# SMART-TTS/SMART-NAR_Fast_TTS

Hardware: AMD Instinct MI355X
Metric: mel_frames_per_sec (higher is better)
Workload: dtype f32

## Files before the change

### include/nar_fs2.h

```cpp
#ifndef NAR_FS2_H
#define NAR_FS2_H

#include <stddef.h>
#include <stdint.h>

#ifdef __cplusplus
extern "C" {
#endif

#define NS_ABI_VERSION 6

typedef struct ns_model ns_model;

typedef struct ns_config {
  int32_t n_vocab;
  int32_t max_seq_len;
  int32_t d_enc, n_enc_layer, n_enc_head;
  int32_t d_dec, n_dec_layer, n_dec_head;
  int32_t d_inner;
  int32_t ffn_k1, ffn_k2;
  int32_t vp_filter, vp_kernel;
  int32_t n_bins;
  int32_t n_mel;
  int32_t postnet_dim, postnet_k, postnet_n;
// ... 73 lines not shown
int ns_op_mel_decoder(ns_model* m, const float* x, const int64_t* lens, int B, int T, float* out, void* ws, size_t ws_bytes, void* stream);
int ns_op_mel_linear(ns_model* m, const float* x, int B, int T, float* out, void* stream);
int ns_op_postnet(ns_model* m, const float* mel, int B, int T, float* out, void* ws, size_t ws_bytes, void* stream);

int ns_op_ffn_conv1(ns_model* m, const char* prefix, const float* x, int B, int S, float* hidden, void* stream);
int ns_op_attention_core(const float* qkv, const int64_t* lens, int B, int S, int H, int dk, float* out, void* scratch,
                         size_t scratch_bytes, void* stream);
int ns_op_attention_core_mode(const float* qkv, const int64_t* lens, int B, int S, int H, int dk, float* out, void* scratch,
                              size_t scratch_bytes, void* stream, int flags);
int ns_op_attention_carve(int B, int S, int H, size_t scratch_bytes, int flags, size_t* partial_floats, int32_t* has_tickets);
int ns_plan_attention_dense(int B, int S, int H, int dk, size_t scratch_floats, int has_tickets, int32_t out[4]);
int ns_op_gemm(ns_model* m, const char* name, const float* x, int B, int S, float* out, void* stream);

int ns_plan_gemm(int M, int N, int Cin, int KW, int32_t out[8]);
int ns_plan_gemm_launches(int M, int N, int Cin, int KW, int epi, int32_t out[2][8]);
int ns_plan_row_tile(int M, int N);
int ns_plan_row_tile_k(int M, int N, int K);
int ns_acc_chunk(void);
int ns_abi_version(void);
int ns_plan_attention_split(int B, int S, int H, int dk);
int ns_plan_gemm_bf16(int M, int N, int32_t* bm, int32_t* bn);
int ns_plan_gemm_bf16_ln(int M, int N, int Cin, int KW);
int ns_plan_gemm_b3(int M, int N, int Cin, int KW, int epi, int32_t out[4]);
size_t ns_op_attention_scratch_bytes(int B, int S, int H, int dk);

int ns_op_pack_plan(const int64_t* lens_dev, const int64_t* lens_host, int B, int S, int H, int guard, int32_t* plan_dev, size_t plan_ints,
                    int32_t* Mp, int32_t* att_wgs, void* stream);
int ns_op_gemm_packed(ns_model* m, const char* name, const float* x_p, const int32_t* plan_dev, int B, int S, int Mp, int att_wgs, float* out_p,
                      void* stream);
int ns_op_attention_core_packed(const float* qkv_p, const int64_t* lens, const int32_t* plan_dev, int B, int S, int Mp, int att_wgs, int H, int dk,
                                float* out_p, void* scratch , size_t scratch_bytes, void* stream, int flags);
int ns_op_attention_packed_carve(int B, int S, int H, size_t scratch_bytes, int flags, size_t* partial_floats, int32_t* has_tickets);
int ns_plan_attention_packed(int B, int S, int H, int dk, int att_wgs, int Mp, size_t scratch_floats, int has_tickets, int32_t out[4]);
int ns_plan_attention_split_packed(int att_wgs, int S, int H, int dk, int Mp);
int ns_op_block_packed(ns_model* m, int which, const char* prefix, const float* x_p, const int64_t* lens ,
                       const int32_t* plan_dev, int B, int S, int Mp, int att_wgs, int mask_rows, float* out_p, void* ws, size_t ws_bytes,
                       void* stream);
int ns_op_length_regulate_packed(const float* x, const int32_t* cum, const int64_t* mel_lens, int B, int L, int D, int T, int Mp, int H,
                                 float* out_p, int32_t* status, int32_t* plan_dev, size_t plan_ints, void* stream);
int ns_op_gaussian_regulate(const float* x, const float* durations, const int64_t* own_len, int B, int L, int D, int T, float* out, float* s,
                            float* w, int32_t* status, int32_t* zero, int nzero, const int32_t* plan_dev, int Mp, int att_wgs, void* stream);
int ns_op_embed_pos_packed(const int64_t* texts, const float* emb, const float* pos, const int32_t* plan_dev, int B, int L, int Mp, int att_wgs, int D,
                           int n_vocab, float* out_p, void* stream);
int ns_op_add_pos_packed(const float* x_p, const float* pos, const int32_t* plan_dev, int B, int S, int Mp, int att_wgs, int D, float* out_p,
                         void* stream);
int ns_op_pack_vector(const float* src, const int32_t* plan_dev, int B, int S, int Mp, int att_wgs, float* dst_p, void* stream);
int ns_op_unpack_rows(const float* src_p, const int64_t* lens , const int32_t* plan_dev, int B, int S, int Mp, int att_wgs, int D,
                      float* dst, void* stream);
int ns_op_unpack_phase1(const float* rows_p, const float* vec_p, const int64_t* lens, const int32_t* plan_dev, int B, int S, int Mp, int att_wgs,
                        int D, float* rows, float* vec, void* stream);
int ns_op_unpack_outputs(const int32_t* plan_dev, int B, int T, int Mp, int att_wgs, int n_mel, const int64_t* mel_lens, const float* mel_p,
                         const float* post_p, const float* p_p, const float* e_p, const float* mel_bias, const float* post_const, float* mel,
                         float* post, float* p_pred, float* e_pred, uint8_t* mel_mask, void* stream);

#define NS_PROFILE_SLOTS 3
#define NS_PROFILE_OFF 0
#define NS_PROFILE_ALL 1
#define NS_PROFILE_SLOT(i) (2 << (i))
#define NS_PROFILE_KEEP 0x10000
int ns_profile_enable(ns_model* m, int on);
int ns_profile_read(ns_model* m, double* total_ms, double* total_flops, int64_t* launches);
int ns_profile_read_slot(ns_model* m, int slot, double* total_ms, double* total_flops, int64_t* launches);

#define NS_VOC_ABI_VERSION 1
typedef struct ns_vocoder ns_vocoder;
typedef struct ns_voc_config {
  int32_t n_mel;
  int32_t initial_channel;
  int32_t n_up;
  int32_t up_rates[4];
  int32_t up_kernels[4];
  int32_t n_rb;
  int32_t rb_kernels[4];
  int32_t rb_dilations[4][4];
  int32_t resblock;
} ns_voc_config;
int ns_voc_abi_version(void);
int ns_voc_create(const ns_voc_config* cfg, ns_vocoder** out);
void ns_voc_destroy(ns_vocoder* v);
int ns_voc_set_matmul(ns_vocoder* v, int mode);
size_t ns_voc_arena_bytes(const ns_vocoder* v);
int ns_voc_bind_arena(ns_vocoder* v, void* dev_arena, size_t bytes);
int ns_voc_set_weight(ns_vocoder* v, const char* name, const float* host, const int64_t* shape, int ndim);
int ns_voc_check_weight(ns_vocoder* v, const char* name, const int64_t* shape, int ndim);
int ns_voc_finalize_weights(ns_vocoder* v, void* stream);
size_t ns_voc_ws_bytes(const ns_vocoder* v, int B, int T);
#define NS_VOC_MEL_CHANNEL_MAJOR 0
#define NS_VOC_MEL_TIME_MAJOR 1
int ns_voc_forward(ns_vocoder* v, const float* mel, int mel_layout, int B, int T, float* wav, void* ws, size_t ws_bytes, void* stream);
int ns_voc_op_conv(ns_vocoder* v, const char* name, const float* x, int B, int S, float* out, void* stream);
int ns_voc_op_conv_form(ns_vocoder* v, const char* name, const float* x, const float* resid, float* y, int B, int S, int in_act,
                        int out_act, int mrf, void* stream);
int ns_voc_op_upsample(ns_vocoder* v, int i, const float* x, int B, int S, float* out, void* stream);
size_t ns_voc_op_stage_ws_bytes(const ns_vocoder* v, int i, int B, int S);
int ns_voc_op_stage(ns_vocoder* v, int i, const float* x, int B, int S, float* out, void* ws, size_t ws_bytes, void* stream);

#define NS_ALN_ABI_VERSION 1
int ns_aln_abi_version(void);
int ns_aln_create(const ns_config* cfg, ns_aligner** out);
void ns_aln_destroy(ns_aligner* a);
size_t ns_aln_arena_bytes(const ns_aligner* a);
int ns_aln_bind_arena(ns_aligner* a, void* dev_arena, size_t bytes);
int ns_aln_set_weight(ns_aligner* a, const char* name, const float* host, const int64_t* shape, int ndim);
int ns_aln_check_weight(ns_aligner* a, const char* name, const int64_t* shape, int ndim);
int ns_aln_finalize_weights(ns_aligner* a, void* stream);
size_t ns_aln_ws_bytes(const ns_aligner* a, int B, int L, int T);
// ... 315 lines not shown
```

### smart-nar_fast_tts_amd/_lib.py

```python
from __future__ import annotations

import ctypes as C
import os

import torch

_HERE = os.path.dirname(os.path.abspath(__file__))
LIB_PATH = os.path.join(_HERE, "csrc", "libnarfs2.so")


class NsConfig(C.Structure):
    _fields_ = [(n, C.c_int32) for n in (
        "n_vocab", "max_seq_len", "d_enc", "n_enc_layer", "n_enc_head", "d_dec", "n_dec_layer", "n_dec_head",
        "d_inner", "ffn_k1", "ffn_k2", "vp_filter", "vp_kernel", "n_bins", "n_mel",
        "postnet_dim", "postnet_k", "postnet_n", "pitch_frame_level", "energy_frame_level", "length_regulator",
        "matmul_bf16x3", "row_epilogue", "phase1_packing")]


class NsLossArgs(C.Structure):
    _fields_ = ([(n, C.c_int32) for n in ("B", "L", "T", "H", "n_mel", "pitch_frame_level", "energy_frame_level")]
                + [(n, C.c_int64) for n in ("mel_targets_stride", "d_targets_stride")]
                + [(n, C.c_void_p) for n in ("mel", "postnet", "mel_targets", "mel_masks", "pitch", "pitch_targets", "energy", "energy_targets",
                                             "log_d", "d_targets", "src_masks", "src_lens", "mel_lens")]
                + [("attn", C.c_void_p * 4)])
# ... 128 lines not shown

    "ns_last_phase2_rows": (C.c_int64, [_P]),
    "ns_plan_gemm": (_I, [_I, _I, _I, _I, C.POINTER(C.c_int32)]),
    "ns_plan_gemm_launches": (_I, [_I, _I, _I, _I, _I, C.POINTER(C.c_int32)]),
    "ns_plan_row_tile": (_I, [_I, _I]),
    "ns_plan_row_tile_k": (_I, [_I, _I, _I]),
    "ns_acc_chunk": (_I, []),
    "ns_plan_attention_split": (_I, [_I, _I, _I, _I]),
    "ns_op_ws_bytes": (_Z, [_P, _I, _I]),
    "ns_op_mask_from_lengths": (_I, [_P, _I, _I, _P, _P]),
    "ns_op_sinusoid_table": (_I, [_I, _I, _P, _P]),
    "ns_op_txt_encoder": (_I, [_P, _P, _P, _I, _I, _P, _P, _Z, _P]),
    "ns_op_multi_head_attention": (_I, [_P, _S, _P, _P, _I, _I, _P, _P, _Z, _P]),
    "ns_op_positionwise_ffn": (_I, [_P, _S, _P, _I, _I, _P, _P, _Z, _P]),
    "ns_op_fft_block": (_I, [_P, _S, _P, _P, _I, _I, _P, _P, _Z, _P]),
    "ns_op_variance_predictor": (_I, [_P, _S, _P, _P, _I, _I, _P, _P, _Z, _P]),
    "ns_op_predictor_conv1": (_I, [_P, _S, _P, _I, _I, _P, _P, _Z, _P]),
    "ns_op_predictor_tail": (_I, [_P, _S, _P, _P, _I, _I, _F, _P, _P, _I, _P, _P, _P, _Z, _P]),
    "ns_op_duration_round": (_I, [_P, _I, _F, _P, _P]),
    "ns_op_duration_scan": (_I, [_P, _I, _I, _P, _P, _P]),
    "ns_op_duration_target_scan": (_I, [_P, _P, _P, _I, _I, _I, _P, _P, _P, _P, _P]),
    "ns_op_length_regulate": (_I, [_P, _P, _I, _I, _I, _I, _P, _P]),
    "ns_op_variance_embedding": (_I, [_P, _I, _P, _P, _I, _I, _F, _P, _P, _P, _P, _Z, _P]),
    "ns_op_bucketize": (_I, [_P, _I, _P, _I, _P, _P]),
    "ns_op_gaussian_upsampling": (_I, [_P, _P, _I, _I, _I, _I, _I, _P, _P, _P, _P]),
    "ns_op_mel_decoder": (_I, [_P, _P, _P, _I, _I, _P, _P, _Z, _P]),
    "ns_op_mel_linear": (_I, [_P, _P, _I, _I, _P, _P]),
    "ns_op_postnet": (_I, [_P, _P, _I, _I, _P, _P, _Z, _P]),
    "ns_op_ffn_conv1": (_I, [_P, _S, _P, _I, _I, _P, _P]),
    "ns_op_attention_core": (_I, [_P, _P, _I, _I, _I, _I, _P, _P, _Z, _P]),
    "ns_op_attention_core_mode": (_I, [_P, _P, _I, _I, _I, _I, _P, _P, _Z, _P, _I]),
    "ns_op_attention_carve": (_I, [_I, _I, _I, _Z, _I, C.POINTER(C.c_size_t), C.POINTER(C.c_int32)]),
    "ns_plan_attention_dense": (_I, [_I, _I, _I, _I, _Z, _I, C.POINTER(C.c_int32)]),
    "ns_op_gemm": (_I, [_P, _S, _P, _I, _I, _P, _P]),
    "ns_plan_gemm_bf16": (_I, [_I, _I, C.POINTER(C.c_int32), C.POINTER(C.c_int32)]),
    "ns_plan_gemm_bf16_ln": (_I, [_I, _I, _I, _I]),
    "ns_plan_gemm_b3": (_I, [_I, _I, _I, _I, _I, C.POINTER(C.c_int32)]),
    "ns_op_attention_scratch_bytes": (_Z, [_I, _I, _I, _I]),
    "ns_op_pack_plan": (_I, [_P, _P, _I, _I, _I, _I, _P, _Z, C.POINTER(C.c_int32), C.POINTER(C.c_int32), _P]),
    "ns_op_gemm_packed": (_I, [_P, _S, _P, _P, _I, _I, _I, _I, _P, _P]),
    "ns_op_attention_core_packed": (_I, [_P, _P, _P, _I, _I, _I, _I, _I, _I, _P, _P, _Z, _P, _I]),
    "ns_op_attention_packed_carve": (_I, [_I, _I, _I, _Z, _I, C.POINTER(C.c_size_t), C.POINTER(C.c_int32)]),
    "ns_plan_attention_packed": (_I, [_I, _I, _I, _I, _I, _I, _Z, _I, C.POINTER(C.c_int32)]),
    "ns_plan_attention_split_packed": (_I, [_I, _I, _I, _I, _I]),
    "ns_op_block_packed": (_I, [_P, _I, _S, _P, _P, _P, _I, _I, _I, _I, _I, _P, _P, _Z, _P]),
    "ns_op_length_regulate_packed": (_I, [_P, _P, _P, _I, _I, _I, _I, _I, _I, _P, _P, _P, _Z, _P]),
    "ns_op_gaussian_regulate": (_I, [_P, _P, _P, _I, _I, _I, _I, _P, _P, _P, _P, _P, _I, _P, _I, _I, _P]),
    "ns_op_embed_pos_packed": (_I, [_P, _P, _P, _P, _I, _I, _I, _I, _I, _I, _P, _P]),
    "ns_op_add_pos_packed": (_I, [_P, _P, _P, _I, _I, _I, _I, _I, _P, _P]),
    "ns_op_pack_vector": (_I, [_P, _P, _I, _I, _I, _I, _P, _P]),
    "ns_op_unpack_rows": (_I, [_P, _P, _P, _I, _I, _I, _I, _I, _P, _P]),
    "ns_op_unpack_phase1": (_I, [_P, _P, _P, _P, _I, _I, _I, _I, _I, _P, _P, _P]),
    "ns_op_unpack_outputs": (_I, [_P, _I, _I, _I, _I, _I, _P, _P, _P, _P, _P, _P, _P, _P, _P, _P, _P, _P, _P]),
    "ns_profile_enable": (_I, [_P, _I]),
    "ns_profile_read": (_I, [_P, C.POINTER(C.c_double), C.POINTER(C.c_double), C.POINTER(C.c_int64)]),
    "ns_profile_read_slot": (_I, [_P, _I, C.POINTER(C.c_double), C.POINTER(C.c_double), C.POINTER(C.c_int64)]),
    **_handle_family("ns_voc", _P),
    "ns_voc_set_matmul": (_I, [_P, _I]),
    "ns_voc_ws_bytes": (_Z, [_P, _I, _I]),
    "ns_voc_forward": (_I, [_P, _P, _I, _I, _I, _P, _P, _Z, _P]),
    "ns_voc_op_conv": (_I, [_P, _S, _P, _I, _I, _P, _P]),
    "ns_voc_op_conv_form": (_I, [_P, _S, _P, _P, _P, _I, _I, _I, _I, _I, _P]),
    "ns_voc_op_upsample": (_I, [_P, _I, _P, _I, _I, _P, _P]),
    "ns_voc_op_stage_ws_bytes": (_Z, [_P, _I, _I, _I]),
    "ns_voc_op_stage": (_I, [_P, _I, _P, _I, _I, _P, _P, _Z, _P]),
    **_handle_family("ns_aln", C.POINTER(NsConfig)),
    "ns_aln_ws_bytes": (_Z, [_P, _I, _I, _I]),
    "ns_aln_forward": (_I, [_P, _P, _P, _P, _P, _I, _I, _I, _P, _P, _P, _P, _Z, _P]),
    "ns_aln_op_cross_attention": (_I, [_P, _P, _P, _I, _I, _I, _I, _I, _P, _P, _P]),
    "ns_aln_op_input": (_I, [_P, _P, _I, _I, _I, _P]),
    "ns_aln_op_durations": (_I, [_P, _P, _P, _I, _I, _I, _I, _P, _P]),
    "ns_loss_abi_version": (_I, []),
    "ns_loss_ws_bytes": (_Z, [_I, _I, _I]),
    "ns_loss_forward": (_I, [C.POINTER(NsLossArgs), _P, _Z, _P, _P]),
    **_handle_family("ns_mel", C.POINTER(NsMelConfig)),
    "ns_mel_frames": (C.c_int64, [C.c_int64, C.c_int32]),
    "ns_mel_ws_bytes": (_Z, [_P, _I, C.c_int64]),
    "ns_mel_forward": (_I, [_P, _P, C.c_int64, _P, _I, C.c_int64, _I, _P, _P, _P, _P, _Z, _P]),
    "ns_mel_op_frame_rows": (_I, [_P, _P, C.c_int64, _P, _I, C.c_int64, _I, _P, _P, _P]),
    "ns_mel_op_stft": (_I, [_P, _P, _I, _I, _P, _P]),
    "ns_mel_op_project": (_I, [_P, _P, _P, _I, _I, C.c_int64, _I, _P, _P, _P]),
    **_handle_family("ns_gl", C.POINTER(NsGlConfig)),
    "ns_gl_ws_bytes": (_Z, [_P, _I, _I]),
    "ns_gl_forward": (_I, [_P, _P, _P, _I, _I, _P, _I, _P, C.c_int64, _P, _P, _Z, _P]),
    "ns_gl_forward_mag": (_I, [_P, _P, _P, _I, _I, _P, _I, _P, C.c_int64, _P, _P, _Z, _P]),
    "ns_gl_transform": (_I, [_P, _P, C.c_int64, _P, _I, C.c_int64, _I, _P, _P, _P, _Z, _P]),
    "ns_gl_op_mel_to_mag": (_I, [_P, _P, _P, _I, _I, _P, _P]),
    "ns_gl_op_recombine": (_I, [_P, _P, _P, _P, _I, _I, _P, _P]),
    "ns_gl_op_rephase": (_I, [_P, _P, _P, _P, _I, _I, _I, _P, _P]),
    "ns_gl_op_inverse": (_I, [_P, _P, _P, _I, _I, _P, C.c_int64, _P, _P, _Z, _P]),
    "ns_gl_op_frame_rows": (_I, [_P, _P, C.c_int64, _P, _I, C.c_int64, _I, _P, _P]),
    "ns_gl_op_step": (_I, [_P, _P, _P, _I, _I, _P, C.c_int64, _P, _P, _Z, _P]),
    "ns_vt_abi_version": (_I, []),
    "ns_vt_ws_bytes": (_Z, [_I, _I, _I]),
    "ns_vt_state_init": (_I, [_P, _P]),
    "ns_vt_targets": (_I, [C.POINTER(NsVtArgs), _P, _Z, _P]),
    "ns_vt_fit": (_I, [C.POINTER(NsVtArgs), _P, _P, _Z, _P]),
    "ns_vt_normalize": (_I, [C.POINTER(NsVtArgs), _P, _P, _Z, _P]),
    "ns_opt_abi_version": (_I, []),
    "ns_opt_plan_sizes": (_I, [C.POINTER(C.c_int64), _I, C.POINTER(NsOptPlan)]),
    "ns_opt_build_table": (_I, [C.POINTER(C.c_int64), C.POINTER(_P), C.POINTER(_P), C.POINTER(C.c_int32), _I, _P, _Z]),
    "ns_opt_grad_norm": (_I, [C.POINTER(NsOptPlan), _P, _Z, _F, _P, _Z, _P, _P]),
    "ns_opt_scale_grads": (_I, [C.POINTER(NsOptPlan), _P, _Z, _P, _P]),
    "ns_opt_adam_step": (_I, [C.POINTER(NsOptPlan), _P, _Z, C.POINTER(NsOptHyper), _P, _P, C.c_int64, _P, _P]),
    "ns_opt_zero_grads": (_I, [C.POINTER(NsOptPlan), _P, _Z, _P]),
    "ns_lossg_abi_version": (_I, []),
# ... 89 lines not shown
```

### smart-nar_fast_tts_amd/csrc/api.hip

```cpp
#include <cstdio>

#include "../../include/nar_fs2.h"
#include "host_core.h"

using namespace ns;

static thread_local std::string g_err;
static int fail(const std::string& s) { g_err = s; return 1; }

namespace {

struct LayerW { ConvW qkv, fc, w1, w2; size_t ln1_g, ln1_b, ln2_g, ln2_b; };
struct PredW { ConvW c1, c2; size_t ln1_g, ln1_b, ln2_g, ln2_b, lin_w, lin_b; };

}

struct ns_model {
  ns_config cfg;
  std::vector<LayerW> enc, dec;
  PredW pred[3];
  size_t hdr;
  size_t emb, enc_pos, dec_pos, pitch_bins, energy_bins, pitch_emb, energy_emb;
  ConvW mel_linear;
  size_t pn_in, pn_hid, pn_const;
  size_t pos_long;
  std::vector<ConvW> post;
  Arena ar;
  float* arena = nullptr;
  bool ready = false;
  WeightRegistry weights;
  const float* P(size_t off) const { return arena + off; }
  const unsigned short* plane(size_t off) const { return off != NO_PLANE ? reinterpret_cast<const unsigned short*>(P(off)) : nullptr; }
  ConvGemm conv(const ConvW& w) const {
    ConvGemm p;
    memset(&p, 0, sizeof(p));
    p.W = P(w.w); p.bias = P(w.b); p.Wb3 = plane(w.b3); p.Wbf = plane(w.bf);
    p.N = w.cout; p.Cin = w.cin; p.KW = w.kw; p.pad = (w.kw - 1) / 2;
    return p;
  }
  struct ProfSlot { std::vector<std::pair<hipEvent_t, hipEvent_t>> ev; size_t used = 0; double flops = 0.0; };
  long long last_rows = 0;
  long long last_rows1 = 0;
  unsigned prof = 0;
  bool prof_active = false;
  ProfSlot prof_slot[NS_PROFILE_SLOTS];
};

static const char* kPredNames[3] = {"duration", "pitch", "energy"};

constexpr uint32_t ARENA_MAGIC = 0x3246534eu;
constexpr uint32_t ARENA_LAYOUT_VERSION = 6;
constexpr int ARENA_HDR_WORDS = 16;
static void arena_header(const ns_model* m, uint32_t* w) {
  memset(w, 0, ARENA_HDR_WORDS * sizeof(uint32_t));
  uint64_t h = 1469598103934665603ull;
  ns_config lay = m->cfg;
  lay.row_epilogue = 0;
  lay.phase1_packing = 0;
  const unsigned char* cb = reinterpret_cast<const unsigned char*>(&lay);
  for (size_t i = 0; i < sizeof(ns_config); ++i) { h ^= cb[i]; h *= 1099511628211ull; }
  w[0] = ARENA_MAGIC; w[1] = ARENA_LAYOUT_VERSION;
  w[2] = (uint32_t)(m->ar.n & 0xffffffffu); w[3] = (uint32_t)((uint64_t)m->ar.n >> 32);
  w[4] = (uint32_t)(h & 0xffffffffu); w[5] = (uint32_t)(h >> 32);
  w[6] = 1;
}
constexpr int POS_LONG_ROWS = 8192;
constexpr int PN_CONST_ROWS = 32;

static void expect(ns_model* m, const std::string& name, std::vector<int64_t> shape, bool optional = false) {
  m->weights.expect(name, std::move(shape), optional);
}

static void take_b3(Arena& ar, ConvW& w) { w.b3 = ar.take((3 * w.elems() + 1) / 2); }
static void take_bf(Arena& ar, ConvW& w) { w.bf = ar.take((bf16_plane_elems(w.cout, w.kw, w.cin) + 1) / 2); }
static void fill_planes(float* img, const ConvW& w) {
  if (w.b3 != NO_PLANE) {
    const size_t n = w.elems();
    unsigned short* pl = reinterpret_cast<unsigned short*>(&img[w.b3]);
    split_weights_b3(&img[w.w], n, pl, pl + n, pl + 2 * n);
  }
  if (w.bf != NO_PLANE) round_weights_bf16(&img[w.w], w.cout, w.kw, w.cin, reinterpret_cast<unsigned short*>(&img[w.bf]));
}

static void plan_stack(ns_model* m, const char* prefix, int n_layer, int d, std::vector<LayerW>& out, bool decoder) {
  const ns_config& c = m->cfg;
  for (int i = 0; i < n_layer; ++i) {
    std::string p = std::string(prefix) + ".layer_stack." + std::to_string(i);
    for (const char* w : {"w_qs", "w_ks", "w_vs", "fc"}) {
      expect(m, p + ".slf_attn." + w + ".weight", {d, d});
      expect(m, p + ".slf_attn." + w + ".bias", {d});
    }
    expect(m, p + ".slf_attn.layer_norm.weight", {d});
    expect(m, p + ".slf_attn.layer_norm.bias", {d});
    expect(m, p + ".pos_ffn.w_1.weight", {c.d_inner, d, c.ffn_k1});
    expect(m, p + ".pos_ffn.w_1.bias", {c.d_inner});
    expect(m, p + ".pos_ffn.w_2.weight", {d, c.d_inner, c.ffn_k2});
    expect(m, p + ".pos_ffn.w_2.bias", {d});
    expect(m, p + ".pos_ffn.layer_norm.weight", {d});
    expect(m, p + ".pos_ffn.layer_norm.bias", {d});
    LayerW L;
    L.qkv = m->ar.conv(3 * d, 1, d);
    L.fc = m->ar.conv(d, 1, d);
    L.ln1_g = m->ar.take(d); L.ln1_b = m->ar.take(d);
    L.w1 = m->ar.conv(c.d_inner, c.ffn_k1, d);
    L.w2 = m->ar.conv(d, c.ffn_k2, c.d_inner);
    L.ln2_g = m->ar.take(d); L.ln2_b = m->ar.take(d);
    if (c.matmul_bf16x3 == 1 && decoder)
      for (ConvW* w : {&L.qkv, &L.fc, &L.w1, &L.w2}) take_b3(m->ar, *w);
    if (c.matmul_bf16x3 == 2 && decoder)
      for (ConvW* w : {&L.qkv, &L.fc, &L.w1, &L.w2}) take_bf(m->ar, *w);
    out.push_back(L);
  }
}

extern "C" const char* ns_last_error(void) { return g_err.c_str(); }
int ns::api_fail(const char* msg) { return fail(msg); }

extern "C" int ns_create(const ns_config* cfg, ns_model** out) {
  if (!cfg || !out) return fail("ns_create: null argument");
// ... 21 lines not shown
  expect(m, "txt_encoder.src_word_emb.weight", {c.n_vocab, d});
  expect(m, "txt_encoder.position_enc", {1, npos, d}, true);
  expect(m, "mel_decoder.position_enc", {1, npos, c.d_dec}, true);
  m->emb = m->ar.take((size_t)c.n_vocab * d);
  m->enc_pos = m->ar.take((size_t)npos * d);
  m->dec_pos = m->ar.take((size_t)npos * c.d_dec);
  plan_stack(m, "txt_encoder", c.n_enc_layer, d, m->enc, false);
  plan_stack(m, "mel_decoder", c.n_dec_layer, c.d_dec, m->dec, true);
  const int F = c.vp_filter, K = c.vp_kernel;
  for (int i = 0; i < 3; ++i) {
    std::string p = std::string("variance_adaptor.") + kPredNames[i] + "_predictor";
    expect(m, p + ".conv_layer.conv1d_1.conv.weight", {F, d, K});
    expect(m, p + ".conv_layer.conv1d_1.conv.bias", {F});
    expect(m, p + ".conv_layer.layer_norm_1.weight", {F});
    expect(m, p + ".conv_layer.layer_norm_1.bias", {F});
    expect(m, p + ".conv_layer.conv1d_2.conv.weight", {F, F, K});
    expect(m, p + ".conv_layer.conv1d_2.conv.bias", {F});
    expect(m, p + ".conv_layer.layer_norm_2.weight", {F});
    expect(m, p + ".conv_layer.layer_norm_2.bias", {F});
    expect(m, p + ".linear_layer.weight", {1, F});
    expect(m, p + ".linear_layer.bias", {1});
    PredW& w = m->pred[i];
    w.c1 = m->ar.conv(F, K, d);
    w.ln1_g = m->ar.take(F); w.ln1_b = m->ar.take(F);
    w.c2 = m->ar.conv(F, K, F);
    w.ln2_g = m->ar.take(F); w.ln2_b = m->ar.take(F);
    w.lin_w = m->ar.take(F); w.lin_b = m->ar.take(1);
  }
  expect(m, "variance_adaptor.pitch_bins", {c.n_bins - 1});
  expect(m, "variance_adaptor.energy_bins", {c.n_bins - 1});
  expect(m, "variance_adaptor.pitch_embedding.weight", {c.n_bins, d});
  expect(m, "variance_adaptor.energy_embedding.weight", {c.n_bins, d});
  m->pitch_bins = m->ar.take(c.n_bins); m->energy_bins = m->ar.take(c.n_bins);
  m->pitch_emb = m->ar.take((size_t)c.n_bins * d); m->energy_emb = m->ar.take((size_t)c.n_bins * d);
  expect(m, "mel_linear.weight", {c.n_mel, c.d_dec});
  expect(m, "mel_linear.bias", {c.n_mel});
  m->mel_linear = m->ar.conv(c.n_mel, 1, c.d_dec);
  if (c.matmul_bf16x3 == 2) take_bf(m->ar, m->mel_linear);
  for (int i = 0; i < c.postnet_n; ++i) {
    const int cin = i == 0 ? c.n_mel : c.postnet_dim, cout = i == c.postnet_n - 1 ? c.n_mel : c.postnet_dim;
    std::string p = "postnet.convolutions." + std::to_string(i);
    expect(m, p + ".0.conv.weight", {cout, cin, c.postnet_k});
    expect(m, p + ".0.conv.bias", {cout});
    for (const char* s : {"weight", "bias", "running_mean", "running_var"}) expect(m, p + ".1." + s, {cout});
    ConvW w = m->ar.conv(cout, c.postnet_k, cin);
    if (c.matmul_bf16x3 == 1 && cin == c.postnet_dim && cout == c.postnet_dim) take_b3(m->ar, w);
    if (c.matmul_bf16x3 == 2) take_bf(m->ar, w);
    m->post.push_back(w);
  }
  m->pn_in = m->ar.take((size_t)PN_CONST_ROWS * c.n_mel);
  m->pn_hid = m->ar.take((size_t)2 * PN_CONST_ROWS * c.postnet_dim);
  m->pn_const = m->ar.take((size_t)PN_CONST_ROWS * c.n_mel);
  m->pos_long = m->ar.take((size_t)POS_LONG_ROWS * c.d_dec);
  *out = m;
  return 0;
}

extern "C" void ns_destroy(ns_model* m) {
  if (!m) return;
  for (auto& ps : m->prof_slot)
    for (auto& ev : ps.ev) { (void)hipEventDestroy(ev.first); (void)hipEventDestroy(ev.second); }
  delete m;
}
extern "C" size_t ns_arena_bytes(const ns_model* m) { return m ? m->ar.n * sizeof(float) : 0; }

extern "C" int ns_bind_arena(ns_model* m, void* dev, size_t bytes) { return bind_arena(m, dev, bytes, ns_arena_bytes(m), "ns_bind_arena"); }

extern "C" int ns_adopt_arena(ns_model* m) {
  if (!m || !m->arena) return fail("ns_adopt_arena: no arena bound");
  uint32_t got[ARENA_HDR_WORDS], want[ARENA_HDR_WORDS];
  int cur_dev = 0;
  NS_HIP(hipGetDevice(&cur_dev));
  hipPointerAttribute_t at;
  NS_HIP(hipPointerGetAttributes(&at, m->arena));
  struct DevGuard { int d; bool on; ~DevGuard() { if (on) (void)hipSetDevice(d); } } guard{cur_dev, at.device != cur_dev};
  if (guard.on) NS_HIP(hipSetDevice(at.device));
  NS_HIP(hipDeviceSynchronize());
  NS_HIP(hipMemcpy(got, m->arena + m->hdr, sizeof(got), hipMemcpyDeviceToHost));
  arena_header(m, want);
  if (got[0] != ARENA_MAGIC) return fail("ns_adopt_arena: the arena does not start with this library's magic word (not a finalized ns_model arena)");
  if (got[1] != want[1]) return fail("ns_adopt_arena: arena layout version " + std::to_string(got[1]) + ", this library packs version " + std::to_string(want[1]));
  if (got[2] != want[2] || got[3] != want[3]) return fail("ns_adopt_arena: arena size differs from ns_arena_bytes of this model");
  if (got[4] != want[4] || got[5] != want[5]) return fail("ns_adopt_arena: the arena was packed for a different ns_config");
  if (got[6] != 1) return fail("ns_adopt_arena: the arena was not finalized (ns_finalize_weights did not complete)");
  m->weights.release();
  m->ready = true;
  return 0;
}

static bool starts_with(const std::string& s, const char* p) { return s.rfind(p, 0) == 0; }
static bool ends_with(const std::string& s, const char* p) {
  size_t n = strlen(p); return s.size() >= n && s.compare(s.size() - n, n, p) == 0;
}

static bool ignored_key(const char* name) { return starts_with(name, "mel_encoder.") || ends_with(name, ".num_batches_tracked"); }

extern "C" int ns_check_weight(ns_model* m, const char* name, const int64_t* shape, int ndim) {
  if (m && name && ignored_key(name)) return 0;
  return check_weight(m, name, shape, ndim, "ns_check_weight");
}

extern "C" int ns_set_weight(ns_model* m, const char* name, const float* host, const int64_t* shape, int ndim) {
  if (m && name && ignored_key(name)) return 0;
  return set_weight(m, name, host, shape, ndim, "ns_set_weight");
}

static int postnet_constants(ns_model* m, hipStream_t st);
extern "C" int ns_finalize_weights(ns_model* m, void* stream) {
  if (!m) return fail("ns_finalize_weights: null model");
  if (!m->arena) return fail("ns_finalize_weights: bind an arena first (ns_bind_arena)");
  const std::vector<std::string> missing = m->weights.missing();
  if (!missing.empty()) return fail("ns_finalize_weights: missing keys: " + join_names(missing));
  const ns_config& c = m->cfg;
  std::vector<float> img(m->ar.n, 0.f);
  auto S = [&](const std::string& k) -> const std::vector<float>& { return m->weights.data(k); };
  auto cp = [&](size_t off, const std::string& k) { const auto& v = S(k); memcpy(&img[off], v.data(), v.size() * sizeof(float)); };

  arena_header(m, reinterpret_cast<uint32_t*>(&img[m->hdr]));
  cp(m->emb, "txt_encoder.src_word_emb.weight");
  const int npos = c.max_seq_len + 1;
  if (m->weights.is_set("txt_encoder.position_enc")) cp(m->enc_pos, "txt_encoder.position_enc");
  else host_sinusoid(npos, c.d_enc, &img[m->enc_pos]);
  if (m->weights.is_set("mel_decoder.position_enc")) cp(m->dec_pos, "mel_decoder.position_enc");
  else host_sinusoid(npos, c.d_dec, &img[m->dec_pos]);

  auto do_stack = [&](const char* prefix, std::vector<LayerW>& Ls, int d) {
    for (size_t i = 0; i < Ls.size(); ++i) {
      const LayerW& L = Ls[i];
      std::string p = std::string(prefix) + ".layer_stack." + std::to_string(i);
      const char* qkv[3] = {"w_qs", "w_ks", "w_vs"};
      for (int t = 0; t < 3; ++t) {
        memcpy(&img[L.qkv.w + (size_t)t * d * d], S(p + ".slf_attn." + qkv[t] + ".weight").data(), (size_t)d * d * 4);
        memcpy(&img[L.qkv.b + (size_t)t * d], S(p + ".slf_attn." + qkv[t] + ".bias").data(), (size_t)d * 4);
      }
      cp(L.fc.w, p + ".slf_attn.fc.weight"); cp(L.fc.b, p + ".slf_attn.fc.bias");
      cp(L.ln1_g, p + ".slf_attn.layer_norm.weight"); cp(L.ln1_b, p + ".slf_attn.layer_norm.bias");
      pack_conv(S(p + ".pos_ffn.w_1.weight"), c.d_inner, d, c.ffn_k1, &img[L.w1.w]); cp(L.w1.b, p + ".pos_ffn.w_1.bias");
      cp(L.ln2_g, p + ".pos_ffn.layer_norm.weight"); cp(L.ln2_b, p + ".pos_ffn.layer_norm.bias");
      pack_conv(S(p + ".pos_ffn.w_2.weight"), d, c.d_inner, c.ffn_k2, &img[L.w2.w]); cp(L.w2.b, p + ".pos_ffn.w_2.bias");
      for (const ConvW* w : {&L.qkv, &L.fc, &L.w1, &L.w2}) fill_planes(img.data(), *w);
    }
  };
  do_stack("txt_encoder", m->enc, c.d_enc);
  do_stack("mel_decoder", m->dec, c.d_dec);

  for (int i = 0; i < 3; ++i) {
    const PredW& w = m->pred[i];
    std::string p = std::string("variance_adaptor.") + kPredNames[i] + "_predictor";
    pack_conv(S(p + ".conv_layer.conv1d_1.conv.weight"), c.vp_filter, w.c1.cin, c.vp_kernel, &img[w.c1.w]);
    cp(w.c1.b, p + ".conv_layer.conv1d_1.conv.bias");
    cp(w.ln1_g, p + ".conv_layer.layer_norm_1.weight"); cp(w.ln1_b, p + ".conv_layer.layer_norm_1.bias");
    pack_conv(S(p + ".conv_layer.conv1d_2.conv.weight"), c.vp_filter, c.vp_filter, c.vp_kernel, &img[w.c2.w]);
    cp(w.c2.b, p + ".conv_layer.conv1d_2.conv.bias");
    cp(w.ln2_g, p + ".conv_layer.layer_norm_2.weight"); cp(w.ln2_b, p + ".conv_layer.layer_norm_2.bias");
    cp(w.lin_w, p + ".linear_layer.weight"); cp(w.lin_b, p + ".linear_layer.bias");
  }
  cp(m->pitch_bins, "variance_adaptor.pitch_bins"); cp(m->energy_bins, "variance_adaptor.energy_bins");
  cp(m->pitch_emb, "variance_adaptor.pitch_embedding.weight"); cp(m->energy_emb, "variance_adaptor.energy_embedding.weight");
  cp(m->mel_linear.w, "mel_linear.weight"); cp(m->mel_linear.b, "mel_linear.bias");
  fill_planes(img.data(), m->mel_linear);

  for (size_t i = 0; i < m->post.size(); ++i) {
    const ConvW& w = m->post[i];
    std::string p = "postnet.convolutions." + std::to_string(i);
    const auto &g = S(p + ".1.weight"), &b = S(p + ".1.bias"), &mu = S(p + ".1.running_mean"), &var = S(p + ".1.running_var");
    const auto& cb = S(p + ".0.conv.bias");
    std::vector<double> sc(w.cout);
    for (int o = 0; o < w.cout; ++o) {
      sc[o] = (double)g[o] / std::sqrt((double)var[o] + 1e-5);
      img[w.b + o] = (float)(((double)cb[o] - (double)mu[o]) * sc[o] + (double)b[o]);
    }
    pack_conv(S(p + ".0.conv.weight"), w.cout, w.cin, c.postnet_k, &img[w.w], sc.data());
    fill_planes(img.data(), w);
  }
  hipStream_t st = (hipStream_t)stream;
  NS_HIP(hipMemcpyAsync(m->arena, img.data(), img.size() * sizeof(float), hipMemcpyHostToDevice, st));
  NS_TRY(postnet_constants(m, st));
  NS_HIP(launch_sinusoid(POS_LONG_ROWS, c.d_dec, m->arena + m->pos_long, st));
  NS_HIP(hipStreamSynchronize(st));
  m->weights.release();
  m->ready = true;
  return 0;
}

namespace {
struct PackedCtx { RowMap rm; int Mp; };

struct Scratch {
  const PackedCtx* pk;
  float *xa, *xb, *qkv, *att, *t1, *x1, *hid, *vp1, *vp2, *pos_ext, *att_part;
  size_t att_part_floats;
  Tickets tk;
};

static size_t imax(size_t a, size_t b) { return a > b ? a : b; }

static Scratch carve(const ns_config& c, Bump& bp, size_t M, int S, bool no_split = false) {
  Scratch s;
  s.pk = nullptr;
  const size_t d = c.d_enc;
  s.xa = bp.f(M * d); s.xb = bp.f(M * d);
  s.qkv = bp.f(M * 3 * d); s.att = bp.f(M * d); s.t1 = bp.f(M * d); s.x1 = bp.f(M * d);
  s.hid = bp.f(M * imax(c.d_inner, 2 * (size_t)c.postnet_dim));
  s.vp1 = bp.f(M * c.vp_filter); s.vp2 = bp.f(M * c.vp_filter);
  s.pos_ext = S > c.max_seq_len ? bp.f((size_t)S * d) : nullptr;
  const int hmax = c.n_enc_head > c.n_dec_head ? c.n_enc_head : c.n_dec_head;
  int nsp = 1;
  if (!no_split && S > 0) {
    const int Bg = (int)(M / (size_t)S);
    const int ne = attention_split(Bg, S, c.n_enc_head, c.d_enc / c.n_enc_head), nd = attention_split(Bg, S, c.n_dec_head, c.d_dec / c.n_dec_head);
    nsp = ne > nd ? ne : nd;
  }
  s.att_part_floats = nsp > 1 ? (size_t)nsp * (M * d + 2 * M * hmax) : 0;
  s.att_part = s.att_part_floats ? bp.f(s.att_part_floats) : nullptr;
  s.tk.base = (int*)bp.raw(TICKET_INTS * sizeof(int));
  if (c.row_epilogue == 1) s.tk.base = nullptr;
  s.tk.used = 0;
  return s;
}
}

extern "C" size_t ns_op_ws_bytes(const ns_model* m, int B, int S) {
  if (!m || B <= 0 || S <= 0) return 256;
  Bump bp(nullptr);
  carve(m->cfg, bp, (size_t)B * S, S);
  return bp.off + 256;
}
static size_t phase1_packed_extra_bytes(const ns_config& c, int B, int L);
extern "C" size_t ns_encoder_ws_bytes(const ns_model* m, int B, int L) {
  if (!m || B <= 0 || L <= 0) return 256;
  Bump bp(nullptr);
  bp.f((size_t)B * L * m->cfg.d_enc);
  bp.raw((size_t)B * L * sizeof(int32_t));
  bp.f((size_t)B * L);
  carve(m->cfg, bp, (size_t)B * L, L);
  return bp.off + phase1_packed_extra_bytes(m->cfg, B, L) + 256;
}
static size_t packed_extra_bytes(const ns_config& c, int B, int T);
extern "C" size_t ns_decoder_ws_bytes(const ns_model* m, int B, int L, int T) {
  (void)L;
  if (!m || B <= 0 || T <= 0) return ns_op_ws_bytes(m, B, T);
  return ns_op_ws_bytes(m, B, T) + packed_extra_bytes(m->cfg, B, T);
}

static int check_ready(const ns_model* m) {
  if (!m) return fail("null model");
  if (!m->ready) return fail("weights not loaded: call ns_set_weight for every key, then ns_finalize_weights (or ns_adopt_arena)");
  return 0;
}

static const RowMap* cur_rm(const Scratch& sc) { return sc.pk ? &sc.pk->rm : nullptr; }
static int rows_of(const Scratch& sc, int B, int S) { return sc.pk ? sc.pk->Mp : B * S; }

struct GemmOpts {
  const RowEpilogue* epi = nullptr; int epi_mode = EPI_NONE;
  const LaunchTiming* tm = nullptr;
  static GemmOpts row(const RowEpilogue& e, int mode) { GemmOpts o; o.epi = &e; o.epi_mode = mode; return o; }
  static GemmOpts timed(const LaunchTiming* tm) { GemmOpts o; o.tm = tm; return o; }
};

static ConvGemm prepare(const ns_model* m, const Scratch& sc, const ConvW& w, const float* X, const float* resid, float* Y, int M, int S, int act) {
  ConvGemm p = m->conv(w);
  p.X = X; p.ldx = w.cin; p.resid = resid; p.ldr = w.cout; p.Y = Y; p.ldy = w.cout;
  p.M = M; p.S = S; p.act = act;
  if (sc.pk) { p.rm = sc.pk->rm; p.e.row_b = sc.pk->rm.row_b; p.e.row_t = sc.pk->rm.row_t; }
  return p;
}

static int gemm(const ns_model* m, const Scratch& sc, const ConvW& w, const float* X, const float* resid, float* Y, int M, int S, int act,
                hipStream_t st, const GemmOpts& o = GemmOpts()) {
  ConvGemm p = prepare(m, sc, w, X, resid, Y, M, S, act);
  const LaunchTiming* tm = o.tm;
  if (o.epi) {
    p.epi = o.epi_mode;
    p.e = *o.epi;
    if (sc.pk) { p.e.row_b = sc.pk->rm.row_b; p.e.row_t = sc.pk->rm.row_t; }
  }
  if (p.Wbf) {
    if (p.epi != EPI_NONE && p.epi != EPI_LN) return fail("gemm: the bf16 path has no predictor-tail epilogue");
    p.Wb3 = nullptr;
    p.e.ticket = nullptr; p.e.y_out = nullptr;
    if (tm && tm->start) NS_HIP(hipEventRecord(tm->start, st));
    NS_HIP(launch_conv_gemm_bf16(p, st));
    if (tm && tm->stop) NS_HIP(hipEventRecord(tm->stop, st));
    return 0;
  }
  if (p.Wb3 && conv_gemm_b3_ok(M, p.N, p.Cin, p.KW, p.epi)) {
// ... 16 lines not shown
}

static int gemm_ln(const ns_model* m, Scratch& sc, const ConvW& w, const float* X, const float* resid, float* tmp, float* Y, int M, int S,
                   int act, const float* g, const float* b, const long long* lens, hipStream_t st) {
  RowEpilogue e;
  memset(&e, 0, sizeof(e));
  e.ln_g = g; e.ln_b = b; e.lens = lens;
  const int N = w.cout;
  if (w.bf != NO_PLANE) {
    if (conv_gemm_bf16_ok(M, N, w.cin, w.kw, EPI_LN)) return gemm(m, sc, w, X, resid, Y, M, S, act, st, GemmOpts::row(e, EPI_LN));
    NS_TRY(gemm(m, sc, w, X, resid, tmp, M, S, act, st));
    NS_HIP(launch_layernorm(tmp, g, b, Y, M, N, S, lens, st, cur_rm(sc)));
    return 0;
  }
  if (w.b3 != NO_PLANE) {
    const B3LnForm form = gemm_ln_b3_form(M, N, w.cin, w.kw);
    if (form == B3_LN_TWO_LAUNCH) {
      NS_TRY(gemm(m, sc, w, X, resid, tmp, M, S, act, st));
      NS_HIP(launch_layernorm(tmp, g, b, Y, M, N, S, lens, st, cur_rm(sc)));
      return 0;
    }
    if (form == B3_LN_FULL_ROW) return gemm(m, sc, w, X, resid, Y, M, S, act, st, GemmOpts::row(e, EPI_LN));
  }
  if (sc.pk) { e.row_b = sc.pk->rm.row_b; e.row_t = sc.pk->rm.row_t; }
  return gemm_ln_fp32(prepare(m, sc, w.fp32(), X, resid, nullptr, M, S, act), e, tmp, Y, sc.tk, st, cur_rm(sc));
}

struct ProfScope {
  ns_model* m; int slot; double flops; bool on;
  LaunchTiming tm{nullptr, nullptr};
  ProfScope(ns_model* m_, int slot_, double flops_) : m(m_), slot(slot_), flops(flops_), on(m_->prof_active && ((m_->prof >> slot_) & 1u)) {}
  int begin() {
    if (!on) return 0;
    ns_model::ProfSlot& ps = m->prof_slot[slot];
    if (ps.used == ps.ev.size()) {
      hipEvent_t a, b;
      NS_HIP(hipEventCreate(&a));
      NS_HIP(hipEventCreate(&b));
      ps.ev.emplace_back(a, b);
    }
    tm = LaunchTiming{ps.ev[ps.used].first, ps.ev[ps.used].second};
    return 0;
  }
  const LaunchTiming* timing() const { return on ? &tm : nullptr; }
  void end() {
    if (!on) return;
    ns_model::ProfSlot& ps = m->prof_slot[slot];
    ps.used++;
    ps.flops += flops;
  }
};

static int mha(ns_model* m, const LayerW& L, int d, int H, const float* x, const long long* lens, int B, int S,
               float* out, bool mask_rows, Scratch& sc, hipStream_t st) {
  const int M = rows_of(sc, B, S);
  const bool bf = L.qkv.bf != NO_PLANE;
  NS_TRY(gemm(m, sc, L.qkv, x, nullptr, sc.qkv, M, S, ACT_NONE, st));
  {
    ProfScope ps(m, 1, 4.0 * (double)M * (double)S * (double)d);
    NS_TRY(ps.begin());
    NS_HIP(launch_attention(sc.qkv, lens, B, S, H, d / H, sc.att, sc.att_part, sc.att_part_floats,
                            (sc.att_part && attention_uses_tickets(B, S, H)) ? sc.tk.take(attention_ticket_ints(B, S, H)) : nullptr, st, cur_rm(sc),
                            ps.timing(), bf));
    ps.end();
  }
  return gemm_ln(m, sc, L.fc, sc.att, x, sc.t1, out, M, S, ACT_NONE, m->P(L.ln1_g), m->P(L.ln1_b), mask_rows ? lens : nullptr, st);
}

static int ffn(ns_model* m, const LayerW& L, int d, const float* x, const long long* lens, int B, int S, float* out,
               bool mask_rows, Scratch& sc, hipStream_t st) {
  const ns_config& c = m->cfg;
  const int M = rows_of(sc, B, S);
  {
    ProfScope ps(m, 0, 2.0 * (double)M * (double)c.ffn_k1 * (double)d * (double)c.d_inner);
    NS_TRY(ps.begin());
    NS_TRY(gemm(m, sc, L.w1, x, nullptr, sc.hid, M, S, ACT_RELU, st, GemmOpts::timed(ps.timing())));
    ps.end();
  }
  return gemm_ln(m, sc, L.w2, sc.hid, x, sc.t1, out, M, S, ACT_NONE, m->P(L.ln2_g), m->P(L.ln2_b), mask_rows ? lens : nullptr, st);
}

static int fft_block(ns_model* m, const LayerW& L, int d, int H, const float* x, const long long* lens, int B, int S,
                     float* out, Scratch& sc, hipStream_t st) {
  NS_TRY(mha(m, L, d, H, x, lens, B, S, sc.x1, true, sc, st));
  NS_TRY(ffn(m, L, d, sc.x1, lens, B, S, out, true, sc, st));
  return 0;
}

static int position_rows(const ns_model* m, size_t cached_off, int S, int d, Scratch& sc, const float** pos, hipStream_t st) {
  if (S > m->cfg.max_seq_len && S <= POS_LONG_ROWS) {
    *pos = m->P(m->pos_long);
  } else if (S > m->cfg.max_seq_len) {
    NS_HIP(launch_sinusoid(S, d, sc.pos_ext, st));
    *pos = sc.pos_ext;
  } else {
    *pos = m->P(cached_off);
  }
  return 0;
}

static int predictor_conv1(const ns_model* m, const PredW& w, const float* x, int B, int S, float* h, Scratch& sc, hipStream_t st) {
  const int M = rows_of(sc, B, S);
  return gemm_ln(m, sc, w.c1, x, nullptr, sc.vp1, h, M, S, ACT_RELU, m->P(w.ln1_g), m->P(w.ln1_b), nullptr, st);
}
static int predictor_tail(const ns_model* m, const PredW& w, const float* h, const long long* lens, int B, int S, float control,
                          const float* target, float* pred, const float* bins, const float* emb, const float* x_in, const float* pos,
                          float* x_out, Scratch& sc, hipStream_t st) {
  const ns_config& c = m->cfg;
  const int M = rows_of(sc, B, S), F = c.vp_filter, D = w.c1.cin;
  RowEpilogue e;
  memset(&e, 0, sizeof(e));
  e.ln_g = m->P(w.ln2_g); e.ln_b = m->P(w.ln2_b); e.lens = lens; e.wlin = m->P(w.lin_w); e.blin = m->P(w.lin_b); e.pred = pred;
  e.control = control; e.target = target; e.bins = bins; e.n_edges = c.n_bins - 1; e.emb = emb; e.x_in = x_in; e.pos = pos; e.x_out = x_out;
  e.D = D;
  if (fuse_row_epilogue(M, F, F)) return gemm(m, sc, w.c2, h, nullptr, nullptr, M, S, ACT_RELU, st, GemmOpts::row(e, EPI_LN_PRED));
  if (conv_gemm_ticket_ok(M, F, F) && (e.ticket = sc.tk.take(conv_gemm_ticket_ints(M))) != nullptr)
    return gemm(m, sc, w.c2, h, nullptr, sc.vp1, M, S, ACT_RELU, st, GemmOpts::row(e, EPI_LN_PRED));
  NS_TRY(gemm(m, sc, w.c2, h, nullptr, sc.vp1, M, S, ACT_RELU, st));
  NS_HIP(launch_ln_linear_embed(sc.vp1, m->P(w.ln2_g), m->P(w.ln2_b), m->P(w.lin_w), m->P(w.lin_b), pred, M, F, S, lens,
                                control, target, bins, c.n_bins, emb, x_in, pos, x_out, D, st, cur_rm(sc)));
  return 0;
}
static int predictor(const ns_model* m, const PredW& w, const float* x, const long long* lens, int B, int S, float control,
                     const float* target,
                     float* pred, const float* bins, const float* emb, const float* pos, float* x_out, Scratch& sc,
                     hipStream_t st) {
  NS_TRY(predictor_conv1(m, w, x, B, S, sc.vp2, sc, st));
  return predictor_tail(m, w, sc.vp2, lens, B, S, control, target, pred, bins, emb, x, pos, x_out, sc, st);
}

static int postnet(ns_model* m, const float* mel, int B, int T, const float* resid, float* out, Scratch& sc, hipStream_t st) {
  const ns_config& c = m->cfg;
  const int M = rows_of(sc, B, T);
  float* ping = sc.hid;
  float* pong = sc.hid + (size_t)M * c.postnet_dim;
  const float* cur = mel;
  for (size_t i = 0; i < m->post.size(); ++i) {
    const ConvW& w = m->post[i];
    const bool last = i + 1 == m->post.size();
    float* dst = last ? out : ((i & 1) ? pong : ping);
    const bool mid = w.cin == c.postnet_dim && w.cout == c.postnet_dim;
    ProfScope ps(m, 2, 2.0 * (double)M * (double)c.postnet_k * (double)w.cin * (double)w.cout);
    if (mid) NS_TRY(ps.begin());
    NS_TRY(gemm(m, sc, w, cur, last ? resid : nullptr, dst, M, T, last ? ACT_NONE : ACT_TANH, st, GemmOpts::timed(mid ? ps.timing() : nullptr)));
    if (mid) ps.end();
    cur = dst;
  }
  return 0;
}

static int postnet_constants(ns_model* m, hipStream_t st) {
  const ns_config& c = m->cfg;
  float* in = m->arena + m->pn_in;
  NS_HIP(launch_broadcast_row(m->P(m->mel_linear.b), in, PN_CONST_ROWS, c.n_mel, st));
  Scratch sc;
  memset(&sc, 0, sizeof(sc));
  sc.hid = m->arena + m->pn_hid;
  return postnet(m, in, 1, PN_CONST_ROWS, in, m->arena + m->pn_const, sc, st);
}

static int encoder(ns_model* m, const long long* texts, const long long* lens, int B, int L, float* out, Scratch& sc,
                   hipStream_t st) {
  const ns_config& c = m->cfg;
  const int M = rows_of(sc, B, L), d = c.d_enc;
  const float* pos;
  NS_TRY(position_rows(m, m->enc_pos, L, d, sc, &pos, st));
  float* cur = m->enc.empty() ? out : sc.xa;
  if (sc.pk) NS_HIP(launch_embed_pos_packed(texts, m->P(m->emb), pos, cur, sc.pk->rm, B, M, L, d, c.n_vocab, sc.tk.base, TICKET_INTS, st));
  else NS_HIP(launch_embed_pos(texts, m->P(m->emb), pos, cur, M, L, d, c.n_vocab, sc.tk.base, TICKET_INTS, st));
  for (size_t i = 0; i < m->enc.size(); ++i) {
    float* dst = (i + 1 == m->enc.size()) ? out : (cur == sc.xa ? sc.xb : sc.xa);
    NS_TRY(fft_block(m, m->enc[i], d, c.n_enc_head, cur, lens, B, L, dst, sc, st));
    cur = dst;
  }
  return 0;
}

static int decoder_stack(ns_model* m, float* x, const long long* lens, int B, int T, float* out, Scratch& sc, hipStream_t st) {
  const ns_config& c = m->cfg;
  float* cur = x;
  float* alt = (x == sc.xa) ? sc.xb : sc.xa;
  for (size_t i = 0; i < m->dec.size(); ++i) {
    float* dst = (i + 1 == m->dec.size()) ? out : alt;
    NS_TRY(fft_block(m, m->dec[i], c.d_dec, c.n_dec_head, cur, lens, B, T, dst, sc, st));
    if (dst != out) { alt = cur; cur = dst; }
  }
  if (m->dec.empty() && out != x) NS_HIP(hipMemcpyAsync(out, x, (size_t)rows_of(sc, B, T) * c.d_dec * 4, hipMemcpyDeviceToDevice, st));
  return 0;
}

static size_t window_rows(const int64_t* lens_host, int B, int S, int guard) {
  size_t mp = 0;
  for (int b = 0; b < B; ++b) {
    long long l = (lens_host[b] < 0 ? 0 : lens_host[b]) + guard;
    mp += (size_t)(l < (long long)S ? l : (long long)S);
  }
  return mp;
}
static int window_att_wgs(const int64_t* lens_host, int B, int S, int guard, int H) {
  int wgs = 0;
  for (int b = 0; b < B; ++b) {
    long long l = (lens_host[b] < 0 ? 0 : lens_host[b]) + guard;
    wgs += (int)(((l < S ? l : S) + 127) / 128) * H;
  }
  return wgs;
}
static size_t phase1_packed_rows(const int64_t* lens_host, int B, int L) { return window_rows(lens_host, B, L, PHONEME_GUARD); }
static size_t phase1_packed_extra_bytes(const ns_config& c, int B, int L) {
  Bump bp(nullptr);
  const size_t M = (size_t)B * L;
  bp.raw(pack_plan_ints(B, M) * sizeof(int));
  bp.f(M * c.d_enc); bp.f(M);
  return bp.off;
}

struct Teacher {
  ns_aligner* aln;
  const float* mels;
  const int64_t* mel_lens_in;
  int T;
  void* ws_aln;
  size_t ws_aln_bytes;
  float *tgt_output, *attn;
  int64_t* d_targets;
};

static int forward_durations(ns_model* m, const int64_t* texts, const int64_t* src_lens, const int64_t* lens_host, int B, int L, float d_control,
                             float p_control, float e_control, const float* p_targets, const float* e_targets,
                             void* ws_enc, size_t ws_bytes, float* log_d, float* d_rounded, uint8_t* src_mask,
                             int64_t* mel_lens, float* p_pred, float* e_pred, int64_t* mel_lens_host, void* stream,
                             const Teacher* tf = nullptr) {
  NS_TRY(check_ready(m));
  if (B <= 0 || L <= 0) return fail("ns_forward_durations: empty batch");
  if (ws_bytes < ns_encoder_ws_bytes(m, B, L)) return fail("ns_forward_durations: workspace too small");
  hipStream_t st = (hipStream_t)stream;
  const ns_config& c = m->cfg;
  if (!c.pitch_frame_level && !p_pred) return fail("ns_forward_durations: phoneme_level pitch needs a p_pred [B,L] output");
  if (!c.energy_frame_level && !e_pred) return fail("ns_forward_durations: phoneme_level energy needs an e_pred [B,L] output");
  Bump bp(ws_enc);
  float* enc_out = bp.f((size_t)B * L * c.d_enc);
  int32_t* cum = (int32_t*)bp.raw((size_t)B * L * sizeof(int32_t));
  float* dur_keep = bp.f((size_t)B * L);
  const long long* lens = (const long long*)src_lens;
  size_t Mp = 0;
  bool packed = lens_host && !m->enc.empty() && launch_planner_enabled() && c.pitch_frame_level && c.energy_frame_level && c.phase1_packing != 2;
  if (packed) {
    Mp = phase1_packed_rows(lens_host, B, L);
    auto cu_rows = [&](size_t rows) {
      const size_t ntn = (size_t)c.d_inner / 128, w32 = (rows + 31) / 32 * ntn, w48 = (rows + 47) / 48 * ntn;
      return (conv_gemm_tile16_enabled() && w32 > 256 && w48 <= 256) ? (size_t)48 : 32 * ((w32 + 255) / 256);
    };
    packed = Mp > 0 && Mp * 10 <= (size_t)B * L * 9 && (c.phase1_packing == 1 || cu_rows(Mp) < cu_rows((size_t)B * L));
  }
  const size_t Mrows = packed ? Mp : (size_t)B * L;
  m->last_rows1 = (long long)Mrows;
  Scratch sc = carve(c, bp, Mrows, L, packed);
  PackedCtx pk;
  memset(&pk, 0, sizeof(pk));
  float *enc_w = enc_out, *logd_w = log_d;
  if (packed) {
    const int M = (int)Mp, d = c.d_enc;
    const int base = window_att_wgs(lens_host, B, L, PHONEME_GUARD, c.n_enc_head);
    size_t n = (size_t)attention_split_packed(base, L, d / c.n_enc_head, Mp, d);
    const size_t per = Mp * d + 2 * Mp * c.n_enc_head;
    const size_t extra = phase1_packed_extra_bytes(c, B, L);
    const size_t avail = ws_bytes > bp.off + extra ? (ws_bytes - bp.off - extra) / sizeof(float) : 0;
    while (n > 1 && n * per > avail) --n;
    if (n > 1) { sc.att_part_floats = n * per; sc.att_part = bp.f(sc.att_part_floats); }
    int* plan = (int*)bp.raw(pack_plan_ints(B, Mp) * sizeof(int));
    enc_w = bp.f(Mp * d); logd_w = bp.f(Mp);
    if (bp.off > ws_bytes) return fail("ns_forward_durations: workspace too small (packed rows)");
    pk.Mp = M;
    pk.rm.rows = M;
    pk.rm.att_wgs = base;
    NS_HIP(launch_pack_plan_only(lens, B, L, c.n_enc_head, M, plan, &pk.rm, st, PHONEME_GUARD));
  }
  {
    sc.pk = packed ? &pk : nullptr;
    NS_TRY(encoder(m, (const long long*)texts, lens, B, L, enc_w, sc, st));
    if (tf) {
      if (tf->T > 0) NS_TRY(ns_aln_forward(tf->aln, enc_w, src_lens, tf->mels, tf->mel_lens_in, B, L, tf->T, tf->tgt_output, tf->attn, tf->d_targets,
                                           tf->ws_aln, tf->ws_aln_bytes, stream));
      else NS_HIP(hipMemsetAsync(tf->d_targets, 0, (size_t)B * L * sizeof(int64_t), st));
    }
    NS_TRY(predictor(m, m->pred[0], enc_w, lens, B, L, 1.0f, nullptr, logd_w, nullptr, nullptr, nullptr, nullptr, sc, st));
    if (!c.pitch_frame_level)
      NS_TRY(predictor(m, m->pred[1], enc_w, lens, B, L, p_control, p_targets, p_pred, m->P(m->pitch_bins), m->P(m->pitch_emb), nullptr, enc_w, sc, st));
    if (!c.energy_frame_level)
      NS_TRY(predictor(m, m->pred[2], enc_w, lens, B, L, e_control, e_targets, e_pred, m->P(m->energy_bins), m->P(m->energy_emb), nullptr, enc_w, sc, st));
  }
  if (packed) {
    NS_HIP(launch_unpack_phase1(pk.rm, lens, B, L, c.d_enc, enc_w, enc_out, logd_w, log_d, st));
  }
  if (tf) {
    NS_HIP(launch_duration_target_tail((const long long*)tf->d_targets, lens, (const long long*)texts, c.n_vocab, B, L, dur_keep, cum,
                                       (long long*)mel_lens, src_mask, st));
    return 0;
  }
  NS_HIP(launch_duration_tail(log_d, lens, (const long long*)texts, c.n_vocab, B, L, d_control, d_rounded, dur_keep, cum,
                              (long long*)mel_lens, src_mask, (long long*)mel_lens_host, st));
  return 0;
}

extern "C" int ns_forward_durations(ns_model* m, const int64_t* texts, const int64_t* src_lens, int B, int L, float d_control,
                                    float p_control, float e_control, const float* p_targets, const float* e_targets,
                                    void* ws_enc, size_t ws_bytes, float* log_d, float* d_rounded, uint8_t* src_mask,
                                    int64_t* mel_lens, float* p_pred, float* e_pred, int64_t* mel_lens_host, void* stream) {
  return forward_durations(m, texts, src_lens, nullptr, B, L, d_control, p_control, e_control, p_targets, e_targets, ws_enc, ws_bytes, log_d,
                           d_rounded, src_mask, mel_lens, p_pred, e_pred, mel_lens_host, stream);
}

extern "C" int ns_forward_durations_teacher(ns_model* m, ns_aligner* aln, const int64_t* texts, const int64_t* src_lens, const float* mels,
                                            const int64_t* mel_lens_in, int B, int L, int T, float p_control, float e_control,
                                            const float* p_targets, const float* e_targets, void* ws_enc, size_t ws_enc_bytes, void* ws_aln,
                                            size_t ws_aln_bytes, float* log_d, uint8_t* src_mask, int64_t* mel_lens, float* p_pred, float* e_pred,
                                            float* tgt_output, float* attn_all_layers, int64_t* d_targets, void* stream) {
  if (!aln) return fail("ns_forward_durations_teacher: null aligner");
  if (T < 0) return fail("ns_forward_durations_teacher: negative T");
  if (!log_d || !src_mask || !mel_lens || !d_targets) return fail("ns_forward_durations_teacher: log_d, src_mask, mel_lens and d_targets are required");
  if (T > 0 && (!mels || !mel_lens_in || !tgt_output || !attn_all_layers || !ws_aln))
    return fail("ns_forward_durations_teacher: mels, mel_lens_in, tgt_output, attn_all_layers and ws_aln are required when T > 0");
  if (m && m->cfg.d_enc != 256) return fail("ns_forward_durations_teacher: the aligner takes a 256-wide encoder output (ns_aln_create)");
  if (T > 0 && B > 0 && L > 0 && ws_aln_bytes < ns_aln_ws_bytes(aln, B, L, T)) return fail("ns_forward_durations_teacher: aligner workspace too small (ns_aln_ws_bytes)");
  if (T > 0 && (((uintptr_t)ws_aln & 255) || ((uintptr_t)ws_enc & 255) || (((uintptr_t)mels | (uintptr_t)tgt_output) & 15)))
    return fail("ns_forward_durations_teacher: workspaces must be 256-byte aligned, mels and tgt_output 16-byte aligned");
  const Teacher tf = {aln, mels, mel_lens_in, T, ws_aln, ws_aln_bytes, tgt_output, attn_all_layers, d_targets};
  return forward_durations(m, texts, src_lens, nullptr, B, L, 1.0f, p_control, e_control, p_targets, e_targets, ws_enc, ws_enc_bytes, log_d,
                           nullptr, src_mask, mel_lens, p_pred, e_pred, nullptr, stream, &tf);
}

extern "C" int ns_upload_lengths(const int64_t* host, int n, int64_t* dev, void* stream) {
  if (n < 0 || (n > 0 && (!host || !dev))) return fail("ns_upload_lengths: null argument");
  NS_HIP(launch_store_lens((const long long*)host, n, (long long*)dev, (hipStream_t)stream));
  return 0;
}

extern "C" int ns_forward_durations_packed(ns_model* m, const int64_t* texts, const int64_t* src_lens, const int64_t* src_lens_host, int B, int L,
                                           float d_control, float p_control, float e_control, const float* p_targets, const float* e_targets,
                                           void* ws_enc, size_t ws_bytes, float* log_d, float* d_rounded, uint8_t* src_mask,
                                           int64_t* mel_lens, float* p_pred, float* e_pred, int64_t* mel_lens_host, void* stream) {
  if (!src_lens_host) return fail("ns_forward_durations_packed: src_lens_host (the host copy of src_lens) is required");
  return forward_durations(m, texts, src_lens, src_lens_host, B, L, d_control, p_control, e_control, p_targets, e_targets, ws_enc, ws_bytes, log_d,
                           d_rounded, src_mask, mel_lens, p_pred, e_pred, mel_lens_host, stream);
}

static size_t packed_rows(const int64_t* lens_host, int B, int T) { return window_rows(lens_host, B, T, PACK_GUARD); }
static size_t packed_extra_bytes(const ns_config& c, int B, int T) {
  Bump bp(nullptr);
  const size_t M = (size_t)B * T;
  bp.raw(pack_plan_ints(B, M) * sizeof(int));
  bp.f(M * c.n_mel); bp.f(M * c.n_mel); bp.f(M); bp.f(M); bp.f(M); bp.f(M);
  return bp.off;
}

static int forward_mel(ns_model* m, int B, int L, int T, const int64_t* mel_lens, const int64_t* lens_host, float p_control, float e_control,
                       const float* p_targets, const float* e_targets,
                       const void* ws_enc, void* ws_dec, size_t ws_bytes, float* mel, float* postnet_mel, float* p_pred,
                       float* e_pred, uint8_t* mel_mask, int32_t* status, void* stream) {
  NS_TRY(check_ready(m));
  if (B <= 0 || L <= 0) return fail("ns_forward_mel: empty batch");
  if (!status) return fail("ns_forward_mel: status [B] is required (a T smaller than an utterance's length must not go unnoticed)");
  if (T < 0) return fail("ns_forward_mel: negative T");
  if (T == 0) {
    Bump be0(const_cast<void*>(ws_enc));
    be0.f((size_t)B * L * m->cfg.d_enc);
    const int32_t* cum0 = (const int32_t*)be0.raw((size_t)B * L * sizeof(int32_t));
    NS_HIP(launch_length_regulate(nullptr, cum0, B, L, m->cfg.d_enc, 0, nullptr, nullptr, (const long long*)mel_lens, status, nullptr, 0, (hipStream_t)stream));
    return 0;
  }
  if (ws_bytes < ns_decoder_ws_bytes(m, B, L, T)) return fail("ns_forward_mel: workspace too small");
  hipStream_t st = (hipStream_t)stream;
  const ns_config& c = m->cfg;
  Bump be(const_cast<void*>(ws_enc));
  const float* enc_out = be.f((size_t)B * L * c.d_enc);
  const int32_t* cum = (const int32_t*)be.raw((size_t)B * L * sizeof(int32_t));
  const float* dur_keep = be.f((size_t)B * L);
  const long long* lens = (const long long*)mel_lens;
  const int d = c.d_dec;
  size_t Mp = 0;
  bool packed = lens_host && c.matmul_bf16x3 != 1 && !m->dec.empty();
  if (packed) {
    Mp = packed_rows(lens_host, B, T);
    const size_t grid_rows = (size_t)B * T;
    packed = Mp > 0 && Mp < ((size_t)1 << 30) && Mp * 10 <= grid_rows * (grid_rows <= 20000 ? 8 : 9);
  }
  const size_t Mrows = packed ? Mp : (size_t)B * T;
  const int M = (int)Mrows;
  m->last_rows = (long long)Mrows;
  Bump bp(ws_dec);
  Scratch sc = carve(c, bp, Mrows, T, packed);
  if (packed) {
    const int base = window_att_wgs(lens_host, B, T, PACK_GUARD, c.n_dec_head);
    size_t n = (size_t)attention_split_packed(base, T, d / c.n_dec_head, Mrows, d);
    if (n > 1) {
      const size_t per = Mrows * d + 2 * Mrows * c.n_dec_head;
      const size_t avail = ws_bytes > bp.off + packed_extra_bytes(c, B, T) ? (ws_bytes - bp.off - packed_extra_bytes(c, B, T)) / sizeof(float) : 0;
      while (n > 1 && n * per > avail) --n;
      if (n > 1) { sc.att_part_floats = n * per; sc.att_part = bp.f(sc.att_part_floats); }
    }
  }

  PackedCtx pk;
  memset(&pk, 0, sizeof(pk));
  float *mel_p = nullptr, *post_p = nullptr, *pp_p = nullptr, *ep_p = nullptr;
  if (packed) {
    int* plan = (int*)bp.raw(pack_plan_ints(B, Mp) * sizeof(int));
    mel_p = bp.f(Mp * c.n_mel); post_p = bp.f(Mp * c.n_mel); pp_p = bp.f(Mp); ep_p = bp.f(Mp);
    float* pt_p = bp.f(Mp);
    float* et_p = bp.f(Mp);
    if (bp.off > ws_bytes) return fail("ns_forward_mel_packed: workspace too small");
    pk.Mp = M;
    pk.rm.rows = M;
    if (c.length_regulator == 1) {
      if ((size_t)B * (L + 1) > (size_t)M * c.vp_filter) return fail("ns_forward_mel: workspace too small for the Gaussian centres");
      NS_HIP(launch_pack_plan(lens, B, T, c.n_dec_head, M, plan, &pk.rm, st));
      NS_HIP(launch_gaussian_upsampling(enc_out, dur_keep, B, L, c.d_enc, T, T, sc.xa, sc.vp2, nullptr, lens, status, sc.tk.base, TICKET_INTS, st, &pk.rm));
    } else {
      NS_HIP(launch_length_regulate_packed(enc_out, cum, B, L, c.d_enc, T, M, c.n_dec_head, sc.xa, lens, status, sc.tk.base, TICKET_INTS, plan, &pk.rm, st));
    }
    pk.rm.att_wgs = window_att_wgs(lens_host, B, T, PACK_GUARD, c.n_dec_head);
    if (p_targets && c.pitch_frame_level) { NS_HIP(launch_pack_vector(pk.rm, T, p_targets, pt_p, M, st)); p_targets = pt_p; }
    if (e_targets && c.energy_frame_level) { NS_HIP(launch_pack_vector(pk.rm, T, e_targets, et_p, M, st)); e_targets = et_p; }
  } else if (c.length_regulator == 1) {
    NS_HIP(launch_mask_from_lengths(lens, B, T, mel_mask, st));
    if ((size_t)B * (L + 1) > (size_t)M * c.vp_filter) return fail("ns_forward_mel: workspace too small for the Gaussian centres");
    NS_HIP(launch_gaussian_upsampling(enc_out, dur_keep, B, L, c.d_enc, T, T, sc.xa, sc.vp2, nullptr, lens, status, sc.tk.base, TICKET_INTS, st));
  } else {
    NS_HIP(launch_length_regulate(enc_out, cum, B, L, c.d_enc, T, sc.xa, mel_mask, lens, status, sc.tk.base, TICKET_INTS, st));
  }
  sc.pk = packed ? &pk : nullptr;
  float* const mel_dst = packed ? mel_p : mel;
  float* const post_dst = packed ? post_p : postnet_mel;
  float* const pp_dst = packed ? pp_p : p_pred;
  float* const ep_dst = packed ? ep_p : e_pred;
  const float* pos;
  NS_TRY(position_rows(m, m->dec_pos, T, d, sc, &pos, st));
  float* cur = sc.xa;
  float* alt = sc.xb;
  if (c.pitch_frame_level) {
    if (!p_pred) return fail("ns_forward_mel: frame_level pitch needs a p_pred [B,T] output");
    NS_TRY(predictor(m, m->pred[1], cur, lens, B, T, p_control, p_targets, pp_dst, m->P(m->pitch_bins), m->P(m->pitch_emb),
                     c.energy_frame_level ? nullptr : pos, alt, sc, st));
    float* t = cur; cur = alt; alt = t;
  }
  if (c.energy_frame_level) {
    if (!e_pred) return fail("ns_forward_mel: frame_level energy needs an e_pred [B,T] output");
    NS_TRY(predictor(m, m->pred[2], cur, lens, B, T, e_control, e_targets, ep_dst, m->P(m->energy_bins), m->P(m->energy_emb), pos,
                     alt, sc, st));
    float* t = cur; cur = alt; alt = t;
  }
  if (!c.pitch_frame_level && !c.energy_frame_level) {
    NS_HIP(launch_add_pos(cur, pos, alt, M, T, d, st, cur_rm(sc)));
    float* t = cur; cur = alt; alt = t;
  }
  m->prof_active = m->prof != 0;
  int rc = decoder_stack(m, cur, lens, B, T, sc.att, sc, st);
  if (!rc) rc = gemm(m, sc, m->mel_linear, sc.att, nullptr, mel_dst, M, T, ACT_NONE, st);
  if (!rc) rc = postnet(m, mel_dst, B, T, mel_dst, post_dst, sc, st);
  m->prof_active = false;
  if (!rc && packed) {
    hipError_t e = launch_unpack_outputs(pk.rm, B, T, c.n_mel, lens, mel_p, post_p, c.pitch_frame_level ? pp_p : nullptr,
                                         c.energy_frame_level ? ep_p : nullptr, m->P(m->mel_linear.b), m->P(m->pn_const) + (size_t)21 * c.n_mel, mel, postnet_mel,
                                         c.pitch_frame_level ? p_pred : nullptr, c.energy_frame_level ? e_pred : nullptr, mel_mask, st);
    if (e != hipSuccess) rc = fail(std::string("launch_unpack_outputs: ") + hipGetErrorString(e));
  }
  return rc;
}

extern "C" int64_t ns_last_phase2_rows(const ns_model* m) { return m ? (int64_t)m->last_rows : 0; }
extern "C" int64_t ns_last_phase1_rows(const ns_model* m) { return m ? (int64_t)m->last_rows1 : 0; }

extern "C" int ns_forward_mel(ns_model* m, int B, int L, int T, const int64_t* mel_lens, float p_control, float e_control,
                              const float* p_targets, const float* e_targets,
                              const void* ws_enc, void* ws_dec, size_t ws_bytes, float* mel, float* postnet_mel, float* p_pred,
                              float* e_pred, uint8_t* mel_mask, int32_t* status, void* stream) {
  return forward_mel(m, B, L, T, mel_lens, nullptr, p_control, e_control, p_targets, e_targets, ws_enc, ws_dec, ws_bytes, mel, postnet_mel,
                     p_pred, e_pred, mel_mask, status, stream);
}

extern "C" int ns_forward_mel_packed(ns_model* m, int B, int L, int T, const int64_t* mel_lens, const int64_t* mel_lens_host,
                                     float p_control, float e_control, const float* p_targets, const float* e_targets,
                                     const void* ws_enc, void* ws_dec, size_t ws_bytes, float* mel, float* postnet_mel, float* p_pred,
                                     float* e_pred, uint8_t* mel_mask, int32_t* status, void* stream) {
  if (!mel_lens_host) return fail("ns_forward_mel_packed: mel_lens_host (the host copy of mel_lens) is required");
  return forward_mel(m, B, L, T, mel_lens, mel_lens_host, p_control, e_control, p_targets, e_targets, ws_enc, ws_dec, ws_bytes, mel,
                     postnet_mel, p_pred, e_pred, mel_mask, status, stream);
}

static int find_layer(ns_model* m, const char* prefix_c, const LayerW** L, int* d, int* H, const char* suffix) {
  std::string p(prefix_c ? prefix_c : "");
  if (suffix && *suffix) {
    if (!ends_with(p, suffix)) return fail("prefix '" + p + "' does not end with '" + suffix + "'");
    p.resize(p.size() - strlen(suffix));
  }
  const bool enc = starts_with(p, "txt_encoder.layer_stack."), dec = starts_with(p, "mel_decoder.layer_stack.");
  if (!enc && !dec) return fail("unknown module prefix '" + std::string(prefix_c ? prefix_c : "") + "'");
  const char* num = p.c_str() + (enc ? strlen("txt_encoder.layer_stack.") : strlen("mel_decoder.layer_stack."));
  char* end = nullptr;
  const long idx = strtol(num, &end, 10);
  if (end == num || *end != 0 || *num < '0' || *num > '9') return fail("no layer index in '" + std::string(prefix_c ? prefix_c : "") + "'");
  auto& v = enc ? m->enc : m->dec;
  if (idx < 0 || idx >= (long)v.size()) return fail("layer index out of range in '" + p + "'");
  *L = &v[idx];
  *d = enc ? m->cfg.d_enc : m->cfg.d_dec;
  *H = enc ? m->cfg.n_enc_head : m->cfg.n_dec_head;
  return 0;
}

#define NS_OP_PROLOGUE(B_, S_)                                                        \
// ... 39 lines not shown
  NS_TRY(find_layer(m, prefix, &L, &d, &H, ""));
  return fft_block(m, *L, d, H, x, (const long long*)lens, B, S, out, sc, st);
}
static int find_pred(const char* prefix, int* idx) {
  std::string p(prefix ? prefix : "");
  for (int i = 0; i < 3; ++i)
    if (p == std::string("variance_adaptor.") + kPredNames[i] + "_predictor") { *idx = i; return 0; }
  return fail("unknown predictor prefix '" + p + "'");
}
extern "C" int ns_op_variance_predictor(ns_model* m, const char* prefix, const float* x, const int64_t* lens, int B, int S,
                                        float* out, void* ws, size_t ws_bytes, void* stream) {
  NS_OP_PROLOGUE(B, S);
  int i;
  NS_TRY(find_pred(prefix, &i));
  return predictor(m, m->pred[i], x, (const long long*)lens, B, S, 1.0f, nullptr, out, nullptr, nullptr, nullptr, nullptr, sc, st);
}
extern "C" int ns_op_duration_round(const float* log_d, int n, float d_control, float* d_rounded, void* stream) {
  NS_HIP(launch_duration_round(log_d, n, d_control, d_rounded, (hipStream_t)stream));
  return 0;
}
extern "C" int ns_op_duration_target_scan(const int64_t* d_targets, const int64_t* src_lens, const int64_t* texts, int n_vocab, int B, int L,
                                          int32_t* cum, float* dur_keep, uint8_t* src_mask, int64_t* mel_lens, void* stream) {
  if (B < 0 || L < 0) return fail("ns_op_duration_target_scan: negative size");
  if (B > 0 && (!src_lens || !mel_lens || (L > 0 && (!d_targets || !cum || !dur_keep || !src_mask)))) return fail("ns_op_duration_target_scan: null argument");
  NS_HIP(launch_duration_target_tail((const long long*)d_targets, (const long long*)src_lens, (const long long*)texts, n_vocab, B, L, dur_keep, cum,
                                     (long long*)mel_lens, src_mask, (hipStream_t)stream));
  return 0;
}
extern "C" int ns_op_duration_scan(const float* d_rounded, int B, int L, int32_t* cum, int64_t* mel_lens, void* stream) {
  NS_HIP(launch_duration_scan(d_rounded, B, L, cum, (long long*)mel_lens, (hipStream_t)stream));
  return 0;
}
extern "C" int ns_op_length_regulate(const float* x, const int32_t* cum, int B, int L, int D, int T, float* out, void* stream) {
  NS_HIP(launch_length_regulate(x, cum, B, L, D, T, out, nullptr, nullptr, nullptr, nullptr, 0, (hipStream_t)stream));
  return 0;
}
extern "C" int ns_op_variance_embedding(ns_model* m, int which, const float* x, const int64_t* lens, int B, int S, float control,
                                        const float* target, float* pred, float* x_out, void* ws, size_t ws_bytes, void* stream) {
  NS_OP_PROLOGUE(B, S);
  if (which != 0 && which != 1) return fail("which must be 0 (pitch) or 1 (energy)");
  const size_t bins = which ? m->energy_bins : m->pitch_bins, emb = which ? m->energy_emb : m->pitch_emb;
  return predictor(m, m->pred[1 + which], x, (const long long*)lens, B, S, control, target, pred, m->P(bins), m->P(emb), nullptr, x_out,
                   sc, st);
}
extern "C" int ns_op_predictor_conv1(ns_model* m, const char* prefix, const float* x, int B, int S, float* h, void* ws, size_t ws_bytes,
                                     void* stream) {
  if (!m) return fail("null model");
  int i;
  NS_TRY(find_pred(prefix, &i));
  if (!x || !h || !ws) return fail("ns_op_predictor_conv1: null argument");
  NS_OP_PROLOGUE(B, S);
  return predictor_conv1(m, m->pred[i], x, B, S, h, sc, st);
}
extern "C" int ns_op_predictor_tail(ns_model* m, const char* prefix, const float* h, const int64_t* lens, int B, int S, float control,
                                    const float* target, const float* x_in, int add_pos, float* pred, float* x_out, void* ws,
                                    size_t ws_bytes, void* stream) {
  if (!m) return fail("null model");
  int i;
  NS_TRY(find_pred(prefix, &i));
  if (!h || !lens || !pred || !ws) return fail("ns_op_predictor_tail: null argument");
  if (i == 0 && (x_in || x_out || add_pos)) return fail("ns_op_predictor_tail: the duration predictor has no embedding");
  if (x_in && !x_out) return fail("ns_op_predictor_tail: x_in without x_out");
  if (!x_in && (x_out || add_pos)) return fail("ns_op_predictor_tail: x_out / add_pos without x_in");
  NS_OP_PROLOGUE(B, S);
  const PredW& w = m->pred[i];
  const float *bins = nullptr, *emb = nullptr, *pos = nullptr;
  if (x_in) {
    bins = m->P(i == 2 ? m->energy_bins : m->pitch_bins);
    emb = m->P(i == 2 ? m->energy_emb : m->pitch_emb);
    if (add_pos) NS_TRY(position_rows(m, m->dec_pos, S, w.c1.cin, sc, &pos, st));
  }
  return predictor_tail(m, w, h, (const long long*)lens, B, S, control, target, pred, bins, emb, x_in, pos, x_out, sc, st);
}
extern "C" int ns_plan_gemm(int M, int N, int Cin, int KW, int32_t out[8]) {
  int o[8] = {0, 0, 0, 0, 0, 0, 0, 0};
  const bool planned = conv_gemm_plan(M, N, Cin, KW, o);
  if (out) for (int i = 0; i < 8; ++i) out[i] = planned ? o[i] : 0;
  return planned ? 1 : 0;
}
extern "C" int ns_plan_gemm_launches(int M, int N, int Cin, int KW, int epi, int32_t out[2][8]) {
  int o[2][8];
  const int n = conv_gemm_describe(M, N, Cin, KW, epi, o);
  if (out)
    for (int l = 0; l < 2; ++l)
      for (int i = 0; i < 8; ++i) out[l][i] = o[l][i];
  return n;
}
extern "C" int ns_plan_row_tile_k(int M, int N, int K) {
  if (M <= 0 || K <= 0 || (N != 256 && N != 512)) return 0;
  return conv_gemm_row_tile(M, N, K);
}
extern "C" int ns_plan_row_tile(int M, int N) { return ns_plan_row_tile_k(M, N, N); }
extern "C" int ns_acc_chunk(void) { return conv_gemm_acc_chunk(); }
extern "C" int ns_abi_version(void) { return NS_ABI_VERSION; }
extern "C" int ns_plan_attention_split(int B, int S, int H, int dk) { return attention_split(B, S, H, dk); }

extern "C" int ns_profile_enable(ns_model* m, int on) {
  if (!m) return fail("ns_profile_enable: null model");
  const bool keep = on > 0 && (on & NS_PROFILE_KEEP) != 0;
  if (on > 0) on &= ~NS_PROFILE_KEEP;
  m->prof = on == 1 ? (1u << NS_PROFILE_SLOTS) - 1u : on < 0 ? 0u : ((unsigned)on >> 1);
  if (!keep)
    for (auto& ps : m->prof_slot) { ps.used = 0; ps.flops = 0.0; }
  return 0;
}
extern "C" int ns_profile_read_slot(ns_model* m, int slot, double* total_ms, double* total_flops, int64_t* launches) {
  if (!m) return fail("ns_profile_read_slot: null model");
  if (slot < 0 || slot >= NS_PROFILE_SLOTS) return fail("ns_profile_read_slot: slot out of range");
  ns_model::ProfSlot& ps = m->prof_slot[slot];
  double ms = 0.0;
  for (size_t i = 0; i < ps.used; ++i) {
    NS_HIP(hipEventSynchronize(ps.ev[i].second));
    float e = 0.f;
    NS_HIP(hipEventElapsedTime(&e, ps.ev[i].first, ps.ev[i].second));
    ms += e;
  }
  if (total_ms) *total_ms = ms;
  if (total_flops) *total_flops = ps.flops;
  if (launches) *launches = (int64_t)ps.used;
  ps.used = 0;
  ps.flops = 0.0;
  return 0;
}
extern "C" int ns_profile_read(ns_model* m, double* total_ms, double* total_flops, int64_t* launches) {
  return ns_profile_read_slot(m, 0, total_ms, total_flops, launches);
// ... 271 lines not shown
  if (!texts || !emb || !pos || !out_p) return fail("ns_op_embed_pos_packed: null argument");
  if (D <= 0 || D % 4 != 0 || n_vocab <= 0) return fail("ns_op_embed_pos_packed: bad shape");
  PackedCtx pk;
  NS_TRY(packed_ctx("ns_op_embed_pos_packed", plan_dev, B, L, Mp, att_wgs, &pk));
  NS_HIP(launch_embed_pos_packed((const long long*)texts, emb, pos, out_p, pk.rm, B, Mp, L, D, n_vocab, nullptr, 0, (hipStream_t)stream));
  return 0;
}
extern "C" int ns_op_add_pos_packed(const float* x_p, const float* pos, const int32_t* plan_dev, int B, int S, int Mp, int att_wgs, int D, float* out_p,
                                    void* stream) {
  if (!x_p || !pos || !out_p) return fail("ns_op_add_pos_packed: null argument");
  if (D <= 0 || D % 4 != 0) return fail("ns_op_add_pos_packed: D must be a positive multiple of 4");
  PackedCtx pk;
  NS_TRY(packed_ctx("ns_op_add_pos_packed", plan_dev, B, S, Mp, att_wgs, &pk));
  NS_HIP(launch_add_pos(x_p, pos, out_p, Mp, S, D, (hipStream_t)stream, &pk.rm));
  return 0;
}
extern "C" int ns_op_pack_vector(const float* src, const int32_t* plan_dev, int B, int S, int Mp, int att_wgs, float* dst_p, void* stream) {
  if (!src || !dst_p) return fail("ns_op_pack_vector: null argument");
  PackedCtx pk;
  NS_TRY(packed_ctx("ns_op_pack_vector", plan_dev, B, S, Mp, att_wgs, &pk));
  NS_HIP(launch_pack_vector(pk.rm, S, src, dst_p, Mp, (hipStream_t)stream));
  return 0;
}
extern "C" int ns_op_unpack_rows(const float* src_p, const int64_t* lens, const int32_t* plan_dev, int B, int S, int Mp, int att_wgs, int D, float* dst,
                                 void* stream) {
  if (!src_p || !dst) return fail("ns_op_unpack_rows: null argument");
  if (D <= 0) return fail("ns_op_unpack_rows: D must be positive");
  PackedCtx pk;
  NS_TRY(packed_ctx("ns_op_unpack_rows", plan_dev, B, S, Mp, att_wgs, &pk));
  NS_HIP(launch_unpack_rows(pk.rm, (const long long*)lens, B, S, D, src_p, dst, (hipStream_t)stream));
  return 0;
}
extern "C" int ns_op_unpack_phase1(const float* rows_p, const float* vec_p, const int64_t* lens, const int32_t* plan_dev, int B, int S, int Mp,
                                   int att_wgs, int D, float* rows, float* vec, void* stream) {
  if (!rows_p || !vec_p || !lens || !rows || !vec) return fail("ns_op_unpack_phase1: null argument");
  if (D <= 0 || D % 4 != 0) return fail("ns_op_unpack_phase1: D must be a positive multiple of 4");
  PackedCtx pk;
  NS_TRY(packed_ctx("ns_op_unpack_phase1", plan_dev, B, S, Mp, att_wgs, &pk));
  NS_HIP(launch_unpack_phase1(pk.rm, (const long long*)lens, B, S, D, rows_p, rows, vec_p, vec, (hipStream_t)stream));
  return 0;
}
extern "C" int ns_op_unpack_outputs(const int32_t* plan_dev, int B, int T, int Mp, int att_wgs, int n_mel, const int64_t* mel_lens, const float* mel_p,
                                    const float* post_p, const float* p_p, const float* e_p, const float* mel_bias, const float* post_const,
                                    float* mel, float* post, float* p_pred, float* e_pred, uint8_t* mel_mask, void* stream) {
  if (!mel_lens || !mel_p || !post_p || !mel_bias || !post_const || !mel || !post) return fail("ns_op_unpack_outputs: null argument");
  if ((p_pred && !p_p) || (e_pred && !e_p)) return fail("ns_op_unpack_outputs: p_pred / e_pred without their packed source");
  if (n_mel <= 0) return fail("ns_op_unpack_outputs: n_mel must be positive");
  PackedCtx pk;
  NS_TRY(packed_ctx("ns_op_unpack_outputs", plan_dev, B, T, Mp, att_wgs, &pk));
  NS_HIP(launch_unpack_outputs(pk.rm, B, T, n_mel, (const long long*)mel_lens, mel_p, post_p, p_p, e_p, mel_bias, post_const, mel, post, p_pred,
                               e_pred, mel_mask, (hipStream_t)stream));
  return 0;
}
```

### smart-nar_fast_tts_amd/csrc/kernels.h

```cpp
#pragma once
#include <hip/hip_runtime.h>
#include <stdint.h>

namespace ns {

enum Act : int { ACT_NONE = 0, ACT_RELU = 1, ACT_TANH = 2 };

struct RowMap {
  const int* row_b; const int* row_t; const int* row_w;
  const int* off; const int* win;
  const int* att_off; const int* att_order; int att_wgs;
  int rows;
};

enum RowEpi : int { EPI_NONE = 0, EPI_LN = 1, EPI_LN_PRED = 2 };
struct RowEpilogue {
  const float* ln_g; const float* ln_b;
  const long long* lens;
  const float* wlin; const float* blin; float* pred; float control; const float* target;
  const float* bins; int n_edges; const float* emb; const float* x_in; const float* pos; float* x_out; int D;
  float* y_out; int* ticket;
  const int* row_b; const int* row_t;
};
inline int conv_gemm_ticket_ints(int M) { return (M + 31) / 32; }
bool conv_gemm_ticket_ok(int M, int N, int Cin);

struct ConvGemm {
  const float* X; int ldx;
  const float* W;
  int ldw;
  const unsigned short* Wb3;
  const unsigned short* Wbf;
  const float* bias;
  const float* resid; int ldr;
  float* Y; int ldy;
  int M, N, Cin, KW, pad, S;
  int m_base;
  int act;
  int epi;
  RowEpilogue e;
  RowMap rm;
};
struct LaunchTiming { hipEvent_t start, stop; };
hipError_t launch_conv_gemm(const ConvGemm& p, hipStream_t st, const LaunchTiming* tm = nullptr);
bool conv_gemm_plan(int M, int N, int Cin, int KW, int out[8]);
int conv_gemm_describe(int M, int N, int Cin, int KW, int epi, int out[2][8]);
bool conv_gemm_tile16_enabled();
int conv_gemm_row_tile(int M, int N, int K = 256);
int conv_gemm_acc_chunk();
bool launch_planner_enabled();
bool conv_gemm_b3_ok(int M, int N, int Cin, int KW, int epi);
int conv_gemm_b3_tile(int M, int N);
hipError_t launch_conv_gemm_b3(const ConvGemm& p, hipStream_t st);
void split_weights_b3(const float* w, size_t n, unsigned short* hi, unsigned short* mid, unsigned short* lo);
bool conv_gemm_bf16_ok(int M, int N, int Cin, int KW, int epi);
void conv_gemm_bf16_plan(int M, int N, int* bm, int* bn);
hipError_t launch_conv_gemm_bf16(const ConvGemm& p, hipStream_t st);
size_t bf16_plane_elems(int N, int KW, int Cin);
void round_weights_bf16(const float* w, int N, int KW, int Cin, unsigned short* dst);
bool conv_gemm_row_epilogue_ok(int M, int N, int Cin);

constexpr int ATT_SPLIT_MAX = 16, ATT_SPLIT_MAX_BLOCKS = 128;
inline int attention_ticket_ints(int B, int S, int H) { return B * H * ((S + 31) / 32); }
bool attention_uses_tickets(int B, int S, int H);
hipError_t launch_attention(const float* qkv, const long long* lens, int B, int S, int H, int dk, float* out, float* scratch,
                            size_t scratch_floats, int* tickets, hipStream_t st, const RowMap* rm = nullptr, const LaunchTiming* tm = nullptr,
                            bool bf16 = false);
int attention_split(int B, int S, int H, int dk);
int attention_split_packed(int att_wgs, int S, int dk, size_t Mp, int d);
struct AttentionPackedPlan { int form, nsplit, merge, tiles; };
AttentionPackedPlan attention_plan_packed(int B, int S, int H, int dk, int att_wgs, size_t Mp, size_t scratch_floats, bool has_tickets);
struct AttentionDensePlan { int kernel, nsplit, merge, tiles; };
AttentionDensePlan attention_plan_dense(int B, int S, int H, int dk, size_t scratch_floats, bool has_tickets);

hipError_t launch_layernorm(const float* x, const float* g, const float* b, float* y, int M, int C, int S,
                            const long long* lens, hipStream_t st, const RowMap* rm = nullptr);
hipError_t launch_ln_linear_embed(const float* x, const float* g, const float* b, const float* wlin, const float* blin,
                                  float* pred, int M, int C, int S, const long long* lens, float control,
                                  const float* target, const float* bins, int n_bins, const float* emb, const float* x_in, const float* pos,
                                  float* x_out, int D, hipStream_t st, const RowMap* rm = nullptr);
hipError_t launch_embed_pos(const long long* texts, const float* emb, const float* pos, float* out, int M, int S, int D, int n_vocab,
                            int* zero, int nzero, hipStream_t st);
hipError_t launch_add_pos(const float* x, const float* pos, float* out, int M, int S, int D, hipStream_t st, const RowMap* rm = nullptr);
hipError_t launch_bucketize(const float* v, int n, const float* bins, int n_edges, long long* idx, hipStream_t st);
hipError_t launch_mask_from_lengths(const long long* lens, int B, int max_len, uint8_t* mask, hipStream_t st);
hipError_t launch_sinusoid(int n_pos, int d, float* out, hipStream_t st);
hipError_t launch_duration_round(const float* log_d, int n, float d_control, float* d_rounded, hipStream_t st);
hipError_t launch_duration_scan(const float* d_rounded, int B, int L, int32_t* cum, long long* mel_lens, hipStream_t st);
hipError_t launch_length_regulate(const float* x, const int32_t* cum, int B, int L, int D, int T, float* out, uint8_t* mel_mask,
                                  const long long* mel_lens, int32_t* status, int* zero, int nzero, hipStream_t st);
hipError_t launch_duration_tail(const float* log_d, const long long* src_lens, const long long* texts, int n_vocab, int B, int L,
                                float d_control, float* d_rounded, float* d_keep, int32_t* cum, long long* mel_lens, uint8_t* src_mask,
                                long long* mel_lens_host , hipStream_t st);
hipError_t launch_duration_target_tail(const long long* d_targets, const long long* src_lens, const long long* texts, int n_vocab, int B, int L,
                                       float* d_keep, int32_t* cum, long long* mel_lens, uint8_t* src_mask, hipStream_t st);
constexpr int PACK_GUARD = 20;
inline size_t pack_plan_ints(int B, size_t Mp) { return (size_t)4 * B + 4 + 3 * Mp; }
void plan_pointers(int* plan, int B, int Mp, RowMap* rm);
hipError_t launch_length_regulate_packed(const float* x, const int32_t* cum, int B, int L, int D, int T, int Mp, int H, float* out,
                                         const long long* mel_lens, int32_t* status, int* zero, int nzero, int* plan, RowMap* rm,
                                         hipStream_t st);
hipError_t launch_broadcast_row(const float* row, float* dst, int rows, int n, hipStream_t st);
hipError_t launch_pack_vector(const RowMap& rm, int T, const float* src, float* dst, int Mp, hipStream_t st);
hipError_t launch_pack_plan(const long long* mel_lens, int B, int T, int H, int Mp, int* plan, RowMap* rm, hipStream_t st, int guard = PACK_GUARD);
constexpr int PHONEME_GUARD = 2;
hipError_t launch_store_lens(const long long* host, int n, long long* dst, hipStream_t st);
hipError_t launch_pack_plan_only(const long long* lens, int B, int T, int H, int Mp, int* plan, RowMap* rm, hipStream_t st, int guard);
hipError_t launch_embed_pos_packed(const long long* texts, const float* emb, const float* pos, float* out, const RowMap& rm, int B, int Mp, int L,
                                   int D, int n_vocab, int* zero, int nzero, hipStream_t st);
hipError_t launch_unpack_phase1(const RowMap& rm, const long long* lens, int B, int S, int D, const float* rows_p, float* rows, const float* vec_p,
                                float* vec, hipStream_t st);
hipError_t launch_unpack_rows(const RowMap& rm, const long long* lens, int B, int S, int D, const float* src, float* dst, hipStream_t st);
hipError_t launch_unpack_outputs(const RowMap& rm, int B, int T, int n_mel, const long long* mel_lens, const float* mel_p, const float* post_p,
                                 const float* p_p, const float* e_p, const float* mel_bias, const float* post_const, float* mel,
                                 float* post, float* p_pred, float* e_pred, uint8_t* mel_mask, hipStream_t st);
hipError_t launch_gaussian_upsampling(const float* x, const float* dur, int B, int L, int D, int T, int T_out,
                                      float* out, float* s, float* w, const long long* own_len, int32_t* status, int* zero, int nzero,
                                      hipStream_t st, const RowMap* rm = nullptr);

struct VocGemm {
  const float* X; const float* W; const float* bias; const float* R; float* Y;
  int B, S_in, Sg, Cin, KW, dil, off0, N, Cb;
  long long out_ustride, out_shift;
  int in_act; float in_slope; int out_act; float out_slope;
  int mrf; float mrf_div;
  const unsigned short* Wbf;
};
bool voc_gemm_ok(const VocGemm& p);
hipError_t launch_voc_gemm(const VocGemm& p, hipStream_t st);
hipError_t launch_voc_gemm_bf16(const VocGemm& p, hipStream_t st);
size_t voc_post_lds_bytes(int C, int KW);
hipError_t launch_voc_post(const float* x, const float* w, const float* bias, float* wav, int B, int S, int C, int KW, float slope, hipStream_t st);
hipError_t launch_voc_transpose(const float* src, float* dst, int B, int C, int T, hipStream_t st);
bool cross_attention_ok(int H, int dk);
hipError_t launch_cross_attention(const float* q, const float* kv, const long long* src_lens, int B, int T, int L, int H, int dk,
                                  float* ctx, float* attn, hipStream_t st);
hipError_t launch_aln_input(const float* mels, float* x, int B, int T, int C, hipStream_t st);
hipError_t launch_aln_durations(const float* attn_last, const long long* src_lens, const long long* mel_lens, int B, int H, int T, int L,
                                long long* out, hipStream_t st);
struct LossArgs {
  int B, L, T, H, n_mel, pitch_frame_level, energy_frame_level;
  long long mel_targets_stride, d_targets_stride;
  const float *mel, *postnet, *mel_targets;
  const unsigned char* mel_masks;
  const float *pitch, *pitch_targets, *energy, *energy_targets;
  const float* log_d; const long long* d_targets; const unsigned char* src_masks;
  const long long *src_lens, *mel_lens;
  const float* attn[4];
};
constexpr int LOSS_FRAME_ROWS = 64;
constexpr int LOSS_PHONEME_ROWS = 1024;
constexpr int LOSS_ATTN_ROWS = 16;
constexpr int LOSS_SLOT_SUMS = 6, LOSS_SLOT_WORDS = 8, LOSS_SLOT_BYTES = 64;
long long loss_slots(int B, int L, int T, int* n_frame_wgs, int* n_phoneme_wgs);
// ... 141 lines not shown
```

### smart-nar_fast_tts_amd/csrc/rowln.h

```cpp
#pragma once
#include "kernels.h"

namespace ns {

typedef float f32x4 __attribute__((ext_vector_type(4)));

template <int CTRL>
__device__ __forceinline__ int dpp_i(int v) { return __builtin_amdgcn_update_dpp(0, v, CTRL, 0xF, 0xF, true); }
template <int CTRL>
__device__ __forceinline__ float dpp_f(float v) { return __builtin_bit_cast(float, dpp_i<CTRL>(__builtin_bit_cast(int, v))); }
constexpr int DPP_XOR1 = 0xB1, DPP_XOR2 = 0x4E, DPP_HALF_MIRROR = 0x141, DPP_MIRROR = 0x140, SWZ_XOR16 = 0x401F;

__device__ __forceinline__ float wave_sum(float v) {
  v += dpp_f<DPP_XOR1>(v);
  v += dpp_f<DPP_XOR2>(v);
  v += dpp_f<DPP_HALF_MIRROR>(v);
  v += dpp_f<DPP_MIRROR>(v);
  v += __builtin_bit_cast(float, __builtin_amdgcn_ds_swizzle(__builtin_bit_cast(int, v), SWZ_XOR16));
  const int iv = __builtin_bit_cast(int, v);
  return __builtin_bit_cast(float, __builtin_amdgcn_readlane(iv, 0)) + __builtin_bit_cast(float, __builtin_amdgcn_readlane(iv, 32));
}

__device__ __forceinline__ int wave_sum(int v) {
  v += dpp_i<DPP_XOR1>(v);
// ... 41 lines not shown
  const float var = wave_sum(q) / (float)C;
  rstd = 1.0f / sqrtf(var + LN_EPS);
}

template <int NV>
__device__ __forceinline__ void ln_store(const f32x4 (&v)[NV], int C, int lane, float mean, float rstd, const float* __restrict__ g,
                                         const float* __restrict__ bta, float* __restrict__ y) {
#pragma unroll
  for (int i = 0; i < NV; ++i) {
    const int c = lane * 4 + i * 256;
    if (c < C) {
      const f32x4 gg = *reinterpret_cast<const f32x4*>(g + c);
      const f32x4 bb = *reinterpret_cast<const f32x4*>(bta + c);
      f32x4 o;
#pragma unroll
      for (int e = 0; e < 4; ++e) o[e] = ln_affine(v[i][e], mean, rstd, gg[e], bb[e]);
      *reinterpret_cast<f32x4*>(y + c) = o;
    }
  }
}

__device__ __forceinline__ float keep_or_zero(float x, unsigned keep) { return __builtin_bit_cast(float, __builtin_bit_cast(unsigned, x) & keep); }

template <int NV>
__device__ __forceinline__ float predictor_row_value(const f32x4 (&v)[NV], int C, int lane, const RowEpilogue& e, int m, unsigned keep, bool store = true) {
#pragma clang fp contract(off)
  float mean, rstd;
  ln_moments<NV>(v, C, lane, mean, rstd);
  float dot = 0.f;
#pragma unroll
  for (int i = 0; i < NV; ++i) {
    const int c = lane * 4 + i * 256;
    if (c < C) {
      const f32x4 gg = *reinterpret_cast<const f32x4*>(e.ln_g + c);
      const f32x4 bb = *reinterpret_cast<const f32x4*>(e.ln_b + c);
      const f32x4 ww = *reinterpret_cast<const f32x4*>(e.wlin + c);
#pragma unroll
      for (int k = 0; k < 4; ++k) dot = __builtin_fmaf(ln_affine(v[i][k], mean, rstd, gg[k], bb[k]), ww[k], dot);
    }
  }
  float pv = wave_sum(dot) + e.blin[0];
  pv = keep_or_zero(pv, keep);
  if (e.target == nullptr) pv *= e.control;
  if (lane == 0 && store) e.pred[m] = pv;
  return pv;
}

template <int NV>
__device__ __forceinline__ void predictor_row_tail(const f32x4 (&v)[NV], int C, int lane, float , float , const RowEpilogue& e,
                                                   int m, int t, bool masked) {
  const float pv = predictor_row_value<NV>(v, C, lane, e, m, masked ? 0u : 0xFFFFFFFFu);
  if (e.emb == nullptr) return;
  const int cnt = wave_bucketize(e.bins, e.n_edges, e.target ? e.target[m] : pv, lane);
  const float* er = e.emb + (size_t)cnt * e.D;
  for (int c = lane * 4; c < e.D; c += 256) {
    f32x4 a = *reinterpret_cast<const f32x4*>(e.x_in + (size_t)m * e.D + c);
    const f32x4 e4 = *reinterpret_cast<const f32x4*>(er + c);
    a += e4;
    if (e.pos) a += *reinterpret_cast<const f32x4*>(e.pos + (size_t)t * e.D + c);
    *reinterpret_cast<f32x4*>(e.x_out + (size_t)m * e.D + c) = a;
  }
}

typedef unsigned u32x4r __attribute__((ext_vector_type(4)));

template <int NV, int R>
__device__ __forceinline__ void row_batch_finish(f32x4 (&v)[R][NV], const int (&tt)[R], const unsigned (&keep)[R], int lane, int epi, const RowEpilogue& e,
                                                 int M, int m_first, int m_step, const f32x4 (&lng)[NV], const f32x4 (&lnb)[NV]) {
  constexpr int C = NV * 256;
  if (epi == EPI_LN) {
#pragma unroll
    for (int j = 0; j < R; ++j) {
      float mean, rstd;
      ln_moments<NV>(v[j], C, lane, mean, rstd);
#pragma unroll
      for (int i = 0; i < NV; ++i)
#pragma unroll
        for (int k = 0; k < 4; ++k) v[j][i][k] = keep_or_zero(ln_affine(v[j][i][k], mean, rstd, lng[i][k], lnb[i][k]), keep[j]);
    }
#pragma unroll
    for (int j = 0; j < R; ++j) {
      const int m = m_first + j * m_step;
      if (m >= M) continue;
#pragma unroll
      for (int i = 0; i < NV; ++i) *reinterpret_cast<f32x4*>(e.y_out + (size_t)m * C + lane * 4 + i * 256) = v[j][i];
    }
    return;
  }
  int cnt[R];
#pragma unroll
  for (int j = 0; j < R; ++j) {
    const int m = m_first + j * m_step, mc = m < M ? m : M - 1;
    const float pv = predictor_row_value<NV>(v[j], C, lane, e, mc, keep[j], m < M);
    cnt[j] = e.emb ? wave_bucketize(e.bins, e.n_edges, e.target ? e.target[mc] : pv, lane) : 0;
  }
  if (e.emb == nullptr) return;
  for (int c0 = 0; c0 < e.D; c0 += 256) {
    const int c = c0 + lane * 4;
    if (c >= e.D) break;
    f32x4 a[R];
#pragma unroll
    for (int j = 0; j < R; ++j) {
      const int m = m_first + j * m_step, mc = m < M ? m : M - 1;
      a[j] = *reinterpret_cast<const f32x4*>(e.x_in + (size_t)mc * e.D + c);
      a[j] += *reinterpret_cast<const f32x4*>(e.emb + (size_t)cnt[j] * e.D + c);
      if (e.pos) a[j] += *reinterpret_cast<const f32x4*>(e.pos + (size_t)tt[j] * e.D + c);
    }
#pragma unroll
    for (int j = 0; j < R; ++j) {
      const int m = m_first + j * m_step;
      if (m < M) *reinterpret_cast<f32x4*>(e.x_out + (size_t)m * e.D + c) = a[j];
    }
  }
}

template <int R>
__device__ __forceinline__ void row_batch_masks(const RowEpilogue& e, int M, int S, int m_first, int m_step, int (&tt)[R], unsigned (&keep)[R]) {
  int bb_[R];
  long long ln[R];
#pragma unroll
  for (int j = 0; j < R; ++j) {
    const int m = m_first + j * m_step, mc = m < M ? m : M - 1;
    if (e.row_b) {
      bb_[j] = e.row_b[mc];
      tt[j] = e.row_t[mc];
    } else {
      bb_[j] = mc / S;
      tt[j] = mc - bb_[j] * S;
    }
  }
  if (e.lens) {
#pragma unroll
    for (int j = 0; j < R; ++j) ln[j] = e.lens[bb_[j]];
  } else {
#pragma unroll
    for (int j = 0; j < R; ++j) ln[j] = 0x7fffffffffffffffll;
  }
#pragma unroll
  for (int j = 0; j < R; ++j) {
    keep[j] = (long long)tt[j] >= ln[j] ? 0u : 0xFFFFFFFFu;
    asm("" : "+v"(keep[j]));
  }
}

template <int NV, int R>
__device__ __forceinline__ void row_epilogue_batch(__amdgpu_buffer_rsrc_t rs, int ldraw, int lane, int epi, const RowEpilogue& e, int M, int S,
                                                   int m_first, int m_step) {
// ... 22 lines not shown
```

### smart-nar_fast_tts_amd/csrc/rowops.hip

```cpp
#include "rowln.h"

namespace ns {

__device__ __forceinline__ void zero_words(int* __restrict__ z, int n) {
  if (!z) return;
  const int nthr = gridDim.x * gridDim.y * blockDim.x;
  for (int i = (blockIdx.y * gridDim.x + blockIdx.x) * blockDim.x + threadIdx.x; i < n; i += nthr) z[i] = 0;
}

template <int NV>
__device__ __forceinline__ void ln_stats(const float* x, int C, int lane, f32x4 (&v)[NV], float& mean, float& rstd) {
#pragma unroll
  for (int i = 0; i < NV; ++i) {
    const int c = lane * 4 + i * 256;
    if (c < C) v[i] = *reinterpret_cast<const f32x4*>(x + c);
    else v[i] = f32x4{0.f, 0.f, 0.f, 0.f};
  }
  ln_moments<NV>(v, C, lane, mean, rstd);
}

template <int NV>
__global__ __launch_bounds__(256) void k_layernorm(const float* __restrict__ x, const float* __restrict__ g,
                                                    const float* __restrict__ bta, float* __restrict__ y, int M, int C,
                                                    int S, const long long* __restrict__ lens, const int* __restrict__ row_b,
                                                    const int* __restrict__ row_t) {
  const int lane = threadIdx.x & 63;
  const int m = blockIdx.x * 4 + (threadIdx.x >> 6);
  if (m >= M) return;
  const int bb = row_b ? row_b[m] : m / S, tt = row_t ? row_t[m] : m % S;
  if (lens && (long long)tt >= lens[bb]) {
    for (int c = lane * 4; c < C; c += 256) *reinterpret_cast<f32x4*>(y + (size_t)m * C + c) = f32x4{0.f, 0.f, 0.f, 0.f};
    return;
  }
  f32x4 v[NV];
  float mean, rstd;
  ln_stats<NV>(x + (size_t)m * C, C, lane, v, mean, rstd);
  ln_store<NV>(v, C, lane, mean, rstd, g, bta, y + (size_t)m * C);
}

hipError_t launch_layernorm(const float* x, const float* g, const float* b, float* y, int M, int C, int S,
                            const long long* lens, hipStream_t st, const RowMap* rm) {
  if (M <= 0) return hipSuccess;
  if (C % 4 != 0 || C > 1024) return hipErrorInvalidValue;
  dim3 grid((M + 3) / 4), block(256);
  const int* rb = rm ? rm->row_b : nullptr;
  const int* rt = rm ? rm->row_t : nullptr;
  if (C <= 256) hipLaunchKernelGGL((k_layernorm<1>), grid, block, 0, st, x, g, b, y, M, C, S, lens, rb, rt);
  else if (C <= 512) hipLaunchKernelGGL((k_layernorm<2>), grid, block, 0, st, x, g, b, y, M, C, S, lens, rb, rt);
  else hipLaunchKernelGGL((k_layernorm<4>), grid, block, 0, st, x, g, b, y, M, C, S, lens, rb, rt);
  return hipGetLastError();
}

template <int NV>
__global__ __launch_bounds__(256) void k_ln_linear_embed(const float* __restrict__ x, const float* __restrict__ g,
                                                          const float* __restrict__ bta, const float* __restrict__ wlin,
                                                          const float* __restrict__ blin, float* __restrict__ pred, int M,
                                                          int C, int S, const long long* __restrict__ lens, float control,
                                                          const float* __restrict__ target,
                                                          const float* __restrict__ bins, int n_edges,
                                                          const float* __restrict__ emb, const float* __restrict__ x_in,
                                                          const float* __restrict__ pos, float* __restrict__ x_out, int D,
                                                          const int* __restrict__ row_b, const int* __restrict__ row_t) {
  const int lane = threadIdx.x & 63;
  const int m = blockIdx.x * 4 + (threadIdx.x >> 6);
  if (m >= M) return;
  f32x4 v[NV];
  float mean, rstd;
  ln_stats<NV>(x + (size_t)m * C, C, lane, v, mean, rstd);
  RowEpilogue e;
  e.y_out = nullptr; e.ticket = nullptr; e.row_b = nullptr; e.row_t = nullptr;
  e.ln_g = g; e.ln_b = bta; e.lens = lens; e.wlin = wlin; e.blin = blin; e.pred = pred; e.control = control; e.target = target;
  e.bins = bins; e.n_edges = n_edges; e.emb = emb; e.x_in = x_in; e.pos = pos; e.x_out = x_out; e.D = D;
  const int bb = row_b ? row_b[m] : m / S, t = row_t ? row_t[m] : m % S;
  predictor_row_tail<NV>(v, C, lane, mean, rstd, e, m, t, lens && (long long)t >= lens[bb]);
}

hipError_t launch_ln_linear_embed(const float* x, const float* g, const float* b, const float* wlin, const float* blin,
                                  float* pred, int M, int C, int S, const long long* lens, float control,
                                  const float* target, const float* bins, int n_bins, const float* emb, const float* x_in, const float* pos,
                                  float* x_out, int D, hipStream_t st, const RowMap* rm) {
  if (M <= 0) return hipSuccess;
  if (C % 4 != 0 || C > 1024 || (emb && D % 4 != 0)) return hipErrorInvalidValue;
  dim3 grid((M + 3) / 4), block(256);
  const int n_edges = n_bins - 1;
  const int* rb = rm ? rm->row_b : nullptr;
  const int* rt = rm ? rm->row_t : nullptr;
#define NS_ARGS x, g, b, wlin, blin, pred, M, C, S, lens, control, target, bins, n_edges, emb, x_in, pos, x_out, D, rb, rt
  if (C <= 256) hipLaunchKernelGGL((k_ln_linear_embed<1>), grid, block, 0, st, NS_ARGS);
  else if (C <= 512) hipLaunchKernelGGL((k_ln_linear_embed<2>), grid, block, 0, st, NS_ARGS);
  else hipLaunchKernelGGL((k_ln_linear_embed<4>), grid, block, 0, st, NS_ARGS);
#undef NS_ARGS
  return hipGetLastError();
}

__global__ __launch_bounds__(256) void k_bucketize(const float* __restrict__ v, int n, const float* __restrict__ bins,
                                                    int n_edges, long long* __restrict__ idx) {
  const int lane = threadIdx.x & 63;
  const int i = blockIdx.x * 4 + (threadIdx.x >> 6);
  if (i >= n) return;
  const int c = wave_bucketize(bins, n_edges, v[i], lane);
  if (lane == 0) idx[i] = c;
}
hipError_t launch_bucketize(const float* v, int n, const float* bins, int n_edges, long long* idx, hipStream_t st) {
  if (n <= 0) return hipSuccess;
  hipLaunchKernelGGL(k_bucketize, dim3((n + 3) / 4), dim3(256), 0, st, v, n, bins, n_edges, idx);
  return hipGetLastError();
}

__global__ __launch_bounds__(256) void k_embed_pos(const long long* __restrict__ texts, const float* __restrict__ emb,
                                                    const float* __restrict__ pos, float* __restrict__ out, int M, int S, int D,
                                                    int n_vocab, int* __restrict__ zero, int nzero) {
  zero_words(zero, nzero);
  const int lane = threadIdx.x & 63;
  const int m = blockIdx.x * 4 + (threadIdx.x >> 6);
  if (m >= M) return;
  long long tok = texts[m];
  if (tok < 0 || tok >= (long long)n_vocab) tok = 0;
  const int t = m % S;
  for (int c = lane * 4; c < D; c += 256) {
    f32x4 a = *reinterpret_cast<const f32x4*>(emb + (size_t)tok * D + c);
    a += *reinterpret_cast<const f32x4*>(pos + (size_t)t * D + c);
    *reinterpret_cast<f32x4*>(out + (size_t)m * D + c) = a;
  }
}
hipError_t launch_embed_pos(const long long* texts, const float* emb, const float* pos, float* out, int M, int S, int D, int n_vocab,
                            int* zero, int nzero, hipStream_t st) {
  if (M <= 0) return hipSuccess;
  hipLaunchKernelGGL(k_embed_pos, dim3((M + 3) / 4), dim3(256), 0, st, texts, emb, pos, out, M, S, D, n_vocab, zero, nzero);
  return hipGetLastError();
}

struct LensBlock { long long v[128]; };
__global__ void k_store_lens(LensBlock blk, int n, long long* __restrict__ dst) {
  const int i = threadIdx.x;
  if (i < n) dst[i] = blk.v[i];
}
hipError_t launch_store_lens(const long long* host, int n, long long* dst, hipStream_t st) {
  for (int o = 0; o < n; o += 128) {
    LensBlock blk;
    const int k = n - o < 128 ? n - o : 128;
// ... 185 lines not shown
    }
    int inc = v;
#pragma unroll
    for (int o = 1; o < 64; o <<= 1) {
      const int n = __shfl_up(inc, o);
      if (lane >= o) inc += n;
    }
    if (lane == 63) wsum[wid] = inc;
    __syncthreads();
    int off = carry_s;
    for (int w = 0; w < wid; ++w) off += wsum[w];
    if (l < L) cum[(size_t)b * L + l] = inc + off;
    __syncthreads();
    if (tid == 255) carry_s = inc + off;
    __syncthreads();
  }
  if (tid == 0) {
    const long long n = bad_s ? -1ll : (long long)carry_s;
    mel_lens[b] = n;
    if constexpr (MODE != SCAN_TARGET) {
      if (mel_lens_host) mel_lens_host[b] = n;
    }
  }
}
hipError_t launch_duration_scan(const float* d_rounded, int B, int L, int32_t* cum, long long* mel_lens, hipStream_t st) {
  if (B <= 0) return hipSuccess;
  hipLaunchKernelGGL((k_duration_scan<SCAN_COUNTS>), dim3(B), dim3(256), 0, st, d_rounded, L, cum, mel_lens, nullptr, 1.0f, nullptr, nullptr,
                     nullptr, nullptr, 0, nullptr);
  return hipGetLastError();
}
hipError_t launch_duration_tail(const float* log_d, const long long* src_lens, const long long* texts, int n_vocab, int B, int L,
                                float d_control, float* d_rounded, float* d_keep, int32_t* cum, long long* mel_lens, uint8_t* src_mask,
                                long long* mel_lens_host, hipStream_t st) {
  if (B <= 0) return hipSuccess;
  hipLaunchKernelGGL((k_duration_scan<SCAN_TAIL>), dim3(B), dim3(256), 0, st, log_d, L, cum, mel_lens, src_lens, d_control, d_rounded, d_keep,
                     src_mask, texts, n_vocab, mel_lens_host);
  return hipGetLastError();
}
hipError_t launch_duration_target_tail(const long long* d_targets, const long long* src_lens, const long long* texts, int n_vocab, int B, int L,
                                       float* d_keep, int32_t* cum, long long* mel_lens, uint8_t* src_mask, hipStream_t st) {
  if (B <= 0) return hipSuccess;
  hipLaunchKernelGGL((k_duration_scan<SCAN_TARGET>), dim3(B), dim3(256), 0, st, d_targets, L, cum, mel_lens, src_lens, 1.0f, nullptr, d_keep,
                     src_mask, texts, n_vocab, nullptr);
  return hipGetLastError();
}

__device__ __forceinline__ int32_t forward_status(long long total, int T, long long mel_len) {
  return (total > (long long)T ? 1 : 0) | (mel_len < 0 ? 2 : 0);
}

__global__ __launch_bounds__(256) void k_length_regulate(const float* __restrict__ x, const int32_t* __restrict__ cum, int L,
                                                          int D, int T, int M, float* __restrict__ out,
                                                          uint8_t* __restrict__ mel_mask, const long long* __restrict__ mel_lens,
                                                          int32_t* __restrict__ status, int* __restrict__ zero, int nzero) {
  zero_words(zero, nzero);
  const int lane = threadIdx.x & 63;
  const int m = blockIdx.x * 4 + (threadIdx.x >> 6);
  if (m >= M) return;
  const int b = m / T, t = m % T;
  const int32_t* cb = cum + (size_t)b * L;
  const int total = L > 0 ? cb[L - 1] : 0;
  if (mel_mask && lane == 0) mel_mask[m] = t >= total ? 1 : 0;
  if (status && t == 0 && lane == 0) status[b] = forward_status(total, T, mel_lens ? mel_lens[b] : 0ll);
  float* dst = out + (size_t)m * D;
  if (t >= total) {
    for (int c = lane * 4; c < D; c += 256) *reinterpret_cast<f32x4*>(dst + c) = f32x4{0.f, 0.f, 0.f, 0.f};
    return;
  }
  int lo = 0, hi = L - 1;
  while (lo < hi) {
    const int mid = (lo + hi) >> 1;
    if (cb[mid] > t) hi = mid;
    else lo = mid + 1;
  }
  const float* src = x + ((size_t)b * L + lo) * D;
  for (int c = lane * 4; c < D; c += 256) *reinterpret_cast<f32x4*>(dst + c) = *reinterpret_cast<const f32x4*>(src + c);
}
__global__ void k_status_only(const int32_t* __restrict__ cum, int L, int B, const long long* __restrict__ mel_lens,
                              int32_t* __restrict__ status) {
  const int b = blockIdx.x * blockDim.x + threadIdx.x;
  if (b < B) status[b] = forward_status(L > 0 ? cum[(size_t)b * L + L - 1] : 0, 0, mel_lens ? mel_lens[b] : 0ll);
}
hipError_t launch_length_regulate(const float* x, const int32_t* cum, int B, int L, int D, int T, float* out, uint8_t* mel_mask,
                                  const long long* mel_lens, int32_t* status, int* zero, int nzero, hipStream_t st) {
  const int M = B * T;
  if (M <= 0) {
    if (B > 0 && status) hipLaunchKernelGGL(k_status_only, dim3((B + 63) / 64), dim3(64), 0, st, cum, L, B, mel_lens, status);
    return hipGetLastError();
  }
  if (D % 4 != 0) return hipErrorInvalidValue;
  hipLaunchKernelGGL(k_length_regulate, dim3((M + 3) / 4), dim3(256), 0, st, x, cum, L, D, T, M, out, mel_mask, mel_lens, status, zero, nzero);
  return hipGetLastError();
}

__global__ __launch_bounds__(256) void k_pack_plan(const long long* __restrict__ mel_lens, int B, int T, int H, int* __restrict__ off,
                                                    int* __restrict__ win, int* __restrict__ att_off, int* __restrict__ att_order, int guard) {
  for (int b = threadIdx.x; b < B; b += blockDim.x) {
    long long l = mel_lens[b];
    if (l < 0) l = 0;
    l += guard;
    win[b] = (int)(l < (long long)T ? l : (long long)T);
  }
  __syncthreads();
  for (int b = threadIdx.x; b < B; b += blockDim.x) {
    const int w = win[b];
    int rank = 0;
    for (int o = 0; o < B; ++o) rank += (win[o] > w || (win[o] == w && o < b)) ? 1 : 0;
    att_order[rank] = b;
  }
  __syncthreads();
  if (threadIdx.x == 0) {
    int o = 0, a = 0;
    for (int b = 0; b < B; ++b) {
      off[b] = o;
      o += win[b];
      att_off[b] = a;
      a += ((win[att_order[b]] + 127) / 128) * H;
    }
    off[B] = o;
    att_off[B] = a;
  }
}

__global__ void k_pack_rows(const int* __restrict__ off, const int* __restrict__ win, int B, int Mp, int* __restrict__ row_b,
                            int* __restrict__ row_t, int* __restrict__ row_w) {
  const int m = blockIdx.x * blockDim.x + threadIdx.x;
  if (m >= Mp) return;
  int lo = 0, hi = B - 1;
  while (lo < hi) {
    const int mid = (lo + hi + 1) >> 1;
    if (off[mid] <= m) lo = mid;
    else hi = mid - 1;
  }
  row_b[m] = lo; row_t[m] = m - off[lo]; row_w[m] = win[lo];
}

void plan_pointers(int* plan, int B, int Mp, RowMap* rm) {
  int* off = plan;
  int* win = off + B + 1;
  int* att_off = win + B + 1;
  int* att_order = att_off + B + 1;
  int* row_b = att_order + B + 1;
  rm->off = off; rm->win = win; rm->att_off = att_off; rm->att_order = att_order;
  rm->row_b = row_b; rm->row_t = row_b + Mp; rm->row_w = row_b + 2 * (size_t)Mp;
}

hipError_t launch_pack_plan_only(const long long* lens, int B, int T, int H, int Mp, int* plan, RowMap* rm, hipStream_t st, int guard) {
  if (B <= 0 || Mp <= 0 || !plan || !rm || !lens) return hipErrorInvalidValue;
  plan_pointers(plan, B, Mp, rm);
  hipLaunchKernelGGL(k_pack_plan, dim3(1), dim3(256), 0, st, lens, B, T, H, const_cast<int*>(rm->off), const_cast<int*>(rm->win),
                     const_cast<int*>(rm->att_off), const_cast<int*>(rm->att_order), guard);
  return hipGetLastError();
}

hipError_t launch_pack_plan(const long long* mel_lens, int B, int T, int H, int Mp, int* plan, RowMap* rm, hipStream_t st, int guard) {
  if (B <= 0 || Mp <= 0 || !plan || !rm || !mel_lens) return hipErrorInvalidValue;
  plan_pointers(plan, B, Mp, rm);
  hipLaunchKernelGGL(k_pack_plan, dim3(1), dim3(256), 0, st, mel_lens, B, T, H, const_cast<int*>(rm->off), const_cast<int*>(rm->win),
                     const_cast<int*>(rm->att_off), const_cast<int*>(rm->att_order), guard);
  hipLaunchKernelGGL(k_pack_rows, dim3((Mp + 255) / 256), dim3(256), 0, st, rm->off, rm->win, B, Mp, const_cast<int*>(rm->row_b),
                     const_cast<int*>(rm->row_t), const_cast<int*>(rm->row_w));
  return hipGetLastError();
}

__global__ __launch_bounds__(256) void k_length_regulate_packed(const float* __restrict__ x, const int32_t* __restrict__ cum, int B, int L,
                                                                 int D, int T, int Mp, float* __restrict__ out,
                                                                 const long long* __restrict__ mel_lens, int32_t* __restrict__ status,
                                                                 const int* __restrict__ off, const int* __restrict__ win,
                                                                 int* __restrict__ row_b, int* __restrict__ row_t, int* __restrict__ row_w,
                                                                 int* __restrict__ zero, int nzero) {
  zero_words(zero, nzero);
  const int lane = threadIdx.x & 63;
  const int m = blockIdx.x * 4 + (threadIdx.x >> 6);
  if (m >= Mp) return;
  int lo = 0, hi = B - 1;
  while (lo < hi) {
    const int mid = (lo + hi + 1) >> 1;
    if (off[mid] <= m) lo = mid;
    else hi = mid - 1;
  }
  const int b = lo, t = m - off[b];
  if (lane == 0) { row_b[m] = b; row_t[m] = t; row_w[m] = win[b]; }
  const int32_t* cb = cum + (size_t)b * L;
  const int total = L > 0 ? cb[L - 1] : 0;
  if (status && t == 0 && lane == 0) status[b] = forward_status(total, T, mel_lens ? mel_lens[b] : 0ll);
  float* dst = out + (size_t)m * D;
  if (t >= total) {
    for (int c = lane * 4; c < D; c += 256) *reinterpret_cast<f32x4*>(dst + c) = f32x4{0.f, 0.f, 0.f, 0.f};
    return;
  }
  lo = 0; hi = L - 1;
  while (lo < hi) {
    const int mid = (lo + hi) >> 1;
    if (cb[mid] > t) hi = mid;
    else lo = mid + 1;
  }
  const float* src = x + ((size_t)b * L + lo) * D;
  for (int c = lane * 4; c < D; c += 256) *reinterpret_cast<f32x4*>(dst + c) = *reinterpret_cast<const f32x4*>(src + c);
}

hipError_t launch_length_regulate_packed(const float* x, const int32_t* cum, int B, int L, int D, int T, int Mp, int H, float* out,
                                         const long long* mel_lens, int32_t* status, int* zero, int nzero, int* plan, RowMap* rm,
                                         hipStream_t st) {
  if (B <= 0 || Mp <= 0 || D % 4 != 0 || !plan || !rm || !mel_lens) return hipErrorInvalidValue;
  plan_pointers(plan, B, Mp, rm);
  int* off = const_cast<int*>(rm->off);
  int* win = const_cast<int*>(rm->win);
  hipLaunchKernelGGL(k_pack_plan, dim3(1), dim3(256), 0, st, mel_lens, B, T, H, off, win, const_cast<int*>(rm->att_off),
                     const_cast<int*>(rm->att_order), PACK_GUARD);
  hipLaunchKernelGGL(k_length_regulate_packed, dim3((Mp + 3) / 4), dim3(256), 0, st, x, cum, B, L, D, T, Mp, out, mel_lens, status, off, win,
                     const_cast<int*>(rm->row_b), const_cast<int*>(rm->row_t), const_cast<int*>(rm->row_w), zero, nzero);
  return hipGetLastError();
}

__global__ void k_broadcast_row(const float* __restrict__ row, float* __restrict__ dst, int total, int n) {
  const int i = blockIdx.x * blockDim.x + threadIdx.x;
  if (i < total) dst[i] = row[i % n];
}
hipError_t launch_broadcast_row(const float* row, float* dst, int rows, int n, hipStream_t st) {
  if (rows <= 0 || n <= 0) return hipSuccess;
  hipLaunchKernelGGL(k_broadcast_row, dim3((rows * n + 255) / 256), dim3(256), 0, st, row, dst, rows * n, n);
  return hipGetLastError();
}

__global__ void k_pack_vector(const int* __restrict__ row_b, const int* __restrict__ row_t, int T, const float* __restrict__ src,
                              float* __restrict__ dst, int Mp) {
  const int m = blockIdx.x * blockDim.x + threadIdx.x;
  if (m < Mp) dst[m] = src[(size_t)row_b[m] * T + row_t[m]];
}
hipError_t launch_pack_vector(const RowMap& rm, int T, const float* src, float* dst, int Mp, hipStream_t st) {
  if (Mp <= 0) return hipSuccess;
  hipLaunchKernelGGL(k_pack_vector, dim3((Mp + 255) / 256), dim3(256), 0, st, rm.row_b, rm.row_t, T, src, dst, Mp);
  return hipGetLastError();
}

__global__ __launch_bounds__(256) void k_unpack_outputs(const int* __restrict__ off, const int* __restrict__ win, int B, int T, int n_mel,
                                                         const long long* __restrict__ mel_lens, const float* __restrict__ mel_p,
                                                         const float* __restrict__ post_p, const float* __restrict__ p_p,
                                                         const float* __restrict__ e_p, const float* __restrict__ mel_bias,
                                                         const float* __restrict__ post_const, float* __restrict__ mel,
                                                         float* __restrict__ post, float* __restrict__ p_pred, float* __restrict__ e_pred,
                                                         uint8_t* __restrict__ mel_mask) {
  const int lane = threadIdx.x & 63;
  const int m = blockIdx.x * 4 + (threadIdx.x >> 6);
  if (m >= B * T) return;
  const int b = m / T, t = m - b * T;
  const int w = win[b];
  long long len_ll = mel_lens[b];
  const int len = (int)(len_ll < 0 ? 0 : (len_ll < (long long)T ? len_ll : (long long)T));
  const size_t src = (size_t)off[b] + t;
  const bool in_win = t < w;
  if (lane == 0) {
    if (mel_mask) mel_mask[m] = t >= len ? 1 : 0;
    if (p_pred) p_pred[m] = in_win ? p_p[src] : 0.f;
    if (e_pred) e_pred[m] = in_win ? e_p[src] : 0.f;
  }
  const float* post_src;
  if (w == T || t < len + 10) post_src = post_p + src * n_mel;
  else if (t >= T - 10) post_src = post_const + (size_t)(1 + t - (T - 10)) * n_mel;
  else post_src = post_const;
  const float* mel_src = in_win ? mel_p + src * n_mel : mel_bias;
  for (int c = lane; c < n_mel; c += 64) {
    mel[(size_t)m * n_mel + c] = mel_src[c];
    post[(size_t)m * n_mel + c] = post_src[c];
// ... 123 lines not shown
```

### smart-nar_fast_tts_amd/ops.py

```python
from __future__ import annotations

import math

import torch

from . import _lib


def _ws(model, B, S):
    n = model._lib.ns_op_ws_bytes(model._h, B, S)
    return model._workspace("op", n)


def _st(t):
    return _lib.stream_ptr(t.device)


def mask_from_lengths(lens: torch.Tensor, max_len: int | None = None) -> torch.Tensor:
    lib = _lib.load()
    lens = lens.long().contiguous()
    if max_len is None:
        max_len = int(lens.max().item())
    out = torch.empty(lens.shape[0], max_len, dtype=torch.bool, device=lens.device)
    _lib.check(lib.ns_op_mask_from_lengths(_lib.ptr(lens), lens.shape[0], int(max_len), _lib.ptr(out), _st(lens)), "mask")
# ... 471 lines not shown
    out = torch.empty_like(x_p)
    _lib.check(lib.ns_op_add_pos_packed(_lib.ptr(x_p), _lib.ptr(pos), *p.args, x_p.shape[1], _lib.ptr(out), _st(x_p)), "add_pos_packed")
    return out


def pack_vector(src, p: PackedPlan):
    lib = _lib.load()
    assert src.shape == (p.B, p.S)
    src = src.contiguous().float()
    out = torch.empty(p.Mp, dtype=torch.float32, device=src.device)
    _lib.check(lib.ns_op_pack_vector(_lib.ptr(src), *p.args, _lib.ptr(out), _st(src)), "pack_vector")
    return out


def unpack_rows(src_p, lens, p: PackedPlan):
    lib = _lib.load()
    assert src_p.shape[0] == p.Mp
    src_p = src_p.contiguous()
    lens_t = lens.long().contiguous() if lens is not None else None
    D = src_p.shape[1]
    out = torch.full((p.B, p.S, D), float("nan"), dtype=torch.float32, device=src_p.device)
    _lib.check(lib.ns_op_unpack_rows(_lib.ptr(src_p), _lib.ptr(lens_t), *p.args, D, _lib.ptr(out), _st(src_p)), "unpack_rows")
    return out


def unpack_phase1(rows_p, vec_p, lens, p: PackedPlan):
    lib = _lib.load()
    assert rows_p.shape[0] == p.Mp == vec_p.shape[0]
    rows_p, vec_p, lens = rows_p.contiguous(), vec_p.contiguous(), lens.long().contiguous()
    D = rows_p.shape[1]
    rows = torch.full((p.B, p.S, D), float("nan"), dtype=torch.float32, device=rows_p.device)
    vec = torch.full((p.B, p.S), float("nan"), dtype=torch.float32, device=rows_p.device)
    _lib.check(lib.ns_op_unpack_phase1(_lib.ptr(rows_p), _lib.ptr(vec_p), _lib.ptr(lens), *p.args, D, _lib.ptr(rows), _lib.ptr(vec), _st(rows_p)),
               "unpack_phase1")
    return rows, vec


def unpack_outputs(p: PackedPlan, mel_lens, mel_p, post_p, p_p, e_p, mel_bias, post_const, mask: bool = True):
    lib = _lib.load()
    n_mel = mel_p.shape[1]
    assert mel_p.shape == post_p.shape == (p.Mp, n_mel) and mel_bias.shape == (n_mel,) and post_const.shape == (11, n_mel)
    dev = mel_p.device
    c = lambda t: None if t is None else t.contiguous()
    mel_lens, mel_p, post_p, p_p, e_p, mel_bias, post_const = mel_lens.long().contiguous(), c(mel_p), c(post_p), c(p_p), c(e_p), c(mel_bias), c(post_const)
    nan = lambda *s: torch.full(s, float("nan"), dtype=torch.float32, device=dev)
    mel, post = nan(p.B, p.S, n_mel), nan(p.B, p.S, n_mel)
    pp = nan(p.B, p.S) if p_p is not None else None
    ep = nan(p.B, p.S) if e_p is not None else None
    mm = torch.full((p.B, p.S), 255, dtype=torch.uint8, device=dev) if mask else None
    _lib.check(lib.ns_op_unpack_outputs(*p.args, n_mel, _lib.ptr(mel_lens), _lib.ptr(mel_p), _lib.ptr(post_p), _lib.ptr(p_p), _lib.ptr(e_p),
                                        _lib.ptr(mel_bias), _lib.ptr(post_const), _lib.ptr(mel), _lib.ptr(post), _lib.ptr(pp), _lib.ptr(ep),
                                        _lib.ptr(mm), _st(mel_p)), "unpack_outputs")
    return mel, post, pp, ep, mm
```

Before: 2.936 million.

## Precompute phoneme-level projections and gather them per frame at decoder entry

Exploits linearity: pitch/energy predictor first convs and the first decoder QKV projection are applied to phoneme-level encoder outputs (and to embedding and positional tables) before length regulation. Per-frame inputs are then built by gathering and summing the precomputed rows with compensated summation, fused with bias, ReLU and LayerNorm. This avoids running those GEMMs at frame level (T rows) and runs them at phoneme level (L rows) instead. It adds arena tables, an extra phoneme-level GEMM, per-frame index/bucket buffers, and some numerical differences from reordered summation.

```diff
diff --git a/include/nar_fs2.h b/include/nar_fs2.h
--- a/include/nar_fs2.h
+++ b/include/nar_fs2.h
@@ -149,6 +149,18 @@
 int ns_op_unpack_outputs(const int32_t* plan_dev, int B, int T, int Mp, int att_wgs, int n_mel, const int64_t* mel_lens, const float* mel_p,
                          const float* post_p, const float* p_p, const float* e_p, const float* mel_bias, const float* post_const, float* mel,
                          float* post, float* p_pred, float* e_pred, uint8_t* mel_mask, void* stream);
+
+int ns_entry_width(const ns_model* m);
+int ns_entry_consumers(const ns_model* m, int B, int L);
+int ns_op_entry_products(ns_model* m, const float* enc_out, int B, int L, float* yh, void* stream);
+int ns_op_entry_length_regulate(const float* x, const int32_t* cum, const int64_t* mel_lens , int B, int L, int D, int T, int Mp,
+                                int H, float* out, int32_t* pidx, uint8_t* mel_mask ,
+                                int32_t* plan_dev, size_t plan_ints, void* stream);
+int ns_op_entry_predictor_tail(ns_model* m, const char* prefix, const float* h, const int64_t* lens, int B, int S, float control,
+                               const float* target , const float* x_in, int add_pos, float* pred, float* x_out, int32_t* bucket,
+                               void* ws, size_t ws_bytes, void* stream);
+int ns_op_entry_gather(ns_model* m, int which, const float* yh, const int32_t* pidx, const int32_t* bkt_p, const int32_t* bkt_e,
+                       const int32_t* plan_dev, int B, int L, int S, int Mp, int att_wgs, float* out, void* stream);
 
 #define NS_PROFILE_SLOTS 3
 #define NS_PROFILE_OFF 0
diff --git a/smart-nar_fast_tts_amd/_lib.py b/smart-nar_fast_tts_amd/_lib.py
--- a/smart-nar_fast_tts_amd/_lib.py
+++ b/smart-nar_fast_tts_amd/_lib.py
@@ -204,6 +204,12 @@
     "ns_op_unpack_rows": (_I, [_P, _P, _P, _I, _I, _I, _I, _I, _P, _P]),
     "ns_op_unpack_phase1": (_I, [_P, _P, _P, _P, _I, _I, _I, _I, _I, _P, _P, _P]),
     "ns_op_unpack_outputs": (_I, [_P, _I, _I, _I, _I, _I, _P, _P, _P, _P, _P, _P, _P, _P, _P, _P, _P, _P, _P]),
+    "ns_entry_width": (_I, [_P]),
+    "ns_entry_consumers": (_I, [_P, _I, _I]),
+    "ns_op_entry_products": (_I, [_P, _P, _I, _I, _P, _P]),
+    "ns_op_entry_length_regulate": (_I, [_P, _P, _P, _I, _I, _I, _I, _I, _I, _P, _P, _P, _P, _Z, _P]),
+    "ns_op_entry_predictor_tail": (_I, [_P, _S, _P, _P, _I, _I, _F, _P, _P, _I, _P, _P, _P, _P, _Z, _P]),
+    "ns_op_entry_gather": (_I, [_P, _I, _P, _P, _P, _P, _P, _I, _I, _I, _I, _I, _P, _P]),
     "ns_profile_enable": (_I, [_P, _I]),
     "ns_profile_read": (_I, [_P, C.POINTER(C.c_double), C.POINTER(C.c_double), C.POINTER(C.c_int64)]),
     "ns_profile_read_slot": (_I, [_P, _I, C.POINTER(C.c_double), C.POINTER(C.c_double), C.POINTER(C.c_int64)]),
diff --git a/smart-nar_fast_tts_amd/csrc/api.hip b/smart-nar_fast_tts_amd/csrc/api.hip
--- a/smart-nar_fast_tts_amd/csrc/api.hip
+++ b/smart-nar_fast_tts_amd/csrc/api.hip
@@ -25,6 +25,10 @@
   size_t pn_in, pn_hid, pn_const;
   size_t pos_long;
   std::vector<ConvW> post;
+  struct EntryW { bool planned = false; size_t wcat = 0, pe_e = 0, pe_q = 0, ee_q = 0, pos_q = 0, pos_q_long = 0; } entry;
+  unsigned entry_cols_bits = 0;
+  unsigned entry_bits = 0;
+  size_t entry_min_rows = 0;
   Arena ar;
   float* arena = nullptr;
   bool ready = false;
@@ -49,7 +53,7 @@
 static const char* kPredNames[3] = {"duration", "pitch", "energy"};
 
 constexpr uint32_t ARENA_MAGIC = 0x3246534eu;
-constexpr uint32_t ARENA_LAYOUT_VERSION = 6;
+constexpr uint32_t ARENA_LAYOUT_VERSION = 7;
 constexpr int ARENA_HDR_WORDS = 16;
 static void arena_header(const ns_model* m, uint32_t* w) {
   memset(w, 0, ARENA_HDR_WORDS * sizeof(uint32_t));
@@ -65,6 +69,9 @@
   w[6] = 1;
 }
 constexpr int POS_LONG_ROWS = 8192;
+constexpr int ENTRY_POS_LONG_ROWS = 4096;
+constexpr size_t ENTRY_MIN_ROWS_DEFAULT = 0;
+constexpr unsigned ENTRY_BITS_DEFAULT = 5u;
 constexpr int PN_CONST_ROWS = 32;
 
 static void expect(ns_model* m, const std::string& name, std::vector<int64_t> shape, bool optional = false) {
@@ -192,6 +199,23 @@
   m->pn_hid = m->ar.take((size_t)2 * PN_CONST_ROWS * c.postnet_dim);
   m->pn_const = m->ar.take((size_t)PN_CONST_ROWS * c.n_mel);
   m->pos_long = m->ar.take((size_t)POS_LONG_ROWS * c.d_dec);
+  if (c.length_regulator == 0 && c.pitch_frame_level && c.energy_frame_level && c.n_dec_layer > 0 && 3 * d <= 1536 && F <= 1024) {
+    ns_model::EntryW& e = m->entry;
+    const size_t nq = 3 * (size_t)d, nf = (size_t)K * F;
+    e.planned = true;
+    e.wcat = m->ar.take((2 * nf + nq) * d);
+    e.pe_e = m->ar.take((size_t)c.n_bins * nf);
+    e.pe_q = m->ar.take((size_t)c.n_bins * nq);
+    e.ee_q = m->ar.take((size_t)c.n_bins * nq);
+    e.pos_q = m->ar.take((size_t)npos * nq);
+    e.pos_q_long = m->ar.take((size_t)ENTRY_POS_LONG_ROWS * nq);
+    const char* eb = getenv("NS_ENTRY_GATHER");
+    m->entry_bits = eb ? ((unsigned)atoi(eb) & 7u) : ENTRY_BITS_DEFAULT;
+    m->entry_cols_bits = m->entry_bits;
+    if (c.matmul_bf16x3 == 2) m->entry_bits &= 3u;
+    const char* er = getenv("NS_ENTRY_MIN_ROWS");
+    m->entry_min_rows = er && atoll(er) >= 0 ? (size_t)atoll(er) : ENTRY_MIN_ROWS_DEFAULT;
+  }
   *out = m;
   return 0;
 }
@@ -246,6 +270,46 @@
 }
 
 static int postnet_constants(ns_model* m, hipStream_t st);
+
+static int entry_col(const ns_model* m, int which) {
+  const int nf = m->cfg.vp_kernel * m->cfg.vp_filter, nq = 3 * m->cfg.d_dec;
+  return which == 0 ? 0 : which == 2 ? nf : nf + nq;
+}
+static int entry_cols(const ns_model* m, unsigned bits, int* lo) {
+  const int nf = m->cfg.vp_kernel * m->cfg.vp_filter, nq = 3 * m->cfg.d_dec;
+  const int first = (bits & 1u) ? 0 : (bits & 4u) ? nf : nf + nq;
+  const int end = (bits & 2u) ? 2 * nf + nq : (bits & 4u) ? nf + nq : nf;
+  *lo = first;
+  return bits ? end - first : 0;
+}
+static int entry_width(const ns_model* m) { return m->entry.planned ? 2 * m->cfg.vp_kernel * m->cfg.vp_filter + 3 * m->cfg.d_dec : 0; }
+static int entry_gemm(const ns_model* m, const float* X, int M, size_t w_row, int N, float* Y, hipStream_t st, int ldy = 0) {
+  const int d = m->cfg.d_dec;
+  ConvGemm p;
+  memset(&p, 0, sizeof(p));
+  p.X = X; p.ldx = d; p.W = m->P(m->entry.wcat) + w_row * d; p.Y = Y; p.ldy = ldy ? ldy : N;
+  p.M = M; p.N = N; p.Cin = d; p.KW = 1; p.S = M; p.act = ACT_NONE; p.epi = EPI_NONE;
+  NS_HIP(launch_conv_gemm(p, st));
+  return 0;
+}
+static int entry_tables(ns_model* m, hipStream_t st) {
+  if (!m->entry.planned) return 0;
+  const ns_config& c = m->cfg;
+  const ns_model::EntryW& e = m->entry;
+  const int nf = c.vp_kernel * c.vp_filter, nq = 3 * c.d_dec;
+  const size_t we = (size_t)entry_col(m, 1), wq = (size_t)entry_col(m, 2);
+  NS_TRY(entry_gemm(m, m->P(m->pitch_emb), c.n_bins, we, nf, m->arena + e.pe_e, st));
+  NS_TRY(entry_gemm(m, m->P(m->pitch_emb), c.n_bins, wq, nq, m->arena + e.pe_q, st));
+  NS_TRY(entry_gemm(m, m->P(m->energy_emb), c.n_bins, wq, nq, m->arena + e.ee_q, st));
+  NS_TRY(entry_gemm(m, m->P(m->dec_pos), c.max_seq_len + 1, wq, nq, m->arena + e.pos_q, st));
+  NS_TRY(entry_gemm(m, m->P(m->pos_long), ENTRY_POS_LONG_ROWS, wq, nq, m->arena + e.pos_q_long, st));
+  return 0;
+}
+static void entry_repack_taps(const float* w, int F, int k, int d, float* dst) {
+  for (int o = 0; o < F; ++o)
+    for (int j = 0; j < k; ++j) memcpy(dst + ((size_t)j * F + o) * d, w + ((size_t)o * k + j) * d, (size_t)d * sizeof(float));
+}
+
 extern "C" int ns_finalize_weights(ns_model* m, void* stream) {
   if (!m) return fail("ns_finalize_weights: null model");
   if (!m->arena) return fail("ns_finalize_weights: bind an arena first (ns_bind_arena)");
@@ -299,6 +363,13 @@
   cp(m->pitch_emb, "variance_adaptor.pitch_embedding.weight"); cp(m->energy_emb, "variance_adaptor.energy_embedding.weight");
   cp(m->mel_linear.w, "mel_linear.weight"); cp(m->mel_linear.b, "mel_linear.bias");
   fill_planes(img.data(), m->mel_linear);
+  if (m->entry.planned) {
+    const int F = c.vp_filter, k = c.vp_kernel, d = c.d_dec;
+    float* wc = &img[m->entry.wcat];
+    entry_repack_taps(&img[m->pred[1].c1.w], F, k, d, wc + (size_t)entry_col(m, 0) * d);
+    entry_repack_taps(&img[m->pred[2].c1.w], F, k, d, wc + (size_t)entry_col(m, 1) * d);
+    memcpy(wc + (size_t)entry_col(m, 2) * d, &img[m->dec[0].qkv.w], (size_t)3 * d * d * sizeof(float));
+  }
 
   for (size_t i = 0; i < m->post.size(); ++i) {
     const ConvW& w = m->post[i];
@@ -317,6 +388,8 @@
   NS_HIP(hipMemcpyAsync(m->arena, img.data(), img.size() * sizeof(float), hipMemcpyHostToDevice, st));
   NS_TRY(postnet_constants(m, st));
   NS_HIP(launch_sinusoid(POS_LONG_ROWS, c.d_dec, m->arena + m->pos_long, st));
+  static_assert(ENTRY_POS_LONG_ROWS <= POS_LONG_ROWS, "pos_q_long is taken from the regenerated table's rows");
+  NS_TRY(entry_tables(m, st));
   NS_HIP(hipStreamSynchronize(st));
   m->weights.release();
   m->ready = true;
@@ -331,6 +404,7 @@
   float *xa, *xb, *qkv, *att, *t1, *x1, *hid, *vp1, *vp2, *pos_ext, *att_part;
   size_t att_part_floats;
   Tickets tk;
+  int *pidx, *bkt_p, *bkt_e;
 };
 
 static size_t imax(size_t a, size_t b) { return a > b ? a : b; }
@@ -356,8 +430,14 @@
   s.tk.base = (int*)bp.raw(TICKET_INTS * sizeof(int));
   if (c.row_epilogue == 1) s.tk.base = nullptr;
   s.tk.used = 0;
+  s.pidx = (int*)bp.raw(M * sizeof(int)); s.bkt_p = (int*)bp.raw(M * sizeof(int)); s.bkt_e = (int*)bp.raw(M * sizeof(int));
   return s;
 }
+}
+
+static unsigned entry_consumers(const ns_model* m, int B, int L) {
+  if (!m->entry.planned || !m->entry_bits || (size_t)B * L < m->entry_min_rows) return 0u;
+  return m->entry_bits;
 }
 
 extern "C" size_t ns_op_ws_bytes(const ns_model* m, int B, int S) {
@@ -373,6 +453,7 @@
   bp.f((size_t)B * L * m->cfg.d_enc);
   bp.raw((size_t)B * L * sizeof(int32_t));
   bp.f((size_t)B * L);
+  if (entry_consumers(m, B, L)) bp.f((size_t)B * L * entry_width(m));
   carve(m->cfg, bp, (size_t)B * L, L);
   return bp.off + phase1_packed_extra_bytes(m->cfg, B, L) + 256;
 }
@@ -495,10 +576,10 @@
 };
 
 static int mha(ns_model* m, const LayerW& L, int d, int H, const float* x, const long long* lens, int B, int S,
-               float* out, bool mask_rows, Scratch& sc, hipStream_t st) {
+               float* out, bool mask_rows, Scratch& sc, hipStream_t st, bool qkv_ready = false) {
   const int M = rows_of(sc, B, S);
   const bool bf = L.qkv.bf != NO_PLANE;
-  NS_TRY(gemm(m, sc, L.qkv, x, nullptr, sc.qkv, M, S, ACT_NONE, st));
+  if (!qkv_ready) NS_TRY(gemm(m, sc, L.qkv, x, nullptr, sc.qkv, M, S, ACT_NONE, st));
   {
     ProfScope ps(m, 1, 4.0 * (double)M * (double)S * (double)d);
     NS_TRY(ps.begin());
@@ -524,8 +605,8 @@
 }
 
 static int fft_block(ns_model* m, const LayerW& L, int d, int H, const float* x, const long long* lens, int B, int S,
-                     float* out, Scratch& sc, hipStream_t st) {
-  NS_TRY(mha(m, L, d, H, x, lens, B, S, sc.x1, true, sc, st));
+                     float* out, Scratch& sc, hipStream_t st, bool qkv_ready = false) {
+  NS_TRY(mha(m, L, d, H, x, lens, B, S, sc.x1, true, sc, st, qkv_ready));
   NS_TRY(ffn(m, L, d, sc.x1, lens, B, S, out, true, sc, st));
   return 0;
 }
@@ -548,20 +629,20 @@
 }
 static int predictor_tail(const ns_model* m, const PredW& w, const float* h, const long long* lens, int B, int S, float control,
                           const float* target, float* pred, const float* bins, const float* emb, const float* x_in, const float* pos,
-                          float* x_out, Scratch& sc, hipStream_t st) {
+                          float* x_out, Scratch& sc, hipStream_t st, int* bucket = nullptr) {
   const ns_config& c = m->cfg;
   const int M = rows_of(sc, B, S), F = c.vp_filter, D = w.c1.cin;
   RowEpilogue e;
   memset(&e, 0, sizeof(e));
   e.ln_g = m->P(w.ln2_g); e.ln_b = m->P(w.ln2_b); e.lens = lens; e.wlin = m->P(w.lin_w); e.blin = m->P(w.lin_b); e.pred = pred;
   e.control = control; e.target = target; e.bins = bins; e.n_edges = c.n_bins - 1; e.emb = emb; e.x_in = x_in; e.pos = pos; e.x_out = x_out;
-  e.D = D;
+  e.D = D; e.bucket = emb ? bucket : nullptr;
   if (fuse_row_epilogue(M, F, F)) return gemm(m, sc, w.c2, h, nullptr, nullptr, M, S, ACT_RELU, st, GemmOpts::row(e, EPI_LN_PRED));
   if (conv_gemm_ticket_ok(M, F, F) && (e.ticket = sc.tk.take(conv_gemm_ticket_ints(M))) != nullptr)
     return gemm(m, sc, w.c2, h, nullptr, sc.vp1, M, S, ACT_RELU, st, GemmOpts::row(e, EPI_LN_PRED));
   NS_TRY(gemm(m, sc, w.c2, h, nullptr, sc.vp1, M, S, ACT_RELU, st));
   NS_HIP(launch_ln_linear_embed(sc.vp1, m->P(w.ln2_g), m->P(w.ln2_b), m->P(w.lin_w), m->P(w.lin_b), pred, M, F, S, lens,
-                                control, target, bins, c.n_bins, emb, x_in, pos, x_out, D, st, cur_rm(sc)));
+                                control, target, bins, c.n_bins, emb, x_in, pos, x_out, D, st, cur_rm(sc), e.bucket));
   return 0;
 }
 static int predictor(const ns_model* m, const PredW& w, const float* x, const long long* lens, int B, int S, float control,
@@ -570,6 +651,35 @@
                      hipStream_t st) {
   NS_TRY(predictor_conv1(m, w, x, B, S, sc.vp2, sc, st));
   return predictor_tail(m, w, sc.vp2, lens, B, S, control, target, pred, bins, emb, x, pos, x_out, sc, st);
+}
+
+static int entry_gather(const ns_model* m, int which, const float* yh, int enc_rows, const int* pidx, const int* bkt_p, const int* bkt_e,
+                        const float* pos_q, int pos_rows, const RowMap* rm, int M, int S, float* out, hipStream_t st) {
+  const ns_config& c = m->cfg;
+  const ns_model::EntryW& e = m->entry;
+  const int F = c.vp_filter, k = c.vp_kernel, nf = k * F, nq = 3 * c.d_dec, NC = entry_width(m);
+  EntryGather g;
+  memset(&g, 0, sizeof(g));
+  g.M = M; g.S = S; g.out = out;
+  if (rm) { g.row_t = rm->row_t; g.row_w = rm->row_w; }
+  int n = 0;
+  auto add = [&](const float* tab, int ld, int rows, const int* idx, int shift) { g.src[n++] = EntrySrc{tab, idx, ld, shift, rows}; };
+  if (which < 2) {
+    const PredW& w = m->pred[1 + which];
+    g.C = F; g.bias = m->P(w.c1.b); g.ln_g = m->P(w.ln1_g); g.ln_b = m->P(w.ln1_b);
+    for (int j = 0; j < k; ++j) add(yh + entry_col(m, which) + (size_t)j * F, NC, enc_rows, pidx, j - (k - 1) / 2);
+    if (which == 1)
+      for (int j = 0; j < k; ++j) add(m->P(e.pe_e) + (size_t)j * F, nf, c.n_bins, bkt_p, j - (k - 1) / 2);
+  } else {
+    g.C = nq; g.bias = m->P(m->dec[0].qkv.b);
+    add(yh + entry_col(m, 2), NC, enc_rows, pidx, 0);
+    add(m->P(e.pe_q), nq, c.n_bins, bkt_p, 0);
+    add(m->P(e.ee_q), nq, c.n_bins, bkt_e, 0);
+    add(pos_q, nq, pos_rows, nullptr, 0);
+  }
+  g.nsrc = n;
+  NS_HIP(launch_entry_gather(g, st));
+  return 0;
 }
 
 static int postnet(ns_model* m, const float* mel, int B, int T, const float* resid, float* out, Scratch& sc, hipStream_t st) {
@@ -619,13 +729,13 @@
   return 0;
 }
 
-static int decoder_stack(ns_model* m, float* x, const long long* lens, int B, int T, float* out, Scratch& sc, hipStream_t st) {
+static int decoder_stack(ns_model* m, float* x, const long long* lens, int B, int T, float* out, Scratch& sc, hipStream_t st, bool qkv0_ready = false) {
   const ns_config& c = m->cfg;
   float* cur = x;
   float* alt = (x == sc.xa) ? sc.xb : sc.xa;
   for (size_t i = 0; i < m->dec.size(); ++i) {
     float* dst = (i + 1 == m->dec.size()) ? out : alt;
-    NS_TRY(fft_block(m, m->dec[i], c.d_dec, c.n_dec_head, cur, lens, B, T, dst, sc, st));
+    NS_TRY(fft_block(m, m->dec[i], c.d_dec, c.n_dec_head, cur, lens, B, T, dst, sc, st, qkv0_ready && i == 0));
     if (dst != out) { alt = cur; cur = dst; }
   }
   if (m->dec.empty() && out != x) NS_HIP(hipMemcpyAsync(out, x, (size_t)rows_of(sc, B, T) * c.d_dec * 4, hipMemcpyDeviceToDevice, st));
@@ -684,6 +794,7 @@
   float* enc_out = bp.f((size_t)B * L * c.d_enc);
   int32_t* cum = (int32_t*)bp.raw((size_t)B * L * sizeof(int32_t));
   float* dur_keep = bp.f((size_t)B * L);
+  float* yh = entry_consumers(m, B, L) ? bp.f((size_t)B * L * entry_width(m)) : nullptr;
   const long long* lens = (const long long*)src_lens;
   size_t Mp = 0;
   bool packed = lens_host && !m->enc.empty() && launch_planner_enabled() && c.pitch_frame_level && c.energy_frame_level && c.phase1_packing != 2;
@@ -738,10 +849,15 @@
   if (tf) {
     NS_HIP(launch_duration_target_tail((const long long*)tf->d_targets, lens, (const long long*)texts, c.n_vocab, B, L, dur_keep, cum,
                                        (long long*)mel_lens, src_mask, st));
-    return 0;
-  }
-  NS_HIP(launch_duration_tail(log_d, lens, (const long long*)texts, c.n_vocab, B, L, d_control, d_rounded, dur_keep, cum,
-                              (long long*)mel_lens, src_mask, (long long*)mel_lens_host, st));
+  } else {
+    NS_HIP(launch_duration_tail(log_d, lens, (const long long*)texts, c.n_vocab, B, L, d_control, d_rounded, dur_keep, cum,
+                                (long long*)mel_lens, src_mask, (long long*)mel_lens_host, st));
+  }
+  if (yh) {
+    int lo = 0;
+    const int n = entry_cols(m, m->entry_cols_bits, &lo);
+    NS_TRY(entry_gemm(m, enc_out, B * L, (size_t)lo, n, yh + lo, st, entry_width(m)));
+  }
   return 0;
 }
 
@@ -818,6 +934,12 @@
   const float* enc_out = be.f((size_t)B * L * c.d_enc);
   const int32_t* cum = (const int32_t*)be.raw((size_t)B * L * sizeof(int32_t));
   const float* dur_keep = be.f((size_t)B * L);
+  unsigned ebits = entry_consumers(m, B, L);
+  const float* yh = ebits ? be.f((size_t)B * L * entry_width(m)) : nullptr;
+  const float* pos_q = nullptr;
+  if (T <= c.max_seq_len) pos_q = m->P(m->entry.pos_q);
+  else if (T <= ENTRY_POS_LONG_ROWS) pos_q = m->P(m->entry.pos_q_long);
+  else ebits &= ~4u;
   const long long* lens = (const long long*)mel_lens;
   const int d = c.d_dec;
   size_t Mp = 0;
@@ -830,6 +952,7 @@
   const size_t Mrows = packed ? Mp : (size_t)B * T;
   const int M = (int)Mrows;
   m->last_rows = (long long)Mrows;
+  if (c.matmul_bf16x3 == 1 && conv_gemm_b3_ok(M, 3 * d, d, 1, EPI_NONE)) ebits &= ~4u;
   Bump bp(ws_dec);
   Scratch sc = carve(c, bp, Mrows, T, packed);
   if (packed) {
@@ -859,7 +982,8 @@
       NS_HIP(launch_pack_plan(lens, B, T, c.n_dec_head, M, plan, &pk.rm, st));
       NS_HIP(launch_gaussian_upsampling(enc_out, dur_keep, B, L, c.d_enc, T, T, sc.xa, sc.vp2, nullptr, lens, status, sc.tk.base, TICKET_INTS, st, &pk.rm));
     } else {
-      NS_HIP(launch_length_regulate_packed(enc_out, cum, B, L, c.d_enc, T, M, c.n_dec_head, sc.xa, lens, status, sc.tk.base, TICKET_INTS, plan, &pk.rm, st));
+      NS_HIP(launch_length_regulate_packed(enc_out, cum, B, L, c.d_enc, T, M, c.n_dec_head, sc.xa, lens, status, sc.tk.base, TICKET_INTS, plan, &pk.rm, st,
+                                           ebits ? sc.pidx : nullptr));
     }
     pk.rm.att_wgs = window_att_wgs(lens_host, B, T, PACK_GUARD, c.n_dec_head);
     if (p_targets && c.pitch_frame_level) { NS_HIP(launch_pack_vector(pk.rm, T, p_targets, pt_p, M, st)); p_targets = pt_p; }
@@ -869,7 +993,8 @@
     if ((size_t)B * (L + 1) > (size_t)M * c.vp_filter) return fail("ns_forward_mel: workspace too small for the Gaussian centres");
     NS_HIP(launch_gaussian_upsampling(enc_out, dur_keep, B, L, c.d_enc, T, T, sc.xa, sc.vp2, nullptr, lens, status, sc.tk.base, TICKET_INTS, st));
   } else {
-    NS_HIP(launch_length_regulate(enc_out, cum, B, L, c.d_enc, T, sc.xa, mel_mask, lens, status, sc.tk.base, TICKET_INTS, st));
+    NS_HIP(launch_length_regulate(enc_out, cum, B, L, c.d_enc, T, sc.xa, mel_mask, lens, status, sc.tk.base, TICKET_INTS, st,
+                                  ebits ? sc.pidx : nullptr));
   }
   sc.pk = packed ? &pk : nullptr;
   float* const mel_dst = packed ? mel_p : mel;
@@ -882,14 +1007,18 @@
   float* alt = sc.xb;
   if (c.pitch_frame_level) {
     if (!p_pred) return fail("ns_forward_mel: frame_level pitch needs a p_pred [B,T] output");
-    NS_TRY(predictor(m, m->pred[1], cur, lens, B, T, p_control, p_targets, pp_dst, m->P(m->pitch_bins), m->P(m->pitch_emb),
-                     c.energy_frame_level ? nullptr : pos, alt, sc, st));
+    if (ebits & 1u) NS_TRY(entry_gather(m, 0, yh, B * L, sc.pidx, nullptr, nullptr, nullptr, 0, cur_rm(sc), M, T, sc.vp2, st));
+    else NS_TRY(predictor_conv1(m, m->pred[1], cur, B, T, sc.vp2, sc, st));
+    NS_TRY(predictor_tail(m, m->pred[1], sc.vp2, lens, B, T, p_control, p_targets, pp_dst, m->P(m->pitch_bins), m->P(m->pitch_emb), cur,
+                          c.energy_frame_level ? nullptr : pos, alt, sc, st, (ebits & 6u) ? sc.bkt_p : nullptr));
     float* t = cur; cur = alt; alt = t;
   }
   if (c.energy_frame_level) {
     if (!e_pred) return fail("ns_forward_mel: frame_level energy needs an e_pred [B,T] output");
-    NS_TRY(predictor(m, m->pred[2], cur, lens, B, T, e_control, e_targets, ep_dst, m->P(m->energy_bins), m->P(m->energy_emb), pos,
-                     alt, sc, st));
+    if (ebits & 2u) NS_TRY(entry_gather(m, 1, yh, B * L, sc.pidx, sc.bkt_p, nullptr, nullptr, 0, cur_rm(sc), M, T, sc.vp2, st));
+    else NS_TRY(predictor_conv1(m, m->pred[2], cur, B, T, sc.vp2, sc, st));
+    NS_TRY(predictor_tail(m, m->pred[2], sc.vp2, lens, B, T, e_control, e_targets, ep_dst, m->P(m->energy_bins), m->P(m->energy_emb), cur, pos,
+                          alt, sc, st, (ebits & 4u) ? sc.bkt_e : nullptr));
     float* t = cur; cur = alt; alt = t;
   }
   if (!c.pitch_frame_level && !c.energy_frame_level) {
@@ -897,7 +1026,9 @@
     float* t = cur; cur = alt; alt = t;
   }
   m->prof_active = m->prof != 0;
-  int rc = decoder_stack(m, cur, lens, B, T, sc.att, sc, st);
+  int rc = 0;
+  if (ebits & 4u) rc = entry_gather(m, 2, yh, B * L, sc.pidx, sc.bkt_p, sc.bkt_e, pos_q, T, cur_rm(sc), M, T, sc.qkv, st);
+  if (!rc) rc = decoder_stack(m, cur, lens, B, T, sc.att, sc, st, (ebits & 4u) != 0);
   if (!rc) rc = gemm(m, sc, m->mel_linear, sc.att, nullptr, mel_dst, M, T, ACT_NONE, st);
   if (!rc) rc = postnet(m, mel_dst, B, T, mel_dst, post_dst, sc, st);
   m->prof_active = false;
@@ -1043,9 +1174,9 @@
   NS_OP_PROLOGUE(B, S);
   return predictor_conv1(m, m->pred[i], x, B, S, h, sc, st);
 }
-extern "C" int ns_op_predictor_tail(ns_model* m, const char* prefix, const float* h, const int64_t* lens, int B, int S, float control,
-                                    const float* target, const float* x_in, int add_pos, float* pred, float* x_out, void* ws,
-                                    size_t ws_bytes, void* stream) {
+static int op_predictor_tail(ns_model* m, const char* prefix, const float* h, const int64_t* lens, int B, int S, float control,
+                             const float* target, const float* x_in, int add_pos, float* pred, float* x_out, void* ws,
+                             size_t ws_bytes, void* stream, int* bucket) {
   if (!m) return fail("null model");
   int i;
   NS_TRY(find_pred(prefix, &i));
@@ -1061,7 +1192,12 @@
     emb = m->P(i == 2 ? m->energy_emb : m->pitch_emb);
     if (add_pos) NS_TRY(position_rows(m, m->dec_pos, S, w.c1.cin, sc, &pos, st));
   }
-  return predictor_tail(m, w, h, (const long long*)lens, B, S, control, target, pred, bins, emb, x_in, pos, x_out, sc, st);
+  return predictor_tail(m, w, h, (const long long*)lens, B, S, control, target, pred, bins, emb, x_in, pos, x_out, sc, st, bucket);
+}
+extern "C" int ns_op_predictor_tail(ns_model* m, const char* prefix, const float* h, const int64_t* lens, int B, int S, float control,
+                                    const float* target, const float* x_in, int add_pos, float* pred, float* x_out, void* ws,
+                                    size_t ws_bytes, void* stream) {
+  return op_predictor_tail(m, prefix, h, lens, B, S, control, target, x_in, add_pos, pred, x_out, ws, ws_bytes, stream, nullptr);
 }
 extern "C" int ns_plan_gemm(int M, int N, int Cin, int KW, int32_t out[8]) {
   int o[8] = {0, 0, 0, 0, 0, 0, 0, 0};
@@ -1439,3 +1575,56 @@
                                e_pred, mel_mask, (hipStream_t)stream));
   return 0;
 }
+
+extern "C" int ns_entry_width(const ns_model* m) { return m ? entry_width(m) : 0; }
+extern "C" int ns_entry_consumers(const ns_model* m, int B, int L) { return (m && B > 0 && L > 0) ? (int)entry_consumers(m, B, L) : 0; }
+extern "C" int ns_op_entry_products(ns_model* m, const float* enc_out, int B, int L, float* yh, void* stream) {
+  NS_TRY(check_ready(m));
+  if (!m->entry.planned) return fail("ns_op_entry_products: this configuration has no entry products (ns_entry_width is 0)");
+  if (!enc_out || !yh) return fail("ns_op_entry_products: null argument");
+  if (B <= 0 || L <= 0 || (size_t)B * L >= ((size_t)1 << 30)) return fail("ns_op_entry_products: bad shape");
+  return entry_gemm(m, enc_out, B * L, 0, entry_width(m), yh, (hipStream_t)stream);
+}
+extern "C" int ns_op_entry_length_regulate(const float* x, const int32_t* cum, const int64_t* mel_lens, int B, int L, int D, int T, int Mp, int H,
+                                           float* out, int32_t* pidx, uint8_t* mel_mask, int32_t* plan_dev, size_t plan_ints, void* stream) {
+  if (!x || !cum || !out || !pidx) return fail("ns_op_entry_length_regulate: null argument");
+  if (mel_mask && Mp != 0) return fail("ns_op_entry_length_regulate: the mel mask is a [B, T] grid output (packed rows: ns_op_unpack_outputs writes it)");
+  if (B <= 0 || L <= 0 || T <= 0 || D <= 0 || D % 4 != 0 || (size_t)B * T >= ((size_t)1 << 30)) return fail("ns_op_entry_length_regulate: bad shape");
+  if (Mp == 0) {
+    if (plan_dev) return fail("ns_op_entry_length_regulate: a plan without packed rows");
+    NS_HIP(launch_length_regulate(x, cum, B, L, D, T, out, mel_mask, nullptr, nullptr, nullptr, 0, (hipStream_t)stream, (int*)pidx));
+    return 0;
+  }
+  if (!mel_lens || !plan_dev || H <= 0 || Mp < 0 || (size_t)Mp > (size_t)B * T) return fail("ns_op_entry_length_regulate: bad packed shape");
+  if (plan_ints < pack_plan_ints(B, (size_t)Mp)) return fail("ns_op_entry_length_regulate: plan buffer smaller than pack_plan_ints(B, Mp)");
+  RowMap rm;
+  memset(&rm, 0, sizeof(rm));
+  NS_HIP(launch_length_regulate_packed(x, cum, B, L, D, T, Mp, H, out, (const long long*)mel_lens, nullptr, nullptr, 0, (int*)plan_dev, &rm,
+                                       (hipStream_t)stream, (int*)pidx));
+  return 0;
+}
+extern "C" int ns_op_entry_predictor_tail(ns_model* m, const char* prefix, const float* h, const int64_t* lens, int B, int S, float control,
+                                          const float* target, const float* x_in, int add_pos, float* pred, float* x_out, int32_t* bucket, void* ws,
+                                          size_t ws_bytes, void* stream) {
+  if (!bucket || !x_in) return fail("ns_op_entry_predictor_tail: bucket and x_in are required");
+  return op_predictor_tail(m, prefix, h, lens, B, S, control, target, x_in, add_pos, pred, x_out, ws, ws_bytes, stream, (int*)bucket);
+}
+extern "C" int ns_op_entry_gather(ns_model* m, int which, const float* yh, const int32_t* pidx, const int32_t* bkt_p, const int32_t* bkt_e,
+                                  const int32_t* plan_dev, int B, int L, int S, int Mp, int att_wgs, float* out, void* stream) {
+  NS_TRY(check_ready(m));
+  if (!m->entry.planned) return fail("ns_op_entry_gather: this configuration has no entry products (ns_entry_width is 0)");
+  if (which < 0 || which > 2) return fail("ns_op_entry_gather: which must be 0 (pitch conv1), 1 (energy conv1) or 2 (qkv of decoder layer 0)");
+  if (!yh || !pidx || !out || (which >= 1 && !bkt_p) || (which == 2 && !bkt_e)) return fail("ns_op_entry_gather: null argument");
+  if (B <= 0 || L <= 0 || S <= 0 || (size_t)B * S >= ((size_t)1 << 30) || (size_t)B * L >= ((size_t)1 << 30)) return fail("ns_op_entry_gather: bad shape");
+  const float* pos_q = nullptr;
+  if (which == 2) {
+    if (S <= m->cfg.max_seq_len) pos_q = m->P(m->entry.pos_q);
+    else if (S <= ENTRY_POS_LONG_ROWS) pos_q = m->P(m->entry.pos_q_long);
+    else return fail("ns_op_entry_gather: more frames than position rows were taken through the QKV weight (the forwards run the GEMM)");
+  }
+  PackedCtx pk;
+  if (plan_dev) NS_TRY(packed_ctx("ns_op_entry_gather", plan_dev, B, S, Mp, att_wgs, &pk));
+  else if (Mp != 0 || att_wgs != 0) return fail("ns_op_entry_gather: Mp / att_wgs without a plan");
+  return entry_gather(m, which, yh, B * L, (const int*)pidx, (const int*)bkt_p, (const int*)bkt_e, pos_q, S, plan_dev ? &pk.rm : nullptr,
+                      plan_dev ? Mp : B * S, S, out, (hipStream_t)stream);
+}
diff --git a/smart-nar_fast_tts_amd/csrc/kernels.h b/smart-nar_fast_tts_amd/csrc/kernels.h
--- a/smart-nar_fast_tts_amd/csrc/kernels.h
+++ b/smart-nar_fast_tts_amd/csrc/kernels.h
@@ -21,6 +21,7 @@
   const float* bins; int n_edges; const float* emb; const float* x_in; const float* pos; float* x_out; int D;
   float* y_out; int* ticket;
   const int* row_b; const int* row_t;
+  int* bucket;
 };
 inline int conv_gemm_ticket_ints(int M) { return (M + 31) / 32; }
 bool conv_gemm_ticket_ok(int M, int N, int Cin);
@@ -78,7 +79,7 @@
 hipError_t launch_ln_linear_embed(const float* x, const float* g, const float* b, const float* wlin, const float* blin,
                                   float* pred, int M, int C, int S, const long long* lens, float control,
                                   const float* target, const float* bins, int n_bins, const float* emb, const float* x_in, const float* pos,
-                                  float* x_out, int D, hipStream_t st, const RowMap* rm = nullptr);
+                                  float* x_out, int D, hipStream_t st, const RowMap* rm = nullptr, int* bucket = nullptr);
 hipError_t launch_embed_pos(const long long* texts, const float* emb, const float* pos, float* out, int M, int S, int D, int n_vocab,
                             int* zero, int nzero, hipStream_t st);
 hipError_t launch_add_pos(const float* x, const float* pos, float* out, int M, int S, int D, hipStream_t st, const RowMap* rm = nullptr);
@@ -88,7 +89,7 @@
 hipError_t launch_duration_round(const float* log_d, int n, float d_control, float* d_rounded, hipStream_t st);
 hipError_t launch_duration_scan(const float* d_rounded, int B, int L, int32_t* cum, long long* mel_lens, hipStream_t st);
 hipError_t launch_length_regulate(const float* x, const int32_t* cum, int B, int L, int D, int T, float* out, uint8_t* mel_mask,
-                                  const long long* mel_lens, int32_t* status, int* zero, int nzero, hipStream_t st);
+                                  const long long* mel_lens, int32_t* status, int* zero, int nzero, hipStream_t st, int* pidx = nullptr);
 hipError_t launch_duration_tail(const float* log_d, const long long* src_lens, const long long* texts, int n_vocab, int B, int L,
                                 float d_control, float* d_rounded, float* d_keep, int32_t* cum, long long* mel_lens, uint8_t* src_mask,
                                 long long* mel_lens_host , hipStream_t st);
@@ -99,7 +100,18 @@
 void plan_pointers(int* plan, int B, int Mp, RowMap* rm);
 hipError_t launch_length_regulate_packed(const float* x, const int32_t* cum, int B, int L, int D, int T, int Mp, int H, float* out,
                                          const long long* mel_lens, int32_t* status, int* zero, int nzero, int* plan, RowMap* rm,
-                                         hipStream_t st);
+                                         hipStream_t st, int* pidx = nullptr);
+constexpr int ENTRY_MAX_SRC = 6;
+struct EntrySrc { const float* tab; const int* idx; int ld; int shift; int rows; };
+struct EntryGather {
+  EntrySrc src[ENTRY_MAX_SRC]; int nsrc;
+  const float* bias;
+  int C, M, S;
+  const int* row_t; const int* row_w;
+  const float* ln_g; const float* ln_b;
+  float* out;
+};
+hipError_t launch_entry_gather(const EntryGather& g, hipStream_t st);
 hipError_t launch_broadcast_row(const float* row, float* dst, int rows, int n, hipStream_t st);
 hipError_t launch_pack_vector(const RowMap& rm, int T, const float* src, float* dst, int Mp, hipStream_t st);
 hipError_t launch_pack_plan(const long long* mel_lens, int B, int T, int H, int Mp, int* plan, RowMap* rm, hipStream_t st, int guard = PACK_GUARD);
diff --git a/smart-nar_fast_tts_amd/csrc/rowln.h b/smart-nar_fast_tts_amd/csrc/rowln.h
--- a/smart-nar_fast_tts_amd/csrc/rowln.h
+++ b/smart-nar_fast_tts_amd/csrc/rowln.h
@@ -117,6 +117,7 @@
   const float pv = predictor_row_value<NV>(v, C, lane, e, m, masked ? 0u : 0xFFFFFFFFu);
   if (e.emb == nullptr) return;
   const int cnt = wave_bucketize(e.bins, e.n_edges, e.target ? e.target[m] : pv, lane);
+  if (e.bucket && lane == 0) e.bucket[m] = cnt;
   const float* er = e.emb + (size_t)cnt * e.D;
   for (int c = lane * 4; c < e.D; c += 256) {
     f32x4 a = *reinterpret_cast<const f32x4*>(e.x_in + (size_t)m * e.D + c);
@@ -158,6 +159,7 @@
     const int m = m_first + j * m_step, mc = m < M ? m : M - 1;
     const float pv = predictor_row_value<NV>(v[j], C, lane, e, mc, keep[j], m < M);
     cnt[j] = e.emb ? wave_bucketize(e.bins, e.n_edges, e.target ? e.target[mc] : pv, lane) : 0;
+    if (e.emb && e.bucket && lane == 0 && m < M) e.bucket[m] = cnt[j];
   }
   if (e.emb == nullptr) return;
   for (int c0 = 0; c0 < e.D; c0 += 256) {
diff --git a/smart-nar_fast_tts_amd/csrc/rowops.hip b/smart-nar_fast_tts_amd/csrc/rowops.hip
--- a/smart-nar_fast_tts_amd/csrc/rowops.hip
+++ b/smart-nar_fast_tts_amd/csrc/rowops.hip
@@ -60,7 +60,8 @@
                                                           const float* __restrict__ bins, int n_edges,
                                                           const float* __restrict__ emb, const float* __restrict__ x_in,
                                                           const float* __restrict__ pos, float* __restrict__ x_out, int D,
-                                                          const int* __restrict__ row_b, const int* __restrict__ row_t) {
+                                                          const int* __restrict__ row_b, const int* __restrict__ row_t,
+                                                          int* __restrict__ bucket) {
   const int lane = threadIdx.x & 63;
   const int m = blockIdx.x * 4 + (threadIdx.x >> 6);
   if (m >= M) return;
@@ -69,6 +70,7 @@
   ln_stats<NV>(x + (size_t)m * C, C, lane, v, mean, rstd);
   RowEpilogue e;
   e.y_out = nullptr; e.ticket = nullptr; e.row_b = nullptr; e.row_t = nullptr;
+  e.bucket = bucket;
   e.ln_g = g; e.ln_b = bta; e.lens = lens; e.wlin = wlin; e.blin = blin; e.pred = pred; e.control = control; e.target = target;
   e.bins = bins; e.n_edges = n_edges; e.emb = emb; e.x_in = x_in; e.pos = pos; e.x_out = x_out; e.D = D;
   const int bb = row_b ? row_b[m] : m / S, t = row_t ? row_t[m] : m % S;
@@ -78,14 +80,14 @@
 hipError_t launch_ln_linear_embed(const float* x, const float* g, const float* b, const float* wlin, const float* blin,
                                   float* pred, int M, int C, int S, const long long* lens, float control,
                                   const float* target, const float* bins, int n_bins, const float* emb, const float* x_in, const float* pos,
-                                  float* x_out, int D, hipStream_t st, const RowMap* rm) {
+                                  float* x_out, int D, hipStream_t st, const RowMap* rm, int* bucket) {
   if (M <= 0) return hipSuccess;
   if (C % 4 != 0 || C > 1024 || (emb && D % 4 != 0)) return hipErrorInvalidValue;
   dim3 grid((M + 3) / 4), block(256);
   const int n_edges = n_bins - 1;
   const int* rb = rm ? rm->row_b : nullptr;
   const int* rt = rm ? rm->row_t : nullptr;
-#define NS_ARGS x, g, b, wlin, blin, pred, M, C, S, lens, control, target, bins, n_edges, emb, x_in, pos, x_out, D, rb, rt
+#define NS_ARGS x, g, b, wlin, blin, pred, M, C, S, lens, control, target, bins, n_edges, emb, x_in, pos, x_out, D, rb, rt, bucket
   if (C <= 256) hipLaunchKernelGGL((k_ln_linear_embed<1>), grid, block, 0, st, NS_ARGS);
   else if (C <= 512) hipLaunchKernelGGL((k_ln_linear_embed<2>), grid, block, 0, st, NS_ARGS);
   else hipLaunchKernelGGL((k_ln_linear_embed<4>), grid, block, 0, st, NS_ARGS);
@@ -377,7 +379,8 @@
 __global__ __launch_bounds__(256) void k_length_regulate(const float* __restrict__ x, const int32_t* __restrict__ cum, int L,
                                                           int D, int T, int M, float* __restrict__ out,
                                                           uint8_t* __restrict__ mel_mask, const long long* __restrict__ mel_lens,
-                                                          int32_t* __restrict__ status, int* __restrict__ zero, int nzero) {
+                                                          int32_t* __restrict__ status, int* __restrict__ zero, int nzero,
+                                                          int* __restrict__ pidx) {
   zero_words(zero, nzero);
   const int lane = threadIdx.x & 63;
   const int m = blockIdx.x * 4 + (threadIdx.x >> 6);
@@ -389,6 +392,7 @@
   if (status && t == 0 && lane == 0) status[b] = forward_status(total, T, mel_lens ? mel_lens[b] : 0ll);
   float* dst = out + (size_t)m * D;
   if (t >= total) {
+    if (pidx && lane == 0) pidx[m] = -1;
     for (int c = lane * 4; c < D; c += 256) *reinterpret_cast<f32x4*>(dst + c) = f32x4{0.f, 0.f, 0.f, 0.f};
     return;
   }
@@ -398,6 +402,7 @@
     if (cb[mid] > t) hi = mid;
     else lo = mid + 1;
   }
+  if (pidx && lane == 0) pidx[m] = b * L + lo;
   const float* src = x + ((size_t)b * L + lo) * D;
   for (int c = lane * 4; c < D; c += 256) *reinterpret_cast<f32x4*>(dst + c) = *reinterpret_cast<const f32x4*>(src + c);
 }
@@ -407,14 +412,14 @@
   if (b < B) status[b] = forward_status(L > 0 ? cum[(size_t)b * L + L - 1] : 0, 0, mel_lens ? mel_lens[b] : 0ll);
 }
 hipError_t launch_length_regulate(const float* x, const int32_t* cum, int B, int L, int D, int T, float* out, uint8_t* mel_mask,
-                                  const long long* mel_lens, int32_t* status, int* zero, int nzero, hipStream_t st) {
+                                  const long long* mel_lens, int32_t* status, int* zero, int nzero, hipStream_t st, int* pidx) {
   const int M = B * T;
   if (M <= 0) {
     if (B > 0 && status) hipLaunchKernelGGL(k_status_only, dim3((B + 63) / 64), dim3(64), 0, st, cum, L, B, mel_lens, status);
     return hipGetLastError();
   }
   if (D % 4 != 0) return hipErrorInvalidValue;
-  hipLaunchKernelGGL(k_length_regulate, dim3((M + 3) / 4), dim3(256), 0, st, x, cum, L, D, T, M, out, mel_mask, mel_lens, status, zero, nzero);
+  hipLaunchKernelGGL(k_length_regulate, dim3((M + 3) / 4), dim3(256), 0, st, x, cum, L, D, T, M, out, mel_mask, mel_lens, status, zero, nzero, pidx);
   return hipGetLastError();
 }
 
@@ -493,7 +498,7 @@
                                                                  const long long* __restrict__ mel_lens, int32_t* __restrict__ status,
                                                                  const int* __restrict__ off, const int* __restrict__ win,
                                                                  int* __restrict__ row_b, int* __restrict__ row_t, int* __restrict__ row_w,
-                                                                 int* __restrict__ zero, int nzero) {
+                                                                 int* __restrict__ zero, int nzero, int* __restrict__ pidx) {
   zero_words(zero, nzero);
   const int lane = threadIdx.x & 63;
   const int m = blockIdx.x * 4 + (threadIdx.x >> 6);
@@ -511,6 +516,7 @@
   if (status && t == 0 && lane == 0) status[b] = forward_status(total, T, mel_lens ? mel_lens[b] : 0ll);
   float* dst = out + (size_t)m * D;
   if (t >= total) {
+    if (pidx && lane == 0) pidx[m] = -1;
     for (int c = lane * 4; c < D; c += 256) *reinterpret_cast<f32x4*>(dst + c) = f32x4{0.f, 0.f, 0.f, 0.f};
     return;
   }
@@ -520,13 +526,14 @@
     if (cb[mid] > t) hi = mid;
     else lo = mid + 1;
   }
+  if (pidx && lane == 0) pidx[m] = b * L + lo;
   const float* src = x + ((size_t)b * L + lo) * D;
   for (int c = lane * 4; c < D; c += 256) *reinterpret_cast<f32x4*>(dst + c) = *reinterpret_cast<const f32x4*>(src + c);
 }
 
 hipError_t launch_length_regulate_packed(const float* x, const int32_t* cum, int B, int L, int D, int T, int Mp, int H, float* out,
                                          const long long* mel_lens, int32_t* status, int* zero, int nzero, int* plan, RowMap* rm,
-                                         hipStream_t st) {
+                                         hipStream_t st, int* pidx) {
   if (B <= 0 || Mp <= 0 || D % 4 != 0 || !plan || !rm || !mel_lens) return hipErrorInvalidValue;
   plan_pointers(plan, B, Mp, rm);
   int* off = const_cast<int*>(rm->off);
@@ -534,7 +541,97 @@
   hipLaunchKernelGGL(k_pack_plan, dim3(1), dim3(256), 0, st, mel_lens, B, T, H, off, win, const_cast<int*>(rm->att_off),
                      const_cast<int*>(rm->att_order), PACK_GUARD);
   hipLaunchKernelGGL(k_length_regulate_packed, dim3((Mp + 3) / 4), dim3(256), 0, st, x, cum, B, L, D, T, Mp, out, mel_lens, status, off, win,
-                     const_cast<int*>(rm->row_b), const_cast<int*>(rm->row_t), const_cast<int*>(rm->row_w), zero, nzero);
+                     const_cast<int*>(rm->row_b), const_cast<int*>(rm->row_t), const_cast<int*>(rm->row_w), zero, nzero, pidx);
+  return hipGetLastError();
+}
+
+__device__ __forceinline__ void entry_two_sum(float& hi, float& lo, float y) {
+#pragma clang fp contract(off)
+  const float s = hi + y;
+  const float t = s - hi;
+  lo += (hi - (s - t)) + (y - t);
+  hi = s;
+}
+
+template <int NV, int NS>
+__global__ __launch_bounds__(256) void k_entry_gather(EntryGather g) {
+  const int lane = threadIdx.x & 63;
+  const int m = blockIdx.x * 4 + __builtin_amdgcn_readfirstlane(threadIdx.x >> 6);
+  if (m >= g.M) return;
+  const int t = g.row_t ? g.row_t[m] : m % g.S, w = g.row_w ? g.row_w[m] : g.S;
+  const float* row[NS];
+  unsigned keep[NS];
+#pragma unroll
+  for (int s = 0; s < NS; ++s) {
+    const EntrySrc& e = g.src[s];
+    const int tt = t + e.shift;
+    const bool in = tt >= 0 && tt < w;
+    const int r = !in ? -1 : e.idx ? e.idx[m + e.shift] : tt;
+    const bool ok = r >= 0 && r < e.rows;
+    keep[s] = ok ? 0xFFFFFFFFu : 0u;
+    row[s] = e.tab + (size_t)(ok ? r : 0) * e.ld;
+  }
+  f32x4 x[NS][NV];
+#pragma unroll
+  for (int s = 0; s < NS; ++s)
+#pragma unroll
+    for (int i = 0; i < NV; ++i) {
+      const int c = lane * 4 + i * 256;
+      x[s][i] = c < g.C ? *reinterpret_cast<const f32x4*>(row[s] + c) : f32x4{0.f, 0.f, 0.f, 0.f};
+    }
+  f32x4 v[NV];
+#pragma unroll
+  for (int i = 0; i < NV; ++i) {
+    const int c = lane * 4 + i * 256;
+    const f32x4 bias = c < g.C ? *reinterpret_cast<const f32x4*>(g.bias + c) : f32x4{0.f, 0.f, 0.f, 0.f};
+    f32x4 a;
+#pragma unroll
+    for (int k = 0; k < 4; ++k) {
+      float hi = 0.f, lo = 0.f;
+#pragma unroll
+      for (int s = 0; s < NS; ++s) entry_two_sum(hi, lo, keep_or_zero(x[s][i][k], keep[s]));
+      entry_two_sum(hi, lo, bias[k]);
+      a[k] = hi + lo;
+    }
+    if (g.ln_g) {
+#pragma unroll
+      for (int k = 0; k < 4; ++k) a[k] = a[k] > 0.f ? a[k] : 0.f;
+    }
+    v[i] = a;
+  }
+  float* dst = g.out + (size_t)m * g.C;
+  if (g.ln_g) {
+    float mean, rstd;
+    ln_moments<NV>(v, g.C, lane, mean, rstd);
+    ln_store<NV>(v, g.C, lane, mean, rstd, g.ln_g, g.ln_b, dst);
+    return;
+  }
+#pragma unroll
+  for (int i = 0; i < NV; ++i) {
+    const int c = lane * 4 + i * 256;
+    if (c < g.C) *reinterpret_cast<f32x4*>(dst + c) = v[i];
+  }
+}
+
+hipError_t launch_entry_gather(const EntryGather& g, hipStream_t st) {
+  if (g.M <= 0) return hipSuccess;
+  if (g.C <= 0 || g.C % 4 != 0 || g.C > 1536 || g.S <= 0 || !g.bias || !g.out || (g.ln_g && (!g.ln_b || g.C > 1024))) return hipErrorInvalidValue;
+  for (int s = 0; s < g.nsrc && s < ENTRY_MAX_SRC; ++s)
+    if (!g.src[s].tab || g.src[s].ld % 4 != 0 || g.src[s].ld < g.C || g.src[s].rows <= 0 || g.src[s].shift < -1 || g.src[s].shift > 1) return hipErrorInvalidValue;
+  dim3 grid((g.M + 3) / 4), block(256);
+  const int nv = (g.C + 255) / 256;
+#define NS_ENTRY(NV, NS) hipLaunchKernelGGL((k_entry_gather<NV, NS>), grid, block, 0, st, g)
+  if (g.ln_g && (g.nsrc == 3 || g.nsrc == 6)) {
+    const bool six = g.nsrc == 6;
+    if (nv == 1) { if (six) NS_ENTRY(1, 6); else NS_ENTRY(1, 3); }
+    else if (nv == 2) { if (six) NS_ENTRY(2, 6); else NS_ENTRY(2, 3); }
+    else { if (six) NS_ENTRY(4, 6); else NS_ENTRY(4, 3); }
+  } else if (!g.ln_g && g.nsrc == 4) {
+    if (nv <= 3) NS_ENTRY(3, 4); else NS_ENTRY(6, 4);
+  } else {
+    return hipErrorInvalidValue;
+  }
+#undef NS_ENTRY
   return hipGetLastError();
 }
 
diff --git a/smart-nar_fast_tts_amd/ops.py b/smart-nar_fast_tts_amd/ops.py
--- a/smart-nar_fast_tts_amd/ops.py
+++ b/smart-nar_fast_tts_amd/ops.py
@@ -547,3 +547,74 @@
                                         _lib.ptr(mel_bias), _lib.ptr(post_const), _lib.ptr(mel), _lib.ptr(post), _lib.ptr(pp), _lib.ptr(ep),
                                         _lib.ptr(mm), _st(mel_p)), "unpack_outputs")
     return mel, post, pp, ep, mm
+
+
+def entry_width(model) -> int:
+    return int(model._lib.ns_entry_width(model._h))
+
+
+def entry_consumers(model, B: int, L: int) -> int:
+    return int(model._lib.ns_entry_consumers(model._h, int(B), int(L)))
+
+
+def entry_products(model, enc_out):
+    B, L, _ = enc_out.shape
+    enc_out = enc_out.contiguous()
+    yh = torch.empty(B, L, entry_width(model), dtype=torch.float32, device=enc_out.device)
+    _lib.check(model._lib.ns_op_entry_products(model._h, _lib.ptr(enc_out), B, L, _lib.ptr(yh), _st(enc_out)), "entry_products")
+    return yh
+
+
+def entry_length_regulate(x, cum, T: int, mel_lens=None, H: int = 2, fill: int = 0):
+    lib = _lib.load()
+    B, L, D = x.shape
+    x, cum = x.contiguous(), cum.int().contiguous()
+    if mel_lens is None:
+        out = torch.empty(B, T, D, dtype=torch.float32, device=x.device)
+        pidx = torch.full((B, T), fill, dtype=torch.int32, device=x.device)
+        mask = torch.full((B, T), 7, dtype=torch.uint8, device=x.device)
+        _lib.check(lib.ns_op_entry_length_regulate(_lib.ptr(x), _lib.ptr(cum), _lib.ptr(None), B, L, D, int(T), 0, int(H), _lib.ptr(out), _lib.ptr(pidx),
+                                                   _lib.ptr(mask), _lib.ptr(None), 0, _st(x)), "entry_length_regulate")
+        return out, pidx, mask
+    mel_lens = mel_lens.long().contiguous()
+    p = pack_plan(mel_lens.cpu().tolist(), T, H, 20)
+    p.plan = torch.full((pack_plan_ints(B, p.Mp),), fill, dtype=torch.int32, device=x.device)
+    out = torch.empty(p.Mp, D, dtype=torch.float32, device=x.device)
+    pidx = torch.full((p.Mp,), fill, dtype=torch.int32, device=x.device)
+    _lib.check(lib.ns_op_entry_length_regulate(_lib.ptr(x), _lib.ptr(cum), _lib.ptr(mel_lens), B, L, D, int(T), p.Mp, int(H), _lib.ptr(out),
+                                               _lib.ptr(pidx), _lib.ptr(None), _lib.ptr(p.plan), p.plan.numel(), _st(x)), "entry_length_regulate")
+    return out, pidx, p
+
+
+def entry_predictor_tail(model, prefix, h, lens, x_in, control: float = 1.0, target=None, add_pos: bool = False, fill: int = -7):
+    B, S, _ = h.shape
+    h, lens, x_in = h.contiguous(), lens.long().contiguous(), x_in.contiguous()
+    pred = torch.empty(B, S, dtype=torch.float32, device=h.device)
+    x_out = torch.empty_like(x_in)
+    bucket = torch.full((B, S), fill, dtype=torch.int32, device=h.device)
+    if target is not None:
+        target = target.contiguous().float()
+    ws = _ws(model, B, S)
+    _lib.check(model._lib.ns_op_entry_predictor_tail(model._h, prefix.encode(), _lib.ptr(h), _lib.ptr(lens), B, S, float(control), _lib.ptr(target),
+                                                     _lib.ptr(x_in), int(bool(add_pos)), _lib.ptr(pred), _lib.ptr(x_out), _lib.ptr(bucket),
+                                                     _lib.ptr(ws), ws.numel(), _st(h)), "entry_predictor_tail")
+    return pred, x_out, bucket
+
+
+def entry_gather(model, which: int, yh, pidx, bkt_p=None, bkt_e=None, S: int | None = None, p: PackedPlan | None = None):
+    B, L, _ = yh.shape
+    yh, pidx = yh.contiguous(), pidx.int().contiguous()
+    bkt_p = bkt_p.int().contiguous() if bkt_p is not None else None
+    bkt_e = bkt_e.int().contiguous() if bkt_e is not None else None
+    C = 3 * model._cfg.d_dec if which == 2 else model._cfg.vp_filter
+    if p is None:
+        S = int(pidx.shape[1] if S is None else S)
+        out = torch.empty(B, S, C, dtype=torch.float32, device=yh.device)
+        args = (_lib.ptr(None), B, L, S, 0, 0)
+    else:
+        assert pidx.numel() == p.Mp and p.B == B
+        out = torch.empty(p.Mp, C, dtype=torch.float32, device=yh.device)
+        args = (_lib.ptr(p.plan), B, L, p.S, p.Mp, p.att_wgs)
+    _lib.check(model._lib.ns_op_entry_gather(model._h, int(which), _lib.ptr(yh), _lib.ptr(pidx), _lib.ptr(bkt_p), _lib.ptr(bkt_e), *args,
+                                             _lib.ptr(out), _st(yh)), "entry_gather")
+    return out
```

Result: no change. 2.956 million, median of 6 (+0.7%).
